# smrt-model/smrt

Measured on AMD Instinct MI355X. Metric: snowpack x frequency DORT solves/sec (20 layers, 32 streams), higher is better.
Workload: dtype f64

## Files before the change

__graft_entry__.py:

```python
import os
import subprocess
import sys
from concurrent.futures import ThreadPoolExecutor

ROOT = os.path.dirname(os.path.abspath(__file__))
CSRC = os.path.join(ROOT, "smrt_amd", "csrc")
LIB = os.path.join(CSRC, "libsmrt_dort.so")
OBJ_DIR = os.path.join(CSRC, "build")
EMU_DIR = os.path.join(ROOT, "tests", "hostemu")
EMU_LIB = os.path.join(EMU_DIR, "libsmrt_emu.so")


def _newer(target, sources):
    if not os.path.exists(target):
        return True
    t = os.path.getmtime(target)
    return any(os.path.getmtime(s) > t for s in sources)


def _run(cmd):
    print("+", " ".join(cmd), flush=True)
    subprocess.check_call(cmd, cwd=ROOT)


def _unit_flags(src):
    with open(src) as fh:
        for _ in range(10):
            line = fh.readline()
            if line.startswith("// hipcc-flags:"):
                return line.split(":", 1)[1].split()
    return []


def _compile_objects(hipcc, sources, headers, force, extra_flags=()):
    from concurrent.futures import ThreadPoolExecutor

    os.makedirs(OBJ_DIR, exist_ok=True)
    jobs = []
    for src in sources:
        obj = os.path.join(OBJ_DIR, os.path.basename(src)[:-4] + ".o")
        if force or _newer(obj, [src] + headers):
            jobs.append([hipcc, "--offload-arch=gfx950", "-O3", "-std=c++17", "-fPIC", "-fvisibility=hidden", "-Rpass-analysis=kernel-resource-usage",
                         *_unit_flags(src), *extra_flags, "-c", src, "-o", obj])

    def compile_one(cmd):
        print("+", " ".join(cmd), flush=True)
        proc = subprocess.run(cmd, cwd=ROOT, stderr=subprocess.PIPE, text=True)
        remarks, other = [], []
        for line in proc.stderr.splitlines():
            (remarks if "kernel-resource-usage" in line else other).append(line)
        kept = [ln for ln in other if not ln.lstrip().startswith(("|", "^")) and "__global__" not in ln]
        if proc.returncode != 0:
            sys.stderr.write(proc.stderr)
            raise subprocess.CalledProcessError(proc.returncode, cmd)
        if kept:
            sys.stderr.write("\n".join(kept) + "\n")
        with open(cmd[-1][:-2] + ".resources.txt", "w") as fh:
            fh.write("\n".join(ln.split("remark:", 1)[1].replace("[-Rpass-analysis=kernel-resource-usage]", "").rstrip()
                               for ln in remarks if "remark:" in ln) + "\n")

    if jobs:
        with ThreadPoolExecutor(max_workers=min(len(jobs), os.cpu_count() or 1)) as pool:
            list(pool.map(compile_one, jobs))
    return [os.path.join(OBJ_DIR, os.path.basename(src)[:-4] + ".o") for src in sources], bool(jobs)


def build(force=False):
    units = sorted(os.path.join(CSRC, f) for f in os.listdir(CSRC) if f.endswith(".hip"))
    headers = sorted(os.path.join(CSRC, f) for f in os.listdir(CSRC) if f.endswith(".hpp"))
    headers.append(os.path.join(ROOT, "include", "smrt_dort.h"))
    hip_src = [os.path.join(CSRC, "dort_hip.hip")] + headers
    hipcc = os.environ.get("HIPCC") or ("/opt/rocm/bin/hipcc" if os.path.exists("/opt/rocm/bin/hipcc") else "hipcc")
    objects, rebuilt = _compile_objects(hipcc, units, headers, force)
    if rebuilt or not os.path.exists(LIB):
        _run([hipcc, "--offload-arch=gfx950", "-shared", "-fPIC", "-o", LIB, *objects, "-ldl"])
    emu_src = hip_src[1:] + [os.path.join(EMU_DIR, "emu_lib.cpp"), os.path.join(EMU_DIR, "emu_runtime.hpp")]
    emu_jobs = [(lib, flags) for lib, flags in ((EMU_LIB, ["-O2"]), (EMU_LIB[:-3] + "_fastpanel.so", ["-O2", "-DSMRT_GJ_FAST_PANEL"]),
                                                (EMU_LIB[:-3] + "_asan.so", ["-O1", "-g", "-fsanitize=address"]))
                if force or _newer(lib, emu_src)]
    if emu_jobs:
        with ThreadPoolExecutor(max_workers=len(emu_jobs)) as pool:
            list(pool.map(lambda j: _run(["g++", "-std=c++17", "-shared", "-fPIC", *j[1], "-I", EMU_DIR, "-o", j[0],
                                          os.path.join(EMU_DIR, "emu_lib.cpp")]), emu_jobs))
    rough_lib = os.path.join(EMU_DIR, "librough_boundary_host.so")
    rough_src = os.path.join(EMU_DIR, "rough_boundary_host.cpp")
    if force or _newer(rough_lib, hip_src[1:] + [rough_src, os.path.join(EMU_DIR, "emu_runtime.hpp")]):
        _run(["g++", "-O2", "-std=c++17", "-shared", "-fPIC", "-DSMRT_HOST_EMU", "-I", EMU_DIR, "-o", rough_lib, rough_src])
    prep_lib = os.path.join(EMU_DIR, "libprep_layer_host.so")
    prep_src = os.path.join(EMU_DIR, "prep_layer_host.cpp")
    if force or _newer(prep_lib, emu_src + [prep_src]):
        _run(["g++", "-O2", "-std=c++17", "-shared", "-fPIC", "-I", EMU_DIR, "-o", prep_lib, prep_src])
    if ROOT not in sys.path:
        sys.path.insert(0, ROOT)
    import smrt_amd
    from smrt_amd import _native

    lib = _native.load_library()
    missing = [s for s in _native.EXPORTED_SYMBOLS if not hasattr(lib, s)]
    if missing:
        raise RuntimeError("libsmrt_dort.so lacks symbols: %s" % missing)
    print("build ok:", lib.smrt_dort_version().decode())


def smoke():
    if ROOT not in sys.path:
        sys.path.insert(0, ROOT)
    import numpy as np

    from oracle import dort_oracle as O
    from smrt_amd._native import DortContext, PackedBatch

    sp = dict(thickness=np.array([0.1, 100.0]), density=np.array([200.0, 400.0]),
              temperature=np.array([250.0, 250.0]), microstructure="exponential",
              corr_length=np.array([5e-5, 5e-5]))
    theta = np.deg2rad([55.0])
    batch = PackedBatch([2], sp["thickness"], sp["density"] / O.DENSITY_OF_ICE, sp["temperature"], sp["corr_length"],
                        None, [36.5e9], theta)
    ctx = DortContext(0)
    out = ctx.run(batch)
    assert out.status[0] == 0, out.status
    tb = out.values[0]
    ref = O.solve(sp, 36.5e9, [55.0])
    print("smoke: Tb(V,H) gpu =", tb[:, 0], " oracle =", ref[:, 0], " kernel ms =", ctx.last_kernel_ms())
    assert np.abs(tb - ref).max() < 1e-6
    assert np.abs(tb[:, 0] - np.array([248.09044325849692, 237.3487270223389])).max() < 1e-4
    radar = PackedBatch([2], sp["thickness"], sp["density"] / O.DENSITY_OF_ICE, sp["temperature"], sp["corr_length"],
                        None, [19e9], theta, mode="A", m_max=2)
    out = ctx.run(radar)
    assert out.status[0] == 0, out.status
    ref = O.solve(sp, 19e9, [55.0], mode="A", theta_inc_deg=[55.0])
    sig = 10 * np.log10(4 * np.pi * np.cos(theta[0]) * np.array([out.values[0][0, 0, 0], out.values[0][1, 1, 0], out.values[0][1, 0, 0]]))
    print("smoke: sigma0 (VV, HH, HV) gpu =", sig, "dB")
    assert (np.abs(out.values[0] - ref)[:2, :2] / np.abs(ref[:2, :2]).max(axis=(0, 1))).max() < 1e-8
    assert np.abs(sig - np.array([-24.044882546524693, -24.416295329469907, -51.544272924876886])).max() < 1e-4
    ctx.close()
    print("smoke ok")


if __name__ == "__main__":
    build(force="--force" in sys.argv)
    if "smoke" in sys.argv:
        smoke()
```

include/smrt_dort.h:

```cpp
#ifndef SMRT_DORT_H
#define SMRT_DORT_H

#include <stdint.h>

#ifdef __cplusplus
extern "C" {
#endif
#if defined(__GNUC__)
#pragma GCC visibility push(default)
#endif

typedef struct smrt_dort_ctx smrt_dort_ctx;

#define SMRT_EM_IBA 0
#define SMRT_EM_DMRT_QCA_SHORTRANGE 1
#define SMRT_EM_DMRT_QCACP_SHORTRANGE 2
#define SMRT_EM_NONSCATTERING 3
#define SMRT_EM_HOST 4
#define SMRT_EM_IBA_INVERTED 5
#define SMRT_EM_IBA_HOST 6
#define SMRT_EM_RAYLEIGH_HOST 7
#define SMRT_MS_EXPONENTIAL 0
#define SMRT_MS_STICKY_HARD_SPHERES 1
#define SMRT_MS_INDEPENDENT_SPHERE 2
// ... 29 lines not shown
    int32_t n_layers_max;
    int32_t n_frequencies;
    int32_t n_theta;
    int32_t emmodel;
    int32_t microstructure;
    int32_t mode;
    int32_t n_max_stream;
    int32_t m_max;
    int32_t phase_normalization;
    int32_t rayleigh_jeans;
    int32_t substrate_kind;
    const int32_t* n_layers;
    const double* thickness;
    const double* frac_volume;
    const double* temperature;
    const double* micro_p1;
    const double* micro_p2;
    const double* frequency;
    const double* theta;
    double phi;
    const double* substrate_p1;
    const double* substrate_p2;
    const double* substrate_temperature;
    const double* atm_tb_down;
    const double* atm_tb_up;
    const double* atm_transmittance;
    double prune_optical_depth;
    const int32_t* layer_kind;
    const double* host_layer;
    const int32_t* host_streams;
    const double* host_phase;
    int32_t process_coherent_layers;
    const double* host_substrate;
    const double* host_substrate_coh;
    const int32_t* host_interface_slot;
    const double* host_interface;
    const double* host_interface_coh;
    int32_t host_interface_slots;
    const double* liquid_water;
    const double* host_iba_coeff;
    const int32_t* rough_kind;
    const double* rough_params;
} smrt_batch;

#define SMRT_ROUGH_NONE 0
#define SMRT_ROUGH_GEOMETRICAL_OPTICS 1
#define SMRT_ROUGH_GEOMETRICAL_OPTICS_BACKSCATTER 2
#define SMRT_ROUGH_IEM_FUNG92 3
#define SMRT_ROUGH_M_MAX 4

int32_t smrt_dort_rough_matrices(smrt_dort_ctx* ctx, const smrt_batch* batch, int32_t* slot, double* itf, double* itf_coh,
                                 double* sub, double* sub_coh);
int32_t smrt_dort_rough_info(smrt_dort_ctx* ctx, double* info, int32_t n);

int32_t smrt_dort_out_stride(const smrt_batch* b);

int32_t smrt_dort_device_count(void);

int32_t smrt_dort_create(smrt_dort_ctx** ctx, int32_t device);
void smrt_dort_destroy(smrt_dort_ctx* ctx);
const char* smrt_dort_last_error(const smrt_dort_ctx* ctx);

int32_t smrt_dort_run(smrt_dort_ctx* ctx, const smrt_batch* batch, int64_t pair_begin, int64_t pair_count,
                      double* out, int32_t* status, double* layer_out, double* stream_out);

int32_t smrt_dort_run_pairs(smrt_dort_ctx* ctx, const smrt_batch* batch, const int64_t* pairs, int64_t n_pairs,
                            double* out, int32_t* status, double* layer_out, double* stream_out);

int32_t smrt_dort_upload(smrt_dort_ctx* ctx, const smrt_batch* batch, int64_t pair_begin, int64_t pair_count);
int32_t smrt_dort_upload_pairs(smrt_dort_ctx* ctx, const smrt_batch* batch, const int64_t* pairs, int64_t n_pairs);
int32_t smrt_dort_launch(smrt_dort_ctx* ctx, void* out_dev, void* status_dev);
int32_t smrt_dort_sync(smrt_dort_ctx* ctx);
int32_t smrt_dort_download(smrt_dort_ctx* ctx, double* out, int32_t* status, double* layer_out,
                           double* stream_out);

double smrt_dort_last_kernel_ms(smrt_dort_ctx* ctx);

int32_t smrt_dort_kernel_breakdown(smrt_dort_ctx* ctx, int32_t enable, double* ms3);

int32_t smrt_dort_set_diagonalisation(smrt_dort_ctx* ctx, int32_t mode);

int32_t smrt_dort_set_prep(smrt_dort_ctx* ctx, int32_t mode);

enum { SMRT_INFO_PIPELINE = 0, SMRT_INFO_CHUNK_PAIRS, SMRT_INFO_CHUNKS, SMRT_INFO_PRUNE_ROUNDS, SMRT_INFO_STAGED_ITEMS,
       SMRT_INFO_BLOCK_THREADS, SMRT_INFO_N_MAX, SMRT_INFO_DIAGONALISATION, SMRT_INFO_RAYLEIGH_CLOSED_FORM, SMRT_INFO_PREP,
       SMRT_INFO_COUNT };
enum { SMRT_PREP_PER_PAIR = 0, SMRT_PREP_PER_LAYER = 1 };
enum { SMRT_DIAG_JACOBI = 0,
       SMRT_DIAG_SYMMETRIC = 1 };
enum { SMRT_PIPELINE_FUSED = 0,
       SMRT_PIPELINE_LDS_TWO_SLOT = 1,
       SMRT_PIPELINE_LDS_FOUR_SLOT = 2,
       SMRT_PIPELINE_LDS_REG = 3,
       SMRT_PIPELINE_FUSED_GMEM = 4,
       SMRT_PIPELINE_GMEM = 5,
       SMRT_PIPELINE_BIG = 6,
       SMRT_PIPELINE_GMEM_STRIP = 7,
       SMRT_PIPELINE_LDS_STRIP = 8 };
int32_t smrt_dort_launch_info(smrt_dort_ctx* ctx, int64_t* info, int32_t n);
double smrt_dort_total_kernel_ms(smrt_dort_ctx* ctx, int64_t* n_launches, int32_t reset);

int32_t smrt_dort_set_block_threads(smrt_dort_ctx* ctx, int32_t threads);

int32_t smrt_dort_set_pipeline(smrt_dort_ctx* ctx, int32_t split);

int32_t smrt_dort_finish_reg_lds_bytes(int32_t n_max_stream, int32_t n_layers_max);

int32_t smrt_dort_finish_strip_lds_bytes(int32_t n_max_stream, int32_t n_layers_max, int32_t wavefronts);

int32_t smrt_dort_jacobi_lds_bytes(int32_t n_max_stream, int32_t n_pol, int32_t size_class_columns);

double smrt_dort_sum_n3(smrt_dort_ctx* ctx);

int32_t smrt_dort_ft_even_phase(smrt_dort_ctx* ctx, int32_t emmodel, int32_t microstructure, double frequency,
                                double frac_volume, double temperature, double micro_p1, double micro_p2,
                                const double* mu_s, int32_t n_s, const double* mu_i, int32_t n_i, int32_t m_max,
                                int32_t npol, double* out);

int32_t smrt_dort_pair_cost(smrt_dort_ctx* ctx, double* cost);

int32_t smrt_dort_stage_cycles(smrt_dort_ctx* ctx, double* out16);

int32_t smrt_gauss_legendre_positive(int32_t n, double* mu, double* weight);

#define SMRT_COMM_ID_BYTES 128
int32_t smrt_dort_comm_library(char* path, int32_t capacity, int32_t* version);
int32_t smrt_dort_comm_unique_id(char* id);
int32_t smrt_dort_comm_init(smrt_dort_ctx* ctx, int32_t world, int32_t rank, const char* id);
int32_t smrt_dort_comm_init_all(smrt_dort_ctx** ctxs, int32_t n);
int32_t smrt_dort_comm_destroy(smrt_dort_ctx* ctx);
int32_t smrt_dort_gather(smrt_dort_ctx* ctx, int32_t root, const int64_t* counts, double* out, int32_t* status);
int32_t smrt_dort_comm_allreduce_max(smrt_dort_ctx* ctx, double* values, int32_t n);

typedef struct smrt_gather_op { int32_t peer; int32_t reserved; int64_t offset_rows; int64_t rows; } smrt_gather_op;
int32_t smrt_dort_gather_plan(int32_t world, int32_t root, int32_t rank, const int64_t* counts, smrt_gather_op* ops,
                              int32_t capacity, int64_t* own_offset_rows, int64_t* total_rows);

int32_t smrt_dort_abi(int32_t* out, int32_t capacity);

const char* smrt_dort_version(void);

typedef struct smrt_first_order_extras {
    int32_t n_interface_slots;
    int32_t reserved;
    const int32_t* host_interface_slot;
    const double* host_interface_values;
    const double* host_phase_samples;
} smrt_first_order_extras;

int32_t smrt_first_order_out_stride(const smrt_batch* b);
int32_t smrt_first_order_run_pairs(smrt_dort_ctx* ctx, const smrt_batch* batch, const smrt_first_order_extras* extras,
                                   const int64_t* pairs, int64_t n_pairs, double* out, int32_t* status, double* layer_out,
                                   double* backscatter_layer, double* diag);
int32_t smrt_first_order_upload_pairs(smrt_dort_ctx* ctx, const smrt_batch* batch, const smrt_first_order_extras* extras,
                                      const int64_t* pairs, int64_t n_pairs);
int32_t smrt_first_order_launch(smrt_dort_ctx* ctx);
int32_t smrt_first_order_sync(smrt_dort_ctx* ctx);
int32_t smrt_first_order_download(smrt_dort_ctx* ctx, double* out, int32_t* status, double* layer_out,
                                  double* backscatter_layer, double* diag);
int32_t smrt_first_order_kernel_ms(smrt_dort_ctx* ctx, double* ms2);
int32_t smrt_first_order_abi(int32_t* out, int32_t capacity);

typedef struct smrt_second_order_extras {
    int32_t compute_scattering_interlayer;
    int32_t reserved;
    int64_t workspace_budget_bytes;
    const smrt_first_order_extras* first_order;
    const double* substrate_diffuse_modes;
} smrt_second_order_extras;
// ... 151 lines not shown
```

smrt_amd/_native.py:

```python
from __future__ import annotations

import ctypes as C
import os
import threading

import numpy as np

from .core.error import SMRTError

_HERE = os.path.dirname(os.path.abspath(__file__))
LIB_PATH = os.environ.get("SMRT_DORT_LIB") or os.path.join(_HERE, "csrc", "libsmrt_dort.so")

EM_CODES = {"iba": 0, "dmrt_qca_shortrange": 1, "dmrt_qcacp_shortrange": 2, "nonscattering": 3, "host": 4,
            "iba_inverted": 5, "iba_host": 6, "rayleigh_host": 7}
MS_CODES = {"exponential": 0, "sticky_hard_spheres": 1, "independent_sphere": 2, "teubner_strey": 3,
            "unified_scaled_exponential": 0, "unified_sticky_hard_spheres": 1, "unified_teubner_strey": 3,
            "exponential_complex_k": 4, "sticky_hard_spheres_complex_k": 5, "independent_sphere_complex_k": 6,
            "teubner_strey_complex_k": 7}
SUBSTRATE_CODES = {"flat": 1, "reflector": 2, "host": 3, "soil_wegmuller": 4, "soil_qnh": 5, "rough_choudhury79": 6}
SOIL_KINDS = ("soil_wegmuller", "soil_qnh", "rough_choudhury79")
NORM_CODES = {False: 0, None: 0, True: 1, "auto": 1, "forced": 2}
STATUS_MESSAGES = {
    1: "The eigen-decomposition did not converge in DORT.",
    2: "The re-normalization of the phase function exceeds the predefined threshold of 30%. This is likely because "
# ... 531 lines not shown
                _dptr(self.vertical), _dptr(self.echo))


_lib = None


def load_library():
    global _lib
    if _lib is not None:
        return _lib
    if not os.path.exists(LIB_PATH):
        raise SMRTError(f"{LIB_PATH} is missing: build it with `python __graft_entry__.py` (hipcc, gfx950). "
                        "smrt_amd has no CPU fallback.")
    lib = C.CDLL(LIB_PATH)
    P = C.POINTER
    lib.smrt_dort_version.restype = C.c_char_p
    lib.smrt_dort_out_stride.argtypes = [P(SmrtBatch)]
    lib.smrt_dort_out_stride.restype = C.c_int32
    lib.smrt_dort_create.argtypes = [P(C.c_void_p), C.c_int32]
    lib.smrt_dort_create.restype = C.c_int32
    lib.smrt_dort_destroy.argtypes = [C.c_void_p]
    lib.smrt_dort_destroy.restype = None
    lib.smrt_dort_last_error.argtypes = [C.c_void_p]
    lib.smrt_dort_last_error.restype = C.c_char_p
    lib.smrt_dort_run.argtypes = [C.c_void_p, P(SmrtBatch), C.c_int64, C.c_int64, P(C.c_double), P(C.c_int32),
                                  P(C.c_double), P(C.c_double)]
    lib.smrt_dort_run.restype = C.c_int32
    lib.smrt_dort_upload.argtypes = [C.c_void_p, P(SmrtBatch), C.c_int64, C.c_int64]
    lib.smrt_dort_upload.restype = C.c_int32
    lib.smrt_dort_run_pairs.argtypes = [C.c_void_p, P(SmrtBatch), P(C.c_int64), C.c_int64, P(C.c_double), P(C.c_int32),
                                        P(C.c_double), P(C.c_double)]
    lib.smrt_dort_run_pairs.restype = C.c_int32
    lib.smrt_dort_upload_pairs.argtypes = [C.c_void_p, P(SmrtBatch), P(C.c_int64), C.c_int64]
    lib.smrt_dort_upload_pairs.restype = C.c_int32
    lib.smrt_dort_ft_even_phase.argtypes = [C.c_void_p, C.c_int32, C.c_int32, C.c_double, C.c_double, C.c_double, C.c_double,
                                            C.c_double, P(C.c_double), C.c_int32, P(C.c_double), C.c_int32, C.c_int32, C.c_int32,
                                            P(C.c_double)]
    lib.smrt_dort_ft_even_phase.restype = C.c_int32
    lib.smrt_dort_rough_matrices.argtypes = [C.c_void_p, P(SmrtBatch), P(C.c_int32), P(C.c_double), P(C.c_double), P(C.c_double),
                                             P(C.c_double)]
    lib.smrt_dort_rough_matrices.restype = C.c_int32
    lib.smrt_dort_rough_info.argtypes = [C.c_void_p, P(C.c_double), C.c_int32]
    lib.smrt_dort_rough_info.restype = C.c_int32
    lib.smrt_dort_pair_cost.argtypes = [C.c_void_p, P(C.c_double)]
    lib.smrt_dort_pair_cost.restype = C.c_int32
    lib.smrt_dort_launch_info.argtypes = [C.c_void_p, P(C.c_int64), C.c_int32]
    lib.smrt_dort_launch_info.restype = C.c_int32
    lib.smrt_dort_comm_library.argtypes = [C.c_char_p, C.c_int32, P(C.c_int32)]
    lib.smrt_dort_comm_library.restype = C.c_int32
    lib.smrt_dort_comm_unique_id.argtypes = [C.c_char_p]
    lib.smrt_dort_comm_unique_id.restype = C.c_int32
    lib.smrt_dort_comm_init.argtypes = [C.c_void_p, C.c_int32, C.c_int32, C.c_char_p]
    lib.smrt_dort_comm_init.restype = C.c_int32
    lib.smrt_dort_comm_init_all.argtypes = [P(C.c_void_p), C.c_int32]
    lib.smrt_dort_comm_init_all.restype = C.c_int32
    lib.smrt_dort_comm_destroy.argtypes = [C.c_void_p]
    lib.smrt_dort_comm_destroy.restype = C.c_int32
    lib.smrt_dort_gather.argtypes = [C.c_void_p, C.c_int32, P(C.c_int64), P(C.c_double), P(C.c_int32)]
    lib.smrt_dort_gather.restype = C.c_int32
    lib.smrt_dort_comm_allreduce_max.argtypes = [C.c_void_p, P(C.c_double), C.c_int32]
    lib.smrt_dort_comm_allreduce_max.restype = C.c_int32
    lib.smrt_dort_abi.argtypes = [P(C.c_int32), C.c_int32]
    lib.smrt_dort_abi.restype = C.c_int32
    lib.smrt_dort_launch.argtypes = [C.c_void_p, C.c_void_p, C.c_void_p]
    lib.smrt_dort_launch.restype = C.c_int32
    lib.smrt_dort_sync.argtypes = [C.c_void_p]
    lib.smrt_dort_sync.restype = C.c_int32
    lib.smrt_dort_download.argtypes = [C.c_void_p, P(C.c_double), P(C.c_int32), P(C.c_double), P(C.c_double)]
    lib.smrt_dort_download.restype = C.c_int32
    lib.smrt_dort_last_kernel_ms.argtypes = [C.c_void_p]
    lib.smrt_dort_last_kernel_ms.restype = C.c_double
    lib.smrt_dort_kernel_breakdown.argtypes = [C.c_void_p, C.c_int32, P(C.c_double)]
    lib.smrt_dort_kernel_breakdown.restype = C.c_int32
    lib.smrt_dort_total_kernel_ms.argtypes = [C.c_void_p, P(C.c_int64), C.c_int32]
    lib.smrt_dort_total_kernel_ms.restype = C.c_double
    lib.smrt_dort_set_block_threads.argtypes = [C.c_void_p, C.c_int32]
    lib.smrt_dort_set_block_threads.restype = C.c_int32
    lib.smrt_dort_set_pipeline.argtypes = [C.c_void_p, C.c_int32]
    lib.smrt_dort_set_pipeline.restype = C.c_int32
    lib.smrt_dort_set_diagonalisation.argtypes = [C.c_void_p, C.c_int32]
    lib.smrt_dort_set_diagonalisation.restype = C.c_int32
    lib.smrt_dort_set_prep.argtypes = [C.c_void_p, C.c_int32]
    lib.smrt_dort_set_prep.restype = C.c_int32
    lib.smrt_dort_gather_plan.argtypes = [C.c_int32, C.c_int32, C.c_int32, P(C.c_int64), C.c_void_p, C.c_int32,
                                          P(C.c_int64), P(C.c_int64)]
    lib.smrt_dort_gather_plan.restype = C.c_int32
    lib.smrt_dort_finish_reg_lds_bytes.argtypes = [C.c_int32, C.c_int32]
    lib.smrt_dort_finish_reg_lds_bytes.restype = C.c_int32
    lib.smrt_dort_finish_strip_lds_bytes.argtypes = [C.c_int32, C.c_int32, C.c_int32]
    lib.smrt_dort_finish_strip_lds_bytes.restype = C.c_int32
    lib.smrt_dort_jacobi_lds_bytes.argtypes = [C.c_int32, C.c_int32, C.c_int32]
    lib.smrt_dort_jacobi_lds_bytes.restype = C.c_int32
    lib.smrt_dort_sum_n3.argtypes = [C.c_void_p]
    lib.smrt_dort_sum_n3.restype = C.c_double
    lib.smrt_dort_stage_cycles.argtypes = [C.c_void_p, P(C.c_double)]
    lib.smrt_dort_stage_cycles.restype = C.c_int32
    lib.smrt_dort_device_count.argtypes = []
    lib.smrt_dort_device_count.restype = C.c_int32
    lib.smrt_gauss_legendre_positive.argtypes = [C.c_int32, P(C.c_double), P(C.c_double)]
    lib.smrt_gauss_legendre_positive.restype = C.c_int32
    X = P(FirstOrderExtras)
    lib.smrt_first_order_out_stride.argtypes = [P(SmrtBatch)]
    lib.smrt_first_order_out_stride.restype = C.c_int32
    lib.smrt_first_order_run_pairs.argtypes = [C.c_void_p, P(SmrtBatch), X, P(C.c_int64), C.c_int64, P(C.c_double), P(C.c_int32),
                                               P(C.c_double), P(C.c_double), P(C.c_double)]
    lib.smrt_first_order_run_pairs.restype = C.c_int32
    lib.smrt_first_order_upload_pairs.argtypes = [C.c_void_p, P(SmrtBatch), X, P(C.c_int64), C.c_int64]
    lib.smrt_first_order_upload_pairs.restype = C.c_int32
    lib.smrt_first_order_launch.argtypes = [C.c_void_p]
    lib.smrt_first_order_launch.restype = C.c_int32
    lib.smrt_first_order_sync.argtypes = [C.c_void_p]
    lib.smrt_first_order_sync.restype = C.c_int32
    lib.smrt_first_order_download.argtypes = [C.c_void_p, P(C.c_double), P(C.c_int32), P(C.c_double), P(C.c_double), P(C.c_double)]
    lib.smrt_first_order_download.restype = C.c_int32
    lib.smrt_first_order_kernel_ms.argtypes = [C.c_void_p, P(C.c_double)]
    lib.smrt_first_order_kernel_ms.restype = C.c_int32
    lib.smrt_first_order_abi.argtypes = [P(C.c_int32), C.c_int32]
    lib.smrt_first_order_abi.restype = C.c_int32
    X2 = P(SecondOrderExtras)
    lib.smrt_second_order_out_stride.argtypes = [P(SmrtBatch)]
    lib.smrt_second_order_run_pairs.argtypes = [C.c_void_p, P(SmrtBatch), X2, P(C.c_int64), C.c_int64, P(C.c_double), P(C.c_int32),
                                                P(C.c_double), P(C.c_double), P(C.c_double)]
    lib.smrt_second_order_upload_pairs.argtypes = [C.c_void_p, P(SmrtBatch), X2, P(C.c_int64), C.c_int64]
    lib.smrt_second_order_launch.argtypes = [C.c_void_p]
    lib.smrt_second_order_sync.argtypes = [C.c_void_p]
    lib.smrt_second_order_download.argtypes = [C.c_void_p, P(C.c_double), P(C.c_int32), P(C.c_double), P(C.c_double), P(C.c_double)]
    lib.smrt_second_order_kernel_ms.argtypes = [C.c_void_p, P(C.c_double)]
    lib.smrt_second_order_abi.argtypes = [P(C.c_int32), C.c_int32]
    for name in ("out_stride", "run_pairs", "upload_pairs", "launch", "sync", "download", "kernel_ms", "abi"):
        getattr(lib, "smrt_second_order_" + name).restype = C.c_int32
    so_out = [P(C.c_double), P(C.c_int32), P(C.c_double), P(C.c_double), P(C.c_int32), P(C.c_double), P(C.c_int32)]
    lib.smrt_successive_order_out_stride.argtypes = [P(SmrtBatch), C.c_int32]
    lib.smrt_successive_order_out_stride.restype = C.c_int32
    lib.smrt_successive_order_run_pairs.argtypes = [C.c_void_p, P(SmrtBatch), C.c_int32, C.c_double, C.c_int64, P(C.c_int64), C.c_int64] + so_out
    lib.smrt_successive_order_run_pairs.restype = C.c_int32
    lib.smrt_successive_order_upload_pairs.argtypes = [C.c_void_p, P(SmrtBatch), C.c_int32, C.c_double, C.c_int64, P(C.c_int64), C.c_int64]
    lib.smrt_successive_order_upload_pairs.restype = C.c_int32
    lib.smrt_successive_order_launch.argtypes = [C.c_void_p]
    lib.smrt_successive_order_launch.restype = C.c_int32
    lib.smrt_successive_order_sync.argtypes = [C.c_void_p]
    lib.smrt_successive_order_sync.restype = C.c_int32
    lib.smrt_successive_order_download.argtypes = [C.c_void_p] + so_out
    lib.smrt_successive_order_download.restype = C.c_int32
    lib.smrt_successive_order_kernel_ms.argtypes = [C.c_void_p, P(C.c_double)]
    lib.smrt_successive_order_kernel_ms.restype = C.c_int32
    lib.smrt_successive_order_launch_info.argtypes = [C.c_void_p, P(C.c_int64), C.c_int32]
    lib.smrt_successive_order_launch_info.restype = C.c_int32
    soa_in = [C.c_void_p, P(SmrtBatch), C.c_int32, C.c_double, C.c_int32, P(C.c_double), C.c_int32, C.c_int32, C.c_int64, P(C.c_int64),
              C.c_int64]
    lib.smrt_so_active_out_stride.argtypes = [C.c_int32, C.c_int32]
    lib.smrt_so_active_out_stride.restype = C.c_int32
    lib.smrt_so_active_run_pairs.argtypes = soa_in + so_out
    lib.smrt_so_active_run_pairs.restype = C.c_int32
    lib.smrt_so_active_upload_pairs.argtypes = soa_in
    lib.smrt_so_active_upload_pairs.restype = C.c_int32
    lib.smrt_so_active_launch.argtypes = [C.c_void_p]
    lib.smrt_so_active_launch.restype = C.c_int32
    lib.smrt_so_active_sync.argtypes = [C.c_void_p]
    lib.smrt_so_active_sync.restype = C.c_int32
    lib.smrt_so_active_download.argtypes = [C.c_void_p] + so_out
    lib.smrt_so_active_download.restype = C.c_int32
    lib.smrt_so_active_kernel_ms.argtypes = [C.c_void_p, P(C.c_double)]
    lib.smrt_so_active_kernel_ms.restype = C.c_int32
    lib.smrt_so_active_launch_info.argtypes = [C.c_void_p, P(C.c_int64), C.c_int32]
    lib.smrt_so_active_launch_info.restype = C.c_int32
    mf_out = [P(C.c_double), P(C.c_int32), P(C.c_int32), P(C.c_double), P(C.c_double)]
# ... 42 lines not shown
    return lib


def abi_layout(lib):
    n = lib.smrt_dort_abi(None, 0)
    a = (C.c_int32 * n)()
    lib.smrt_dort_abi(a, n)
    return list(a)


def check_struct_layout(lib):
    mine = [C.sizeof(SmrtBatch)] + [getattr(SmrtBatch, name).offset for name, _ in SmrtBatch._fields_]
    theirs = abi_layout(lib)
    if mine != theirs:
        raise SMRTError(f"smrt_batch layout mismatch between smrt_amd/_native.py {mine} and {LIB_PATH} {theirs}: "
                        "rebuild the library or update the binding (include/smrt_dort.h)")
    mine, theirs = first_order_extras_layout(), first_order_abi_layout(lib)
    if mine != theirs:
        raise SMRTError(f"smrt_first_order_extras layout mismatch between smrt_amd/_native.py {mine} and {LIB_PATH} {theirs}: "
                        "rebuild the library or update the binding (include/smrt_dort.h)")
    mine, theirs = second_order_extras_layout(), second_order_abi_layout(lib)
    if mine != theirs:
        raise SMRTError(f"smrt_second_order_extras layout mismatch between smrt_amd/_native.py {mine} and {LIB_PATH} {theirs}: "
                        "rebuild the library or update the binding (include/smrt_dort.h)")
    mine, theirs = lrm_params_layout(), lrm_abi_layout(lib)
    if mine != theirs:
        raise SMRTError(f"smrt_lrm_params layout mismatch between smrt_amd/_native.py {mine} and {LIB_PATH} {theirs}: "
                        "rebuild the library or update the binding (include/smrt_dort.h)")
    mine, theirs = sar_params_layout(), sar_abi_layout(lib)
    if mine != theirs:
        raise SMRTError(f"smrt_sar_params layout mismatch between smrt_amd/_native.py {mine} and {LIB_PATH} {theirs}: "
                        "rebuild the library or update the binding (include/smrt_dort.h)")


def sar_params_layout():
    return [C.sizeof(SarParams)] + [getattr(SarParams, name).offset for name, _ in SarParams._fields_]


def sar_abi_layout(lib):
    n = lib.smrt_sar_abi(None, 0)
    a = (C.c_int32 * n)()
    lib.smrt_sar_abi(a, n)
    return list(a)


def lrm_params_layout():
    return [C.sizeof(LrmParams)] + [getattr(LrmParams, name).offset for name, _ in LrmParams._fields_]


def lrm_abi_layout(lib):
    n = lib.smrt_lrm_abi(None, 0)
    a = (C.c_int32 * n)()
    lib.smrt_lrm_abi(a, n)
    return list(a)


def second_order_extras_layout():
    return [C.sizeof(SecondOrderExtras)] + [getattr(SecondOrderExtras, name).offset for name, _ in SecondOrderExtras._fields_]


def second_order_abi_layout(lib):
    n = lib.smrt_second_order_abi(None, 0)
    a = (C.c_int32 * n)()
    lib.smrt_second_order_abi(a, n)
    return list(a)


def first_order_extras_layout():
    return [C.sizeof(FirstOrderExtras)] + [getattr(FirstOrderExtras, name).offset for name, _ in FirstOrderExtras._fields_]


def first_order_abi_layout(lib):
    n = lib.smrt_first_order_abi(None, 0)
    a = (C.c_int32 * n)()
    lib.smrt_first_order_abi(a, n)
    return list(a)


EXPORTED_SYMBOLS = [
    "smrt_dort_out_stride", "smrt_dort_create", "smrt_dort_destroy", "smrt_dort_last_error", "smrt_dort_run",
    "smrt_dort_upload", "smrt_dort_upload_pairs", "smrt_dort_run_pairs", "smrt_dort_abi", "smrt_dort_pair_cost", "smrt_dort_ft_even_phase",
    "smrt_dort_launch_info", "smrt_dort_comm_library", "smrt_dort_comm_unique_id", "smrt_dort_comm_init", "smrt_dort_comm_init_all", "smrt_dort_comm_destroy", "smrt_dort_gather",
    "smrt_dort_comm_allreduce_max", "smrt_dort_launch", "smrt_dort_sync", "smrt_dort_download", "smrt_dort_last_kernel_ms", "smrt_dort_kernel_breakdown",
    "smrt_dort_total_kernel_ms", "smrt_dort_set_block_threads", "smrt_dort_set_pipeline", "smrt_dort_set_diagonalisation", "smrt_dort_set_prep", "smrt_dort_sum_n3", "smrt_dort_stage_cycles", "smrt_dort_device_count", "smrt_gauss_legendre_positive",
    "smrt_dort_version", "smrt_dort_finish_reg_lds_bytes", "smrt_dort_finish_strip_lds_bytes", "smrt_dort_jacobi_lds_bytes", "smrt_dort_gather_plan",
    "smrt_first_order_out_stride", "smrt_first_order_run_pairs", "smrt_first_order_upload_pairs", "smrt_first_order_launch",
    "smrt_first_order_sync", "smrt_first_order_download", "smrt_first_order_kernel_ms", "smrt_first_order_abi",
    "smrt_second_order_out_stride", "smrt_second_order_run_pairs", "smrt_second_order_upload_pairs", "smrt_second_order_launch",
    "smrt_second_order_sync", "smrt_second_order_download", "smrt_second_order_kernel_ms", "smrt_second_order_abi",
    "smrt_successive_order_out_stride", "smrt_successive_order_run_pairs", "smrt_successive_order_upload_pairs",
    "smrt_successive_order_launch", "smrt_successive_order_sync", "smrt_successive_order_download",
    "smrt_successive_order_kernel_ms", "smrt_successive_order_launch_info",
    "smrt_so_active_out_stride", "smrt_so_active_run_pairs", "smrt_so_active_upload_pairs", "smrt_so_active_launch",
    "smrt_so_active_sync", "smrt_so_active_download", "smrt_so_active_kernel_ms", "smrt_so_active_launch_info",
    "smrt_multifresnel_out_stride", "smrt_multifresnel_run_pairs", "smrt_multifresnel_upload_pairs", "smrt_multifresnel_launch",
    "smrt_multifresnel_sync", "smrt_multifresnel_download", "smrt_multifresnel_kernel_ms",
    "smrt_lrm_out_stride", "smrt_lrm_run_pairs", "smrt_lrm_upload_pairs", "smrt_lrm_launch", "smrt_lrm_sync", "smrt_lrm_download",
    "smrt_lrm_kernel_ms", "smrt_lrm_abi", "smrt_lrm_layers",
    "smrt_sar_out_stride", "smrt_sar_run_pairs", "smrt_sar_upload_pairs", "smrt_sar_launch", "smrt_sar_sync", "smrt_sar_download",
    "smrt_sar_kernel_ms", "smrt_sar_abi",
    "smrt_dort_rough_matrices", "smrt_dort_rough_info",
]


class RoughMatrices:

    def __init__(self, batch):
        s = batch.struct
        S, Lmax = int(s.n_snowpacks), int(s.n_layers_max)
        FS, ne = batch.n_pairs, 3 * int(s.n_max_stream)
        nm = int(s.m_max) + 1 if batch.mode == "A" else 1
        kinds = batch.rough_kind
        self.slots = max(int(np.count_nonzero(kinds[k, :batch.n_layers[k]])) for k in range(S))
        self.has_substrate = bool(kinds[0, batch.n_layers[0]])
        self.slot = -np.ones((FS, Lmax), np.int32)
        self.itf = np.zeros((FS, self.slots, nm, 4, ne, ne))
        self.itf_coh = np.zeros((FS, self.slots, 4, ne))
        self.sub = np.zeros((FS, nm, ne, ne))
        self.sub_coh = np.zeros((FS, nm, ne))

    def pointers(self):
        return (self.slot.ctypes.data_as(C.POINTER(C.c_int32)), _dptr(self.itf), _dptr(self.itf_coh), _dptr(self.sub),
                _dptr(self.sub_coh))


class BatchOutput:
    def __init__(self, batch, pair_count):
        Lmax, nmax = int(batch.struct.n_layers_max), int(batch.struct.n_max_stream)
        self.values = np.empty((pair_count,) + batch.out_shape(), dtype=np.float64)
        self.status = np.empty(pair_count, dtype=np.int32)
        self.layers = np.empty((pair_count, Lmax, 5), dtype=np.float64)
        self.streams = np.empty((pair_count, 1 + nmax), dtype=np.float64)


class DortContext:

    def __init__(self, device=0):
        self._lib = load_library()
        self._h = C.c_void_p()
        rc = self._lib.smrt_dort_create(C.byref(self._h), int(device))
        if rc != 0:
            self._h = C.c_void_p()
            raise SMRTError(f"smrt_dort_create(device={device}) failed with code {rc}: no usable MI355X GPU. "
                            "smrt_amd has no CPU fallback.")
        self.device = int(device)
        self.lock = threading.RLock()

    def close(self):
        if getattr(self, "_h", None) is not None and self._h.value:
            self._lib.smrt_dort_destroy(self._h)
            self._h = C.c_void_p()

    def __del__(self):
        try:
            self.close()
        except Exception:
            pass

    def _check(self, rc, what):
        if rc != 0:
            raise SMRTError(f"{what} failed: {self._lib.smrt_dort_last_error(self._h).decode()}")

    def set_block_threads(self, n):
        self._check(self._lib.smrt_dort_set_block_threads(self._h, int(n)), "smrt_dort_set_block_threads")

    def set_pipeline(self, split=1):
        self._check(self._lib.smrt_dort_set_pipeline(self._h, int(split)), "smrt_dort_set_pipeline")

    DIAGONALISATIONS = ("jacobi", "symmetric")

    def set_diagonalisation(self, mode="default"):
        code = -1 if mode in (None, "default") else self.DIAGONALISATIONS.index(mode)
        self._check(self._lib.smrt_dort_set_diagonalisation(self._h, code), "smrt_dort_set_diagonalisation")

    PREPS = ("per_pair", "per_layer")

    def set_prep(self, mode="default"):
        code = -1 if mode in (None, "default") else self.PREPS.index(mode)
        self._check(self._lib.smrt_dort_set_prep(self._h, code), "smrt_dort_set_prep")

    def run(self, batch: PackedBatch, pair_begin=0, pair_count=-1, pairs=None) -> BatchOutput:
        if pairs is not None:
            pairs = np.ascontiguousarray(pairs, dtype=np.int64)
            o = BatchOutput(batch, len(pairs))
            with self.lock:
                self._check(self._lib.smrt_dort_run_pairs(
                    self._h, C.byref(batch.struct), pairs.ctypes.data_as(C.POINTER(C.c_int64)), len(pairs),
                    _dptr(o.values), o.status.ctypes.data_as(C.POINTER(C.c_int32)), _dptr(o.layers), _dptr(o.streams)),
                    "smrt_dort_run_pairs")
            return o
        if pair_count < 0:
            pair_count = batch.n_pairs - pair_begin
        o = BatchOutput(batch, pair_count)
        with self.lock:
            self._check(self._lib.smrt_dort_run(self._h, C.byref(batch.struct), pair_begin, pair_count, _dptr(o.values),
                                                o.status.ctypes.data_as(C.POINTER(C.c_int32)), _dptr(o.layers),
                                                _dptr(o.streams)), "smrt_dort_run")
        return o

    def upload(self, batch: PackedBatch, pair_begin=0, pair_count=-1, pairs=None):
        if pairs is not None:
            pairs = np.ascontiguousarray(pairs, dtype=np.int64)
            self._check(self._lib.smrt_dort_upload_pairs(self._h, C.byref(batch.struct),
                                                         pairs.ctypes.data_as(C.POINTER(C.c_int64)), len(pairs)),
                        "smrt_dort_upload_pairs")
            self._resident = (batch, len(pairs))
            return
        if pair_count < 0:
            pair_count = batch.n_pairs - pair_begin
        self._check(self._lib.smrt_dort_upload(self._h, C.byref(batch.struct), pair_begin, pair_count), "smrt_dort_upload")
        self._resident = (batch, pair_count)

    def launch(self, out_dev=None, status_dev=None):
        self._check(self._lib.smrt_dort_launch(self._h, C.c_void_p(out_dev or 0), C.c_void_p(status_dev or 0)),
                    "smrt_dort_launch")

    def sync(self):
        self._check(self._lib.smrt_dort_sync(self._h), "smrt_dort_sync")

    def download(self) -> BatchOutput:
        batch, pair_count = self._resident
        o = BatchOutput(batch, pair_count)
        self._check(self._lib.smrt_dort_download(self._h, _dptr(o.values), o.status.ctypes.data_as(C.POINTER(C.c_int32)),
                                                 _dptr(o.layers), _dptr(o.streams)), "smrt_dort_download")
        return o

    def _solver_call(self, symbol, *args):
        with self.lock:
            rc = getattr(self._lib, symbol)(self._h, *args)
            if rc < 0:
                raise SMRTError(f"{symbol} failed: {self._lib.smrt_dort_last_error(self._h).decode()}")
        return rc

    def _solver_run(self, prefix, output, cargs, oargs):
        o = output(*oargs)
        self._solver_call(f"smrt_{prefix}_run_pairs", *cargs, *o.pointers())
        return o

    def _solver_upload(self, prefix, cargs, oargs):
        with self.lock:
            self._solver_call(f"smrt_{prefix}_upload_pairs", *cargs)
            setattr(self, f"_{prefix}_resident", oargs)

    def _solver_download(self, prefix, output):
        with self.lock:
            o = output(*getattr(self, f"_{prefix}_resident"))
            self._solver_call(f"smrt_{prefix}_download", *o.pointers())
        return o

    def _solver_kernel_ms(self, prefix, n):
        a = np.zeros(n)
        self._solver_call(f"smrt_{prefix}_kernel_ms", _dptr(a))
        return tuple(float(x) for x in a)

    def _solver_launch_info(self, prefix):
        a = np.zeros(4, dtype=np.int64)
        self._solver_call(f"smrt_{prefix}_launch_info", a.ctypes.data_as(C.POINTER(C.c_int64)), 4)
        return dict(chunks=int(a[0]), reserved_bytes=int(a[1]), over_budget=int(a[2]), budget=int(a[3]))

    @staticmethod
    def _pair_list(batch, pairs):
        if pairs is None:
            return None, -1, batch.n_pairs
# ... 159 lines not shown
        self._solver_upload("lrm", *self._lrm_pack(batch, params, pairs))

    def lrm_layers(self, batch: PackedBatch, params):
        a = np.empty((batch.n_pairs, int(batch.struct.n_layers_max), 5))
        with self.lock:
            self.lrm_upload(batch, params)
            self._solver_call("smrt_lrm_layers", _dptr(a))
        return a

    def lrm_launch(self):
        self._solver_call("smrt_lrm_launch")

    def lrm_sync(self):
        self._solver_call("smrt_lrm_sync")

    def lrm_download(self) -> LrmOutput:
        return self._solver_download("lrm", LrmOutput)

    def lrm_kernel_ms(self):
        return self._solver_kernel_ms("lrm", 3)

    def sar_run(self, batch: PackedBatch, params, pairs=None) -> SarOutput:
        return self._solver_run("sar", SarOutput, *self._lrm_pack(batch, params, pairs))

    def sar_upload(self, batch: PackedBatch, params, pairs=None):
        self._solver_upload("sar", *self._lrm_pack(batch, params, pairs))

    def sar_launch(self):
        self._solver_call("smrt_sar_launch")

    def sar_sync(self):
        self._solver_call("smrt_sar_sync")

    def sar_download(self) -> SarOutput:
        return self._solver_download("sar", SarOutput)

    def sar_kernel_ms(self):
        return self._solver_kernel_ms("sar", 4)

    def ft_even_phase(self, emmodel, microstructure, frequency, frac_volume, temperature, p1, p2, mu_s, mu_i, m_max, npol):
        mu_s = np.ascontiguousarray(np.atleast_1d(mu_s), dtype=np.float64)
        mu_i = np.ascontiguousarray(np.atleast_1d(mu_i), dtype=np.float64)
        out = np.empty((npol, npol, m_max + 1, len(mu_s), len(mu_i)))
        with self.lock:
            self._check(self._lib.smrt_dort_ft_even_phase(
                self._h, EM_CODES[emmodel], MS_CODES[microstructure], float(frequency), float(frac_volume), float(temperature),
                float(p1), float(p2), _dptr(mu_s), len(mu_s), _dptr(mu_i), len(mu_i), int(m_max), int(npol), _dptr(out)),
                "smrt_dort_ft_even_phase")
        return out

    rough_on_device = True

    @property
    def rough_workspace_budget(self):
        v = (C.c_double * 6)()
        self._lib.smrt_dort_rough_info(self._h, v, 6)
        return min(4 << 30, int(0.5 * v[5]))

    def rough_matrices(self, batch: PackedBatch) -> RoughMatrices:
        o = RoughMatrices(batch)
        with self.lock:
            rc = self._lib.smrt_dort_rough_matrices(self._h, C.byref(batch.struct), *o.pointers())
            self._check(0 if rc >= 0 else -1, "smrt_dort_rough_matrices")
        return o

    def rough_info(self):
        v = (C.c_double * 5)()
        self._lib.smrt_dort_rough_info(self._h, v, 5)
        return dict(m_max_limit=int(v[0]), slots=int(v[1]), builder_ms=float(v[2]), built_bytes=int(v[3]), host_matrix_bytes=int(v[4]))

    def pair_cost(self):
        _, pair_count = self._resident
        cost = np.empty(pair_count)
        self._check(self._lib.smrt_dort_pair_cost(self._h, _dptr(cost)), "smrt_dort_pair_cost")
        return cost

    PIPELINES = ("fused", "lds_two_slot", "lds_four_slot", "lds_reg", "fused_gmem", "gmem", "big", "gmem_strip", "lds_strip")

    def launch_info(self):
        v = (C.c_int64 * 16)()
        n = self._lib.smrt_dort_launch_info(self._h, v, 16)
        self._check(0 if n > 0 else -1, "smrt_dort_launch_info")
        keys = ("pipeline", "chunk_pairs", "chunks", "prune_rounds", "staged_items", "block_threads", "n_max", "diagonalisation",
                "rayleigh_closed_form", "prep")
        d = {k: int(v[i]) for i, k in enumerate(keys[:n])}
        d["pipeline"] = self.PIPELINES[d["pipeline"]]
        d["diagonalisation"] = self.DIAGONALISATIONS[d["diagonalisation"]]
        d["rayleigh_closed_form"] = bool(d.get("rayleigh_closed_form", 0))
        d["prep"] = self.PREPS[d.get("prep", 0)]
        if d.get("staged_items", -1) < 0:
            d["staged_items"] = None
        return d

    @staticmethod
    def comm_library():
        lib = load_library()
        buf, version = C.create_string_buffer(1024), C.c_int32(0)
        if lib.smrt_dort_comm_library(buf, len(buf), C.byref(version)) != 0:
            raise SMRTError("RCCL is not available: " + buf.value.decode(errors="replace"))
        v = int(version.value)
        return buf.value.decode(), "%d.%d.%d" % (v // 10000, v // 100 % 100, v % 100) if v >= 10000 else str(v)

    @staticmethod
    def comm_unique_id():
        lib = load_library()
        buf = C.create_string_buffer(128)
        if lib.smrt_dort_comm_unique_id(buf) != 0:
            raise SMRTError("smrt_dort_comm_unique_id failed (is librccl available?)")
        return buf.raw

    def comm_init(self, world, rank, unique_id):
        self._check(self._lib.smrt_dort_comm_init(self._h, int(world), int(rank), bytes(unique_id)), "smrt_dort_comm_init")
        self.world, self.rank = int(world), int(rank)

    @staticmethod
    def comm_init_all(contexts):
        lib = load_library()
        arr = (C.c_void_p * len(contexts))(*[c._h for c in contexts])
        if lib.smrt_dort_comm_init_all(arr, len(contexts)) != 0:
            raise SMRTError("smrt_dort_comm_init_all failed: " + lib.smrt_dort_last_error(contexts[0]._h).decode())
        for r, c in enumerate(contexts):
            c.world, c.rank = len(contexts), r

    def gather(self, counts, root=0, want_host=True):
        batch, _ = self._resident
        counts = np.ascontiguousarray(counts, dtype=np.int64)
        is_root = self.rank == root and want_host
        total = int(counts.sum())
        values = np.empty((total,) + batch.out_shape()) if is_root else None
        status = np.empty(total, np.int32) if is_root else None
        self._check(self._lib.smrt_dort_gather(self._h, int(root), counts.ctypes.data_as(C.POINTER(C.c_int64)),
                                               _dptr(values) if is_root else None,
                                               status.ctypes.data_as(C.POINTER(C.c_int32)) if is_root else None),
                    "smrt_dort_gather")
        return values, status

    def allreduce_max(self, values):
        a = np.ascontiguousarray(np.atleast_1d(values), dtype=np.float64).copy()
        self._check(self._lib.smrt_dort_comm_allreduce_max(self._h, _dptr(a), len(a)), "smrt_dort_comm_allreduce_max")
        return a

    def barrier(self):
        self._check(self._lib.smrt_dort_comm_allreduce_max(self._h, None, 0), "smrt_dort_comm_allreduce_max")

    def last_kernel_ms(self):
        return float(self._lib.smrt_dort_last_kernel_ms(self._h))

    def total_kernel_ms(self, reset=False):
        n = C.c_int64()
        ms = float(self._lib.smrt_dort_total_kernel_ms(self._h, C.byref(n), 1 if reset else 0))
        return ms, int(n.value)

    STAGE_NAMES = ["setup", "assemble", "cholesky", "LtL", "jacobi", "triangular", "R1", "LU1", "R45", "LU2", "R78",
                   "out"]

    def kernel_breakdown(self, enable=None):
        if enable is not None:
            self._check(min(self._lib.smrt_dort_kernel_breakdown(self._h, 1 if enable else 0, None), 0), "smrt_dort_kernel_breakdown")
            return None
        a = np.zeros(3)
        n = self._lib.smrt_dort_kernel_breakdown(self._h, -1, _dptr(a))
        self._check(min(n, 0), "smrt_dort_kernel_breakdown")
        return {"prep": float(a[0]), "jacobi": float(a[1]), "finish": float(a[2]), "intervals": int(n)}

    def stage_cycles(self):
        a = np.zeros(16)
        self._check(self._lib.smrt_dort_stage_cycles(self._h, _dptr(a)), "smrt_dort_stage_cycles")
        d = dict(zip(self.STAGE_NAMES, a[: len(self.STAGE_NAMES)]))
        d["_jacobi_sweeps"] = a[12]
        d["_gj_panel"], d["_gj_update"], d["_gj_perm"] = a[13], a[14], a[15]
        return d

# ... 31 lines not shown
```

smrt_amd/csrc/dort_ctx.hpp:

```cpp
#pragma once
#include <hip/hip_runtime.h>
#include <string>
#include <vector>

#include "dort_layout.hpp"

namespace smrt { struct PhaseRequest; struct FoBatch; }
struct smrt_batch;

struct DevBuf {
    void* p = nullptr;
    size_t cap = 0;
    hipError_t reserve(size_t bytes) {
        if (bytes <= cap) return hipSuccess;
        if (p) (void)hipFree(p);
        p = nullptr;
        cap = 0;
        hipError_t e = hipMalloc(&p, bytes);
        if (e == hipSuccess) cap = bytes;
        return e;
    }
    void release() { if (p) (void)hipFree(p); p = nullptr; cap = 0; }
};

struct smrt_dort_ctx {
    int device = 0;
    hipStream_t stream = nullptr;
    hipEvent_t ev0 = nullptr, ev1 = nullptr;
    std::string err;
    DevBuf d_nl, d_thick, d_fv, d_temp, d_p1, d_p2, d_freq, d_theta, d_gl, d_out, d_status, d_layer, d_stream, d_n3, d_stage, d_work, d_stL, d_stB, d_std, d_sts, d_stn, d_sti, d_sub1, d_sub2, d_subT, d_atm, d_pairmap, d_kind, d_phase, d_done, d_hostlayer, d_hostcoeff, d_hoststreams, d_hostphase, d_dispatch, d_regws, d_itfslot, d_itf, d_itfcoh, d_lw, d_ste, d_strot, d_strec;
    smrt::DevBatch dev{};
    bool uploaded = false;
    int out_stride = 0;
    int nt = 256;
    size_t lds_bytes = 0;
    size_t prep_lds_bytes = 0;
    size_t finish2_lds_bytes = 0;
    size_t finish_reg_lds_bytes = 0;
    size_t prep_wide_lds_bytes = 0;
    int prep_mode = -1;
    bool prep_layers = false;
    bool prep_wide = false;
    size_t finish_strip_lds_bytes = 0, finish_strip4_lds_bytes = 0;
    bool finish_strip4 = false;
    bool finish_strip = false;
    bool finish_reg = false;
    int finish_mode = -1;
    bool finish2 = true;
    float last_ms = 0.f;
    double total_ms = 0.0;
    int64_t n_launch = 0;
    bool timing_pending = false;
    bool breakdown_on = false;
    std::vector<hipEvent_t> bd_events;
    std::vector<int> bd_kind;
    size_t bd_used = 0;
    int max_lds = 0;
    bool split = true;
    long long chunk_pairs = 0;
    int lanes = 1;
    hipStream_t lane_stream[4] = {nullptr, nullptr, nullptr, nullptr};
    hipEvent_t lane_ev[4] = {nullptr, nullptr, nullptr, nullptr};
    hipEvent_t fork_ev = nullptr;
    size_t jacobi_lds = 0;
    int diag_mode = -1;
    bool eig = false;
    size_t jacobi16_lds = 0;
    smrt::DevStage stage{};
    bool gmem_path = false;
    bool gmem_split = false;
    bool big = false;
    int jac_in_lds = 0;
    bool active = false;
    int gmem_grid = 0;
    long long ws_stride = 0;
    int nmax_rows = 0;
    void* comm = nullptr;
    int comm_world = 0, comm_rank = 0;
    DevBuf d_gather_out, d_gather_status, d_scalar;
    struct FirstOrderState* first_order = nullptr;
    struct SuccessiveOrderState* successive_order = nullptr;
    struct SuccessiveOrderActiveState* successive_order_active = nullptr;
    struct MultiFresnelState* multifresnel = nullptr;
    struct SecondOrderState* second_order = nullptr;
    struct LrmState* lrm = nullptr;
    struct SarState* sar = nullptr;
    struct RoughState* rough = nullptr;
    struct { int slots = 0, has_sub = 0; float ms = 0.f; size_t built_bytes = 0, host_matrix_bytes = 0; } rough_info;
};

#ifndef SMRT_JACOBI_NT
#define SMRT_JACOBI_NT 256
#endif

namespace smrt_launch {
hipError_t prep(smrt_dort_ctx* ctx, const smrt::DevBatch& c, int nt);
hipError_t prep_wide(smrt_dort_ctx* ctx, const smrt::DevBatch& c);
hipError_t finish(smrt_dort_ctx* ctx, const smrt::DevBatch& c, int nt, bool two_slot);
void occupancy_report(smrt_dort_ctx* ctx, int nt);
hipError_t prep_layers(smrt_dort_ctx* ctx, const smrt::DevBatch& c, long long items);
hipError_t finish_reg(smrt_dort_ctx* ctx, const smrt::DevBatch& c);
hipError_t finish_strip(smrt_dort_ctx* ctx, const smrt::DevBatch& c);
hipError_t finish_strip4(smrt_dort_ctx* ctx, const smrt::DevBatch& c);
hipError_t jacobi(smrt_dort_ctx* ctx, const smrt::DevBatch& c, long long items);
hipError_t eig(smrt_dort_ctx* ctx, const smrt::DevBatch& c, long long items);
hipError_t rayleigh(smrt_dort_ctx* ctx, const smrt::DevBatch& c, long long items);
hipError_t active_prep(smrt_dort_ctx* ctx, const smrt::DevBatch& c, int nt);
hipError_t active_finish(smrt_dort_ctx* ctx, const smrt::DevBatch& c, int nt);
hipError_t prep_gmem(smrt_dort_ctx* ctx, const smrt::DevBatch& c, unsigned grid, bool active);
hipError_t finish_gmem(smrt_dort_ctx* ctx, const smrt::DevBatch& c, unsigned grid, bool active);
hipError_t prep_gmem_big(smrt_dort_ctx* ctx, const smrt::DevBatch& c, unsigned grid, bool active, int ch);
hipError_t finish_gmem_big(smrt_dort_ctx* ctx, const smrt::DevBatch& c, unsigned grid, bool active, int ch);
hipError_t jacobi_big(smrt_dort_ctx* ctx, const smrt::DevBatch& c, long long items);
hipError_t fused(smrt_dort_ctx* ctx, const smrt::DevBatch& d, int nt, bool active);
hipError_t fused_gmem(smrt_dort_ctx* ctx, const smrt::DevBatch& d, int ch, bool active);
hipError_t ft_even_phase(smrt_dort_ctx* ctx, const smrt::PhaseRequest& q);
hipError_t prune_mark(smrt_dort_ctx* ctx, const smrt::DevBatch& c, int* done_dev);
hipError_t pair_cost(smrt_dort_ctx* ctx, const smrt::DevBatch& d, double* cost_dev);
void first_order_release(smrt_dort_ctx* ctx);
void successive_order_release(smrt_dort_ctx* ctx);
void successive_order_active_release(smrt_dort_ctx* ctx);
void multifresnel_release(smrt_dort_ctx* ctx);
void second_order_release(smrt_dort_ctx* ctx);
void lrm_release(smrt_dort_ctx* ctx);
void sar_release(smrt_dort_ctx* ctx);
int rough_prepare(smrt_dort_ctx* ctx, const smrt_batch* b, smrt::DevBatch& d);
void rough_release(smrt_dort_ctx* ctx);
smrt::FoBatch* first_order_resident(smrt_dort_ctx* ctx);
}
```

smrt_amd/csrc/dort_device.hpp:

```cpp
#pragma once
#include "spmd.hpp"
#include <math.h>
#include <string.h>

#include "dort_layout.hpp"
#include "dort_physics.hpp"
#include "dort_dense.hpp"
#include "dort_gauss_jordan.hpp"
#include "dort_passive.hpp"
#include "dort_jacobi_kernel.hpp"
#include "dort_jacobi_big.hpp"
```

smrt_amd/csrc/dort_hip.hip:

```cpp
#include <hip/hip_runtime.h>
#include <algorithm>
#include <cstddef>
#include <cstdio>
#include <cstdlib>
#include <cstring>
#include <string>
#include <vector>

#include "dort_ctx.hpp"
#include "dort_eig_kernel.hpp"
#include "dort_rayleigh_kernel.hpp"
#include "dort_jacobi_big.hpp"
#include "dort_host_common.hpp"
#include "dort_phase_kernel.hpp"
#include "dort_finish_reg.hpp"
#include "dort_finish_strip.hpp"
#include "solver_host.hpp"

using namespace smrt;

static int upload_array(smrt_dort_ctx* ctx, DevBuf& buf, const void* src, size_t bytes) {
    HIPCHK(buf.reserve(bytes));
    HIPCHK(hipMemcpyAsync(buf.p, src, bytes, hipMemcpyHostToDevice, ctx->stream));
    return 0;
}


static DevBatch chunk_of(const smrt_dort_ctx* ctx, const DevBatch& d, long long c0, long long cn) {
    DevBatch c = d;
    c.pair_begin = d.pair_begin + c0; c.pair_count = cn;
    c.out = d.out + c0 * ctx->out_stride; c.status = d.status + c0;
    c.layer_out = d.layer_out + c0 * (long long)d.Lmax * 5;
    c.stream_out = d.stream_out + c0 * (long long)(1 + d.n_max_stream);
    c.n3_out = d.n3_out + c0; c.stage_out = d.stage_out + c0 * 16;
    if (d.dispatch) c.dispatch = d.dispatch + c0;
    return c;
}

#ifndef SMRT_DORT_LANES_DEFAULT
#define SMRT_DORT_LANES_DEFAULT 1
#endif
#ifndef SMRT_PREP_DEFAULT
#define SMRT_PREP_DEFAULT SMRT_PREP_PER_LAYER
#endif
#ifndef SMRT_FINISH_STRIP_DEFAULT
#define SMRT_FINISH_STRIP_DEFAULT 1
#endif
#ifndef SMRT_FINISH_REG_DEFAULT
#define SMRT_FINISH_REG_DEFAULT 1
#endif
static hipError_t launch_pipeline(smrt_dort_ctx* ctx, const DevBatch& d) {
    const long long items_per_pair = (long long)(ctx->active ? d.m_max + 1 : 1) * d.Lmax;
    const long long modes = ctx->active ? d.m_max + 1 : 1;
    if (getenv("SMRT_DORT_DEBUG_OCCUPANCY") && !ctx->gmem_path && !ctx->active) smrt_launch::occupancy_report(ctx, ctx->nt);
    const int rounds = (d.prune_tau > 0.0 && !d.coherent && getenv("SMRT_DORT_NO_PRUNE_ROUNDS") == nullptr) ? std::min(4, d.Lmax) : 1;
    auto prep = [&](const DevBatch& c, unsigned grid) {
        if (ctx->prep_layers) return smrt_launch::prep_layers(ctx, c, c.pair_count * (c.layer_hi - c.layer_lo));
        if (ctx->big) return smrt_launch::prep_gmem_big(ctx, c, grid, ctx->active, ctx->nmax_rows <= 256 ? 4 : 6);
        if (ctx->prep_wide) return smrt_launch::prep_wide(ctx, c);
        if (ctx->gmem_split) return smrt_launch::prep_gmem(ctx, c, grid, ctx->active);
        return ctx->active ? smrt_launch::active_prep(ctx, c, ctx->nt) : smrt_launch::prep(ctx, c, ctx->nt);
    };
    auto finish = [&](const DevBatch& c, unsigned grid) {
        if (ctx->big) return smrt_launch::finish_gmem_big(ctx, c, grid, ctx->active, ctx->nmax_rows <= 256 ? 4 : 6);
        if (ctx->finish_strip) return smrt_launch::finish_strip(ctx, c);
        if (ctx->gmem_split) return smrt_launch::finish_gmem(ctx, c, grid, ctx->active);
        if (ctx->finish_strip4) return smrt_launch::finish_strip4(ctx, c);
        if (ctx->finish_reg) return smrt_launch::finish_reg(ctx, c);
        return ctx->active ? smrt_launch::active_finish(ctx, c, ctx->nt) : smrt_launch::finish(ctx, c, ctx->nt, ctx->finish2);
    };
    const hipStream_t main_stream = ctx->stream;
    const DevStage stage0 = ctx->stage;
    const int lanes = (ctx->lanes > 1 && d.pair_count > ctx->chunk_pairs) ? ctx->lanes : 1;
    struct Restore { smrt_dort_ctx* c; hipStream_t s; DevStage st; ~Restore() { c->stream = s; c->stage = st; } } restore{ctx, main_stream, stage0};
    if (lanes > 1) {
        hipError_t e;
        if ((e = hipEventRecord(ctx->fork_ev, main_stream)) != hipSuccess) return e;
        for (int k = 0; k < lanes; ++k)
            if ((e = hipStreamWaitEvent(ctx->lane_stream[k], ctx->fork_ev, 0)) != hipSuccess) return e;
    }
    auto timed = [&](int kind, auto&& launch) -> hipError_t {
        if (!ctx->breakdown_on) return launch();
        for (int k = 0; k < 2; ++k)
            if (ctx->bd_used + k >= ctx->bd_events.size()) {
                hipEvent_t ev;
                hipError_t e = hipEventCreate(&ev);
                if (e != hipSuccess) return e;
                ctx->bd_events.push_back(ev);
            }
        hipError_t e = hipEventRecord(ctx->bd_events[ctx->bd_used], ctx->stream);
        if (e != hipSuccess) return e;
        e = launch();
        if (e != hipSuccess) return e;
        e = hipEventRecord(ctx->bd_events[ctx->bd_used + 1], ctx->stream);
        ctx->bd_used += 2;
        ctx->bd_kind.push_back(kind);
        return e;
    };
    if (ctx->breakdown_on) { ctx->bd_used = 0; ctx->bd_kind.clear(); }
    long long chunk_index = 0;
    for (long long c0 = 0; c0 < d.pair_count; c0 += ctx->chunk_pairs, ++chunk_index) {
        const long long cn = std::min<long long>(ctx->chunk_pairs, d.pair_count - c0);
        DevBatch c = chunk_of(ctx, d, c0, cn);
        const unsigned grid = (unsigned)(ctx->gmem_path ? std::min<long long>(cn, ctx->gmem_grid) : cn);
        hipError_t e;
        const int lane = (int)(chunk_index % lanes);
        int* done_lane = (int*)ctx->d_done.p + (size_t)lane * ctx->chunk_pairs;
        if (lanes > 1) {
            const long long it0 = (long long)lane * ctx->chunk_pairs * items_per_pair;
            ctx->stream = ctx->lane_stream[lane];
            ctx->stage = stage0;
            ctx->stage.L = stage0.L + it0 * stage0.mat_stride; ctx->stage.B = stage0.B + it0 * stage0.mat_stride;
            ctx->stage.d = stage0.d + it0 * stage0.vec_stride; ctx->stage.sigma = stage0.sigma + it0 * stage0.vec_stride;
            ctx->stage.n = stage0.n + it0; ctx->stage.Linv = stage0.Linv + it0 * stage0.linv_stride;
            if (stage0.eig_rot) { ctx->stage.eig_e = stage0.eig_e + it0 * 2 * stage0.vec_stride; ctx->stage.eig_rot = stage0.eig_rot + it0 * stage0.rot_stride; }
            if (stage0.rec) ctx->stage.rec = stage0.rec + it0 * stage0.rec_stride;
            if (stage0.ws) ctx->stage.ws = stage0.ws + (long long)lane * ctx->chunk_pairs * rg::kSlotDoubles;
        }
        if (rounds > 1 || d.coherent) {
            if ((e = hipMemsetAsync(ctx->stage.n, 0, sizeof(int) * (size_t)(cn * items_per_pair), ctx->stream)) != hipSuccess) return e;
        }
        if (rounds > 1) {
            if ((e = hipMemsetAsync(done_lane, 0, sizeof(int) * (size_t)cn, ctx->stream)) != hipSuccess) return e;
            c.pair_done = (const int*)done_lane;
        }
        for (int r = 0; r < rounds; ++r) {
            c.layer_lo = (int)((long long)d.Lmax * r / rounds);
            c.layer_hi = (int)((long long)d.Lmax * (r + 1) / rounds);
            if ((e = timed(0, [&]() { return prep(c, grid); })) != hipSuccess) return e;
            const long long jitems = cn * modes * (c.layer_hi - c.layer_lo);
            if ((e = timed(1, [&]() { hipError_t e1 = ctx->big ? smrt_launch::jacobi_big(ctx, c, jitems) : ctx->eig ? smrt_launch::eig(ctx, c, jitems) : smrt_launch::jacobi(ctx, c, jitems);
                                           if (e1 == hipSuccess && c.rayleigh_direct) e1 = smrt_launch::rayleigh(ctx, c, jitems);
                                           return e1; })) != hipSuccess) return e;
            if (r + 1 < rounds && (e = smrt_launch::prune_mark(ctx, c, done_lane)) != hipSuccess) return e;
        }
        c.layer_lo = 0; c.layer_hi = d.Lmax; c.pair_done = nullptr;
        if ((e = timed(2, [&]() { return finish(c, grid); })) != hipSuccess) return e;
    }
    if (lanes > 1) {
        for (int k = 0; k < lanes; ++k) {
            hipError_t e;
            if ((e = hipEventRecord(ctx->lane_ev[k], ctx->lane_stream[k])) != hipSuccess) return e;
            if ((e = hipStreamWaitEvent(main_stream, ctx->lane_ev[k], 0)) != hipSuccess) return e;
        }
    }
    return hipSuccess;
}

extern "C" {

const char* smrt_dort_version(void) { return "smrt_dort 0.1 (gfx950)"; }

int32_t smrt_dort_out_stride(const smrt_batch* b) { return smrt_host::out_stride(b); }

int32_t smrt_gauss_legendre_positive(int32_t n, double* mu, double* weight) {
    if (n < 1 || !mu) return -1;
    smrt_host::gauss_legendre_positive(n, mu, weight);
    return 0;
}

int32_t smrt_dort_device_count(void) {
    int ndev = 0;
    if (hipGetDeviceCount(&ndev) != hipSuccess) return 0;
    return ndev;
}

int32_t smrt_dort_create(smrt_dort_ctx** out, int32_t device) {
    if (!out) return -1;
    *out = nullptr;
    int ndev = 0;
    if (hipGetDeviceCount(&ndev) != hipSuccess || ndev <= 0) return -2;
    if (device < 0 || device >= ndev) return -3;
    smrt_dort_ctx* ctx = new smrt_dort_ctx();
    ctx->device = device;
    if (hipSetDevice(device) != hipSuccess || hipStreamCreateWithFlags(&ctx->stream, hipStreamNonBlocking) != hipSuccess ||
        hipEventCreate(&ctx->ev0) != hipSuccess || hipEventCreate(&ctx->ev1) != hipSuccess) {
        delete ctx;
        return -4;
    }
    hipDeviceProp_t prop;
    if (hipGetDeviceProperties(&prop, device) == hipSuccess) ctx->max_lds = (int)prop.sharedMemPerBlock;
    if (ctx->max_lds < 160 * 1024) ctx->max_lds = 160 * 1024;
    *out = ctx;
    return 0;
}

void smrt_dort_destroy(smrt_dort_ctx* ctx) {
    if (!ctx) return;
    (void)smrt_dort_comm_destroy(ctx);
    (void)hipSetDevice(ctx->device);
    DevBuf* bufs[] = {&ctx->d_nl, &ctx->d_thick, &ctx->d_fv, &ctx->d_temp, &ctx->d_p1, &ctx->d_p2, &ctx->d_freq,
                      &ctx->d_theta, &ctx->d_gl, &ctx->d_out, &ctx->d_status, &ctx->d_layer, &ctx->d_stream, &ctx->d_n3, &ctx->d_stage, &ctx->d_work,
                      &ctx->d_stL, &ctx->d_stB, &ctx->d_std, &ctx->d_sts, &ctx->d_stn, &ctx->d_sti, &ctx->d_ste, &ctx->d_strot, &ctx->d_strec, &ctx->d_regws, &ctx->d_itfslot, &ctx->d_itf, &ctx->d_itfcoh,
                      &ctx->d_sub1, &ctx->d_sub2, &ctx->d_subT, &ctx->d_atm, &ctx->d_pairmap, &ctx->d_kind, &ctx->d_hostlayer, &ctx->d_hoststreams, &ctx->d_hostphase, &ctx->d_dispatch, &ctx->d_phase, &ctx->d_done, &ctx->d_lw, &ctx->d_gather_out, &ctx->d_gather_status,
                      &ctx->d_scalar};
    for (DevBuf* b : bufs) b->release();
    smrt_launch::first_order_release(ctx);
    smrt_launch::successive_order_release(ctx);
    smrt_launch::successive_order_active_release(ctx);
    smrt_launch::multifresnel_release(ctx);
    smrt_launch::lrm_release(ctx);
    smrt_launch::sar_release(ctx);
    smrt_launch::second_order_release(ctx);
    smrt_launch::rough_release(ctx);
    if (ctx->ev0) (void)hipEventDestroy(ctx->ev0);
    if (ctx->ev1) (void)hipEventDestroy(ctx->ev1);
    for (int k = 0; k < 4; ++k) {
        if (ctx->lane_ev[k]) (void)hipEventDestroy(ctx->lane_ev[k]);
        if (ctx->lane_stream[k]) (void)hipStreamDestroy(ctx->lane_stream[k]);
    }
    if (ctx->fork_ev) (void)hipEventDestroy(ctx->fork_ev);
    for (hipEvent_t ev : ctx->bd_events) (void)hipEventDestroy(ev);
    if (ctx->stream) (void)hipStreamDestroy(ctx->stream);
    delete ctx;
}

const char* smrt_dort_last_error(const smrt_dort_ctx* ctx) { return ctx ? ctx->err.c_str() : "null context"; }

int32_t smrt_dort_set_pipeline(smrt_dort_ctx* ctx, int32_t split) {
    if (!ctx) return -1;
    ctx->split = (split != 0);
    ctx->finish2 = (split != 2);
    ctx->finish_mode = (split == 3) ? 1 : (split == 4 ? 0 : (split == 5 ? 2 : -1));
    ctx->uploaded = false;
    return 0;
}

int32_t smrt_dort_set_diagonalisation(smrt_dort_ctx* ctx, int32_t mode) {
    if (!ctx) return -1;
    if (mode < -1 || mode > SMRT_DIAG_SYMMETRIC) { ctx->err = "unknown diagonalisation mode"; return -1; }
    ctx->diag_mode = mode;
    ctx->uploaded = false;
    return 0;
}

int32_t smrt_dort_set_prep(smrt_dort_ctx* ctx, int32_t mode) {
    if (!ctx) return -1;
    if (mode < -1 || mode > SMRT_PREP_PER_LAYER) { ctx->err = "unknown prep mode"; return -1; }
    ctx->prep_mode = mode;
    ctx->uploaded = false;
    return 0;
}

int32_t smrt_dort_finish_reg_lds_bytes(int32_t n_max_stream, int32_t n_layers_max) {
    return (int32_t)(sizeof(double) * (size_t)finish_reg_lds_doubles(n_max_stream, n_layers_max));
}

int32_t smrt_dort_finish_strip_lds_bytes(int32_t n_max_stream, int32_t n_layers_max, int32_t wavefronts) {
    if (wavefronts != 4 && wavefronts != 8) return -1;
    return (int32_t)(sizeof(double) * (size_t)finish_strip_lds_doubles(n_max_stream, n_layers_max, wavefronts));
}

int32_t smrt_dort_jacobi_lds_bytes(int32_t n_max_stream, int32_t n_pol, int32_t size_class_columns) {
    if (n_max_stream < 1 || (n_pol != 2 && n_pol != 3) || n_max_stream * n_pol > 128 || size_class_columns < 0) return -1;
    return (int32_t)(make_jacobi_plan(n_max_stream, n_pol, size_class_columns).total * sizeof(double));
}

int32_t smrt_dort_set_block_threads(smrt_dort_ctx* ctx, int32_t threads) {
    if (!ctx) return -1;
    if (threads == 0) threads = 256;
    if (threads != 64 && threads != 256) {
        ctx->err = "block threads must be 64 or 256";
        return -1;
    }
    ctx->nt = threads;
    return 0;
}

}

static int32_t upload_impl(smrt_dort_ctx* ctx, const smrt_batch* b, int64_t pair_begin, int64_t pair_count,
                           const int64_t* pairs) {
    if (!ctx) return -1;
    const char* why = smrt_host::validate(b);
    if (why) { ctx->err = why; return -1; }
    HIPCHK(hipSetDevice(ctx->device));
    ctx->active = (b->mode == SMRT_MODE_ACTIVE);
    if (ctx->active && (b->m_max < 0 || b->m_max > 64)) { ctx->err = "m_max must be in 0..64"; return -1; }
    const int64_t npairs = (int64_t)b->n_snowpacks * b->n_frequencies;
    if (pairs) {
        pair_begin = 0;
        if (pair_count <= 0) { ctx->err = "empty pair list"; return -1; }
        for (int64_t i = 0; i < pair_count; ++i)
            if (pairs[i] < 0 || pairs[i] >= npairs) { ctx->err = "pair index out of bounds"; return -1; }
    } else {
        if (pair_count < 0) pair_count = npairs - pair_begin;
        if (pair_begin < 0 || pair_count <= 0 || pair_begin + pair_count > npairs) { ctx->err = "pair range out of bounds"; return -1; }
    }
    const int P = ctx->active ? 3 : 2;
    const int nphi = ctx->active ? azimuth_samples(b->m_max) / 2 + 1 : 9;
    const int actd = ctx->active ? active_doubles(b->n_max_stream, b->n_layers_max, b->n_theta) : 0;
    const int actd_fin = ctx->active ? active_doubles(b->n_max_stream, b->n_layers_max, b->n_theta, false) : 0;
    LdsPlan plan = make_plan(b->n_max_stream, P, b->n_layers_max, b->n_theta, nphi, 1, actd);
    size_t lds = (size_t)plan.total * sizeof(double);
    ctx->gmem_path = (plan.NMAX > 64 || lds > (size_t)ctx->max_lds || getenv("SMRT_DORT_FORCE_GLOBAL_WORKSPACE") != nullptr);
    if (ctx->gmem_path) {
        if (plan.NMAX > 384) {
            ctx->err = "streams x polarisations above 384 (n_max_stream > 192 passive, > 128 active) is not supported by this build";
            return -1;
        }
        plan = make_plan(b->n_max_stream, P, b->n_layers_max, b->n_theta, nphi, 0, actd, 0, 1);
        ctx->jac_in_lds = 1;
        if ((size_t)plan.total * sizeof(double) > (size_t)ctx->max_lds) {
            plan = make_plan(b->n_max_stream, P, b->n_layers_max, b->n_theta, nphi, 0, actd);
            ctx->jac_in_lds = 0;
        }
        lds = (size_t)plan.total * sizeof(double);
        if (lds > (size_t)ctx->max_lds) { ctx->err = "too many layers for the LDS-resident per-layer tables"; return -1; }
        ctx->gmem_grid = (int)std::min<int64_t>(pair_count, 1024);
        ctx->ws_stride = (long long)plan.mat_doubles + plan.scratch_doubles;
        HIPCHK(ctx->d_work.reserve(sizeof(double) * (size_t)ctx->gmem_grid * (size_t)ctx->ws_stride));
    }
    ctx->nmax_rows = plan.NMAX;
    ctx->chunk_pairs = 0;
    ctx->eig = false;
    {
        int want = ctx->prep_mode < 0 ? SMRT_PREP_DEFAULT : ctx->prep_mode;
        if (const char* e = getenv("SMRT_DORT_PREP_LAYERS")) want = atoi(e) ? SMRT_PREP_PER_LAYER : SMRT_PREP_PER_PAIR;
        ctx->prep_layers = !ctx->gmem_path && ctx->split && !ctx->active && plan.NMAX <= 64 && want == SMRT_PREP_PER_LAYER;
    }
    const size_t rec_doubles = ctx->prep_layers ? (size_t)prep_record_doubles(b->n_max_stream) : 0;
    int big_min = 128;
    if (const char* e = getenv("SMRT_DORT_BIG_MIN_N")) big_min = std::max(64, atoi(e));
    ctx->big = ctx->gmem_path && ctx->split && plan.NMAX > big_min && getenv("SMRT_DORT_NO_BIG_PIPELINE") == nullptr &&
               (size_t)make_jacobi_big_plan(b->n_max_stream, P).total * sizeof(double) <= (size_t)ctx->max_lds;
    const bool split128 = ctx->gmem_path && ctx->split && !ctx->big && plan.NMAX <= 128 &&
        (size_t)make_jacobi_plan(b->n_max_stream, P).total * sizeof(double) <= (size_t)ctx->max_lds &&
        (size_t)make_plan(b->n_max_stream, P, b->n_layers_max, b->n_theta, nphi, 0, actd_fin, 0, 2).total * sizeof(double) <= (size_t)ctx->max_lds &&
        (size_t)make_plan(b->n_max_stream, P, b->n_layers_max, b->n_theta, nphi, 0, actd, 1).total * sizeof(double) <= (size_t)ctx->max_lds;
    if (split128) ctx->jac_in_lds = 1;
    ctx->gmem_split = ctx->big || split128;
    if (ctx->big) ctx->jac_in_lds = 0;
    if ((!ctx->gmem_path && ctx->split) || ctx->gmem_split) {
        const size_t nmodes = ctx->active ? (size_t)b->m_max + 1 : 1;
        const size_t mat = (size_t)plan.NMAX * plan.LD;
        const int linv_stride = (plan.NMAX > 64) ? 2048 : 1024;
        const size_t per_pair = nmodes * b->n_layers_max * ((2 * mat + 2 * plan.NMAX + linv_stride + rec_doubles) * sizeof(double) + sizeof(int));
        double budget = 12.0e9;
        if (ctx->big) {
            size_t free_b = 0, total_b = 0;
            if (hipMemGetInfo(&free_b, &total_b) == hipSuccess) budget = std::max(budget, 0.6 * (double)(free_b + ctx->d_stL.cap + ctx->d_stB.cap));
        }
        const bool one_per_cu = ctx->gmem_split && !ctx->big;
        if (one_per_cu) budget = 40.0e9;
        long long chunk = (long long)(budget / (double)per_pair);
        if (chunk < 1) chunk = 1;
        if (one_per_cu && chunk >= 512) chunk -= chunk % 256;
        const long long chunk_cap = chunk;
        if (chunk > pair_count) chunk = pair_count;
        {
            int want = ctx->diag_mode < 0 ? SMRT_DIAG_SYMMETRIC : ctx->diag_mode;
            if (const char* e = getenv("SMRT_DORT_EIG")) want = atoi(e) ? SMRT_DIAG_SYMMETRIC : SMRT_DIAG_JACOBI;
            ctx->eig = !ctx->gmem_path && !ctx->active && plan.NMAX <= 64 && want == SMRT_DIAG_SYMMETRIC;
        }
        ctx->lanes = 1;
        if (!ctx->gmem_path) {
            int want = ctx->eig ? 3 : SMRT_DORT_LANES_DEFAULT;
            if (const char* e = getenv("SMRT_DORT_LANES")) want = atoi(e);
            ctx->lanes = std::max(1, std::min(4, want));
            while (ctx->lanes > 1 && pair_count < 1024LL * ctx->lanes) --ctx->lanes;
        }
        {
            long long nchunks = (pair_count + chunk - 1) / chunk;
            if (ctx->lanes > 1) nchunks = ((nchunks + ctx->lanes - 1) / ctx->lanes) * ctx->lanes;
            chunk = (pair_count + nchunks - 1) / nchunks;
            if (one_per_cu && nchunks > 1) chunk = std::min(chunk_cap, ((chunk + 255) / 256) * 256);
        }
        ctx->chunk_pairs = chunk;
        for (int k = 0; k < ctx->lanes && ctx->lanes > 1; ++k) {
            if (!ctx->lane_stream[k]) HIPCHK(hipStreamCreateWithFlags(&ctx->lane_stream[k], hipStreamNonBlocking));
            if (!ctx->lane_ev[k]) HIPCHK(hipEventCreateWithFlags(&ctx->lane_ev[k], hipEventDisableTiming));
        }
        if (ctx->lanes > 1 && !ctx->fork_ev) HIPCHK(hipEventCreateWithFlags(&ctx->fork_ev, hipEventDisableTiming));
        const size_t items = (size_t)chunk * ctx->lanes * b->n_layers_max * nmodes;
        HIPCHK(ctx->d_stL.reserve(items * mat * sizeof(double)));
        HIPCHK(ctx->d_stB.reserve(items * mat * sizeof(double)));
        HIPCHK(ctx->d_std.reserve(items * plan.NMAX * sizeof(double)));
        HIPCHK(ctx->d_sts.reserve(items * plan.NMAX * sizeof(double)));
        HIPCHK(ctx->d_stn.reserve(items * sizeof(int)));
        HIPCHK(ctx->d_sti.reserve(ctx->big ? 8 : items * linv_stride * sizeof(double)));
        ctx->stage.L = (double*)ctx->d_stL.p; ctx->stage.B = (double*)ctx->d_stB.p;
        ctx->stage.d = (double*)ctx->d_std.p; ctx->stage.sigma = (double*)ctx->d_sts.p;
        ctx->stage.n = (int*)ctx->d_stn.p; ctx->stage.Linv = ctx->big ? nullptr : (double*)ctx->d_sti.p;
        ctx->stage.linv_stride = linv_stride;
        ctx->stage.mat_stride = (long long)mat; ctx->stage.vec_stride = plan.NMAX;
        ctx->stage.rec = nullptr; ctx->stage.rec_stride = (int)rec_doubles;
        if (ctx->prep_layers) {
            HIPCHK(ctx->d_strec.reserve(items * rec_doubles * sizeof(double)));
            ctx->stage.rec = (double*)ctx->d_strec.p;
        }
        {
            ctx->stage.eig_e = nullptr; ctx->stage.eig_rot = nullptr; ctx->stage.rot_stride = 0;
            if (ctx->eig) {
                const long long rs = eig_rot_doubles(plan.NMAX);
                HIPCHK(ctx->d_ste.reserve(items * 2 * plan.NMAX * sizeof(double)));
                HIPCHK(ctx->d_strot.reserve(items * (size_t)rs * sizeof(double)));
                ctx->stage.eig_e = (double*)ctx->d_ste.p; ctx->stage.eig_rot = (double*)ctx->d_strot.p; ctx->stage.rot_stride = rs;
            }
        }
        ctx->jacobi_lds = ctx->big ? (size_t)make_jacobi_big_plan(b->n_max_stream, P).total * sizeof(double)
                                   : (size_t)make_jacobi_plan(b->n_max_stream, P).total * sizeof(double);
        ctx->jacobi16_lds = 0;
        if (ctx->gmem_split && !ctx->big) {
            const size_t l16 = (size_t)make_jacobi_plan(b->n_max_stream, P, 0, 16).total * sizeof(double);
            if (l16 <= (size_t)ctx->max_lds) ctx->jacobi16_lds = l16;
        }
        ctx->prep_lds_bytes = (size_t)make_plan(b->n_max_stream, P, b->n_layers_max, b->n_theta, nphi, ctx->gmem_split ? 0 : 1, actd,
                                                (!ctx->gmem_split && !ctx->active) ? 3 : 1).total * sizeof(double);
        ctx->finish2_lds_bytes = ctx->gmem_split
            ? (size_t)make_plan(b->n_max_stream, P, b->n_layers_max, b->n_theta, nphi, 0, actd_fin, 0, ctx->big ? 3 : 2).total * sizeof(double)
            : (size_t)make_plan(b->n_max_stream, P, b->n_layers_max, b->n_theta, nphi, 1, actd_fin, 2).total * sizeof(double);
    }
    {
        const bool supported = !ctx->gmem_path && ctx->split && ctx->finish2 && !ctx->active && ctx->chunk_pairs > 0 &&
                               !b->process_coherent_layers && b->substrate_kind != SUB_HOST && !b->host_interface_slot && !b->rough_kind;
        int want = (ctx->finish_mode == 2) ? -1 : ctx->finish_mode;
        if (const char* e = getenv("SMRT_DORT_FINISH_REG")) want = atoi(e) ? 1 : 0;
        ctx->finish_reg_lds_bytes = sizeof(double) * (size_t)finish_reg_lds_doubles(b->n_max_stream, b->n_layers_max);
        const size_t cap = (want == 1) ? (size_t)64 * 1024 : (size_t)160 * 1024 / 3;
        ctx->finish_reg = supported && ctx->finish_reg_lds_bytes <= cap &&
                          (want == 1 || (want == -1 && SMRT_FINISH_REG_DEFAULT));
        ctx->stage.ws = nullptr;
        ctx->finish_strip4 = false;
        {
            int want4 = (ctx->finish_mode == 2) ? 1 : (ctx->finish_mode == -1 ? -1 : 0);
            if (getenv("SMRT_DORT_FINISH_REG") && want == 1 && want4 == -1) want4 = 0;
            if (const char* e = getenv("SMRT_DORT_FINISH_STRIP4")) want4 = atoi(e) ? 1 : 0;
            const size_t lds4 = sizeof(double) * (size_t)finish_strip_lds_doubles(b->n_max_stream, b->n_layers_max, 4);
            const size_t cap4 = (want4 == 1) ? (size_t)64 * 1024 : (size_t)160 * 1024 / 3;
            if (supported && lds4 <= cap4 && (want4 == 1 || (want4 == -1 && SMRT_FINISH_STRIP_DEFAULT))) {
                ctx->finish_strip4 = true; ctx->finish_strip4_lds_bytes = lds4; ctx->finish_reg = false;
                HIPCHK(ctx->d_regws.reserve(sizeof(double) * (size_t)ctx->chunk_pairs * ctx->lanes * StripFinish<4>::kWsDoubles));
                ctx->stage.ws = (double*)ctx->d_regws.p;
            }
        }
        if (ctx->finish_reg) {
            HIPCHK(ctx->d_regws.reserve(sizeof(double) * (size_t)ctx->chunk_pairs * ctx->lanes * rg::kSlotDoubles));
// ... 45 lines not shown
    if (b->host_layer && b->host_streams && b->host_phase) {
        const size_t PL = (size_t)npairs * b->n_layers_max;
        if (upload_array(ctx, ctx->d_hoststreams, b->host_streams, sizeof(int32_t) * PL)) return -1;
        if (upload_array(ctx, ctx->d_hostphase, b->host_phase, sizeof(double) * PL * host_modes * 2 * host_ne * host_ne)) return -1;
    }
    const size_t FS = (size_t)b->n_snowpacks * b->n_frequencies;
    ctx->rough_info = {};
    if (b->host_interface_slot) {
        const size_t ne = 3 * (size_t)b->n_max_stream, nm = ctx->active ? (size_t)b->m_max + 1 : 1, ns = (size_t)b->host_interface_slots;
        if (upload_array(ctx, ctx->d_itfslot, b->host_interface_slot, sizeof(int32_t) * FS * b->n_layers_max)) return -1;
        if (upload_array(ctx, ctx->d_itf, b->host_interface, sizeof(double) * FS * ns * nm * 4 * ne * ne)) return -1;
        if (upload_array(ctx, ctx->d_itfcoh, b->host_interface_coh, sizeof(double) * FS * ns * 4 * ne)) return -1;
        ctx->rough_info.host_matrix_bytes += sizeof(double) * FS * ns * nm * 4 * ne * ne;
    }
    if (b->substrate_kind == SMRT_SUBSTRATE_HOST) {
        const size_t ne = 3 * (size_t)b->n_max_stream, nm = ctx->active ? (size_t)b->m_max + 1 : 1;
        if (upload_array(ctx, ctx->d_sub1, b->host_substrate, sizeof(double) * FS * nm * ne * ne)) return -1;
        if (upload_array(ctx, ctx->d_sub2, b->host_substrate_coh, sizeof(double) * FS * nm * ne)) return -1;
        if (b->substrate_temperature && upload_array(ctx, ctx->d_subT, b->substrate_temperature, sizeof(double) * b->n_snowpacks)) return -1;
        ctx->rough_info.host_matrix_bytes += sizeof(double) * FS * nm * ne * ne;
    } else
    if (smrt_host::rough_substrate(b)) {
        if (upload_array(ctx, ctx->d_subT, b->substrate_temperature, sizeof(double) * b->n_snowpacks)) return -1;
    } else
    if (b->substrate_kind != SMRT_SUBSTRATE_NONE) {
        const size_t sub_doubles = smrt_host::substrate_array_doubles(b);
        if (upload_array(ctx, ctx->d_sub1, b->substrate_p1, sizeof(double) * sub_doubles)) return -1;
        if (upload_array(ctx, ctx->d_sub2, b->substrate_p2, sizeof(double) * sub_doubles)) return -1;
        if (upload_array(ctx, ctx->d_subT, b->substrate_temperature, sizeof(double) * b->n_snowpacks)) return -1;
    }
    std::vector<double> atm;
    if (b->atm_tb_down) {
        atm.insert(atm.end(), b->atm_tb_down, b->atm_tb_down + b->n_frequencies);
        atm.insert(atm.end(), b->atm_tb_up, b->atm_tb_up + b->n_frequencies);
        atm.insert(atm.end(), b->atm_transmittance, b->atm_transmittance + b->n_frequencies);
        if (upload_array(ctx, ctx->d_atm, atm.data(), sizeof(double) * atm.size())) return -1;
    }
    std::vector<double> gl(b->n_max_stream);
    smrt_host::gauss_legendre_positive(b->n_max_stream, gl.data(), nullptr);
    if (upload_array(ctx, ctx->d_gl, gl.data(), sizeof(double) * gl.size())) return -1;
    ctx->out_stride = smrt_host::out_stride(b);
    HIPCHK(ctx->d_out.reserve(sizeof(double) * pair_count * ctx->out_stride));
    HIPCHK(ctx->d_status.reserve(sizeof(int32_t) * pair_count));
    HIPCHK(ctx->d_layer.reserve(sizeof(double) * pair_count * b->n_layers_max * 5));
    HIPCHK(ctx->d_stream.reserve(sizeof(double) * pair_count * (1 + b->n_max_stream)));
    HIPCHK(ctx->d_n3.reserve(sizeof(double) * pair_count));
    HIPCHK(ctx->d_stage.reserve(sizeof(double) * pair_count * 16));
    HIPCHK(hipMemsetAsync(ctx->d_stage.p, 0, sizeof(double) * pair_count * 16, ctx->stream));
    DevBatch& d = ctx->dev;
    d.S = b->n_snowpacks; d.Lmax = b->n_layers_max; d.F = b->n_frequencies; d.n_theta = b->n_theta;
    d.emmodel = b->emmodel; d.micro = b->microstructure; d.mode = b->mode; d.n_max_stream = b->n_max_stream;
    d.m_max = b->m_max; d.normalization = b->phase_normalization; d.rayleigh_jeans = b->rayleigh_jeans;
    d.want_layer_out = 1; d.want_stream_out = 1;
    d.jac_in_lds = ctx->gmem_path ? ctx->jac_in_lds : 0;
    d.pair_begin = pair_begin; d.pair_count = pair_count;
    d.pair_map = pairs ? (const long long*)ctx->d_pairmap.p : nullptr;
    d.n_layers = (const int*)ctx->d_nl.p; d.thickness = (const double*)ctx->d_thick.p;
    d.frac_volume = (const double*)ctx->d_fv.p; d.temperature = (const double*)ctx->d_temp.p;
    d.p1 = (const double*)ctx->d_p1.p; d.p2 = (const double*)ctx->d_p2.p;
    d.frequency = (const double*)ctx->d_freq.p; d.theta = (const double*)ctx->d_theta.p;
    d.gl_mu = (const double*)ctx->d_gl.p; d.phi = b->phi;
    d.layer_kind = b->layer_kind ? (const int*)ctx->d_kind.p : nullptr;
    d.liquid_water = b->liquid_water ? (const double*)ctx->d_lw.p : nullptr;
    const bool has_host = b->host_layer && b->host_streams && b->host_phase;
    d.host_layer = b->host_layer ? (const double*)ctx->d_hostlayer.p : nullptr;
    d.host_coeff = (b->host_layer && b->host_iba_coeff) ? (const double*)ctx->d_hostcoeff.p : nullptr;
    d.host_streams = has_host ? (const int*)ctx->d_hoststreams.p : nullptr;
    d.host_phase = has_host ? (const double*)ctx->d_hostphase.p : nullptr;
    d.host_modes = (int)host_modes; d.host_ne = (int)host_ne;
    d.coherent = b->process_coherent_layers ? 1 : 0;
    d.sub_kind = b->substrate_kind;
    d.sub_p1 = (const double*)ctx->d_sub1.p; d.sub_p2 = (const double*)ctx->d_sub2.p; d.sub_T = (const double*)ctx->d_subT.p;
    d.host_itf_slot = b->host_interface_slot ? (const int*)ctx->d_itfslot.p : nullptr;
    d.host_itf = b->host_interface_slot ? (const double*)ctx->d_itf.p : nullptr;
    d.host_itf_coh = b->host_interface_slot ? (const double*)ctx->d_itfcoh.p : nullptr;
    d.host_itf_slots = b->host_interface_slot ? b->host_interface_slots : 0;
    d.host_substrate = (const double*)ctx->d_sub1.p; d.host_substrate_coh = (const double*)ctx->d_sub2.p;
    const bool has_atm = (b->atm_tb_down != nullptr) && b->mode == SMRT_MODE_PASSIVE;
    d.atm_down = has_atm ? (const double*)ctx->d_atm.p : nullptr;
    d.atm_up = has_atm ? (const double*)ctx->d_atm.p + b->n_frequencies : nullptr;
    d.atm_trans = has_atm ? (const double*)ctx->d_atm.p + 2 * b->n_frequencies : nullptr;
    d.prune_tau = (b->prune_optical_depth > 0.0) ? b->prune_optical_depth : 0.0;
    d.layer_lo = 0; d.layer_hi = b->n_layers_max; d.pair_done = nullptr;
    if (d.prune_tau > 0.0) HIPCHK(ctx->d_done.reserve(sizeof(int) * (size_t)std::max<long long>(ctx->chunk_pairs, 1) * ctx->lanes));
    const bool orth = ctx->finish_reg || ctx->finish_strip || ctx->finish_strip4;
    d.jacobi_skip2 = ctx->active ? 1e-30 : (orth ? SMRT_JACOBI_REG_SKIP_COS2 : SMRT_JACOBI_PASSIVE_SKIP_COS2);
    d.jacobi_exit2 = ctx->active ? 1e-22 : (orth ? SMRT_JACOBI_REG_EXIT_COS2 : SMRT_JACOBI_PASSIVE_EXIT_COS2);
    if (const char* e = getenv("SMRT_DORT_JACOBI_SKIP2")) d.jacobi_skip2 = atof(e);
    if (const char* e = getenv("SMRT_DORT_JACOBI_EXIT2")) d.jacobi_exit2 = atof(e);
    d.out = (double*)ctx->d_out.p; d.status = (int*)ctx->d_status.p; d.layer_out = (double*)ctx->d_layer.p;
    d.stream_out = (double*)ctx->d_stream.p; d.n3_out = (double*)ctx->d_n3.p; d.stage_out = (double*)ctx->d_stage.p;
    {
        const bool may_hold = b->layer_kind != nullptr || em_has_rayleigh_phase(b->emmodel);
        const char* e = getenv("SMRT_DORT_RAYLEIGH");
        d.rayleigh_direct = (!ctx->active && (ctx->finish_strip || ctx->finish_strip4) && ctx->stage.Linv && may_hold && !(e && atoi(e) == 0)) ? 1 : 0;
    }
    ctx->lds_bytes = lds;
    if (b->rough_kind && smrt_launch::rough_prepare(ctx, b, d)) return -1;
    HIPCHK(hipStreamSynchronize(ctx->stream));
    ctx->uploaded = true;
    d.dispatch = nullptr;
    if (pair_count > 1 && getenv("SMRT_DORT_NO_COST_ORDER") == nullptr) {
        HIPCHK(smrt_launch::pair_cost(ctx, d, d.n3_out));
        std::vector<double> cost((size_t)pair_count);
        HIPCHK(hipMemcpyAsync(cost.data(), d.n3_out, sizeof(double) * cost.size(), hipMemcpyDeviceToHost, ctx->stream));
        HIPCHK(hipStreamSynchronize(ctx->stream));
        std::vector<int32_t> order((size_t)pair_count);
        const long long chunk = ctx->chunk_pairs > 0 ? ctx->chunk_pairs : pair_count;
        for (long long c0 = 0; c0 < pair_count; c0 += chunk) {
            const long long cn = std::min<long long>(chunk, pair_count - c0);
            for (long long i = 0; i < cn; ++i) order[(size_t)(c0 + i)] = (int32_t)i;
            std::stable_sort(order.begin() + c0, order.begin() + c0 + cn,
                             [&](int32_t a, int32_t b2) { return cost[(size_t)(c0 + a)] > cost[(size_t)(c0 + b2)]; });
        }
        if (upload_array(ctx, ctx->d_dispatch, order.data(), sizeof(int32_t) * order.size())) return -1;
        d.dispatch = (const int*)ctx->d_dispatch.p;
    }
    return 0;
}

extern "C" {

int32_t smrt_dort_upload(smrt_dort_ctx* ctx, const smrt_batch* b, int64_t pair_begin, int64_t pair_count) {
    return upload_impl(ctx, b, pair_begin, pair_count, nullptr);
}

int32_t smrt_dort_upload_pairs(smrt_dort_ctx* ctx, const smrt_batch* b, const int64_t* pairs, int64_t n_pairs) {
    if (ctx && !pairs) { ctx->err = "null pair list"; return -1; }
    return upload_impl(ctx, b, 0, n_pairs, pairs);
}

int32_t smrt_dort_abi(int32_t* out, int32_t capacity) {
#define SMRT_OFF(f) (int32_t)offsetof(smrt_batch, f)
    const int32_t desc[] = {(int32_t)sizeof(smrt_batch),
        SMRT_OFF(n_snowpacks), SMRT_OFF(n_layers_max), SMRT_OFF(n_frequencies), SMRT_OFF(n_theta), SMRT_OFF(emmodel),
        SMRT_OFF(microstructure), SMRT_OFF(mode), SMRT_OFF(n_max_stream), SMRT_OFF(m_max), SMRT_OFF(phase_normalization),
        SMRT_OFF(rayleigh_jeans), SMRT_OFF(substrate_kind), SMRT_OFF(n_layers), SMRT_OFF(thickness), SMRT_OFF(frac_volume),
        SMRT_OFF(temperature), SMRT_OFF(micro_p1), SMRT_OFF(micro_p2), SMRT_OFF(frequency), SMRT_OFF(theta), SMRT_OFF(phi),
        SMRT_OFF(substrate_p1), SMRT_OFF(substrate_p2), SMRT_OFF(substrate_temperature), SMRT_OFF(atm_tb_down),
        SMRT_OFF(atm_tb_up), SMRT_OFF(atm_transmittance), SMRT_OFF(prune_optical_depth), SMRT_OFF(layer_kind),
        SMRT_OFF(host_layer), SMRT_OFF(host_streams), SMRT_OFF(host_phase), SMRT_OFF(process_coherent_layers),
        SMRT_OFF(host_substrate), SMRT_OFF(host_substrate_coh), SMRT_OFF(host_interface_slot), SMRT_OFF(host_interface),
        SMRT_OFF(host_interface_coh), SMRT_OFF(host_interface_slots), SMRT_OFF(liquid_water), SMRT_OFF(host_iba_coeff),
        SMRT_OFF(rough_kind), SMRT_OFF(rough_params)};
#undef SMRT_OFF
    const int32_t n = (int32_t)(sizeof(desc) / sizeof(desc[0]));
    for (int32_t i = 0; out && i < n && i < capacity; ++i) out[i] = desc[i];
    return n;
}

int32_t smrt_dort_rough_matrices(smrt_dort_ctx* ctx, const smrt_batch* b, int32_t* slot, double* itf, double* itf_coh, double* sub,
                                 double* sub_coh) {
    if (!ctx) return -1;
    if (!b || !b->rough_kind) { ctx->err = "smrt_dort_rough_matrices needs a batch with rough_kind"; return -1; }
    if (upload_impl(ctx, b, 0, -1, nullptr)) return -1;
    const size_t FS = (size_t)b->n_snowpacks * b->n_frequencies, ne = 3 * (size_t)b->n_max_stream, nm = ctx->active ? (size_t)b->m_max + 1 : 1;
    const size_t ns = (size_t)ctx->rough_info.slots;
    if (ns > 0) {
        if (slot) HIPCHK(hipMemcpy(slot, ctx->d_itfslot.p, sizeof(int32_t) * FS * b->n_layers_max, hipMemcpyDeviceToHost));
        if (itf) HIPCHK(hipMemcpy(itf, ctx->d_itf.p, sizeof(double) * FS * ns * nm * 4 * ne * ne, hipMemcpyDeviceToHost));
        if (itf_coh) HIPCHK(hipMemcpy(itf_coh, ctx->d_itfcoh.p, sizeof(double) * FS * ns * 4 * ne, hipMemcpyDeviceToHost));
    }
    if (ctx->rough_info.has_sub) {
        if (sub) HIPCHK(hipMemcpy(sub, ctx->d_sub1.p, sizeof(double) * FS * nm * ne * ne, hipMemcpyDeviceToHost));
        if (sub_coh) HIPCHK(hipMemcpy(sub_coh, ctx->d_sub2.p, sizeof(double) * FS * nm * ne, hipMemcpyDeviceToHost));
    }
    return (int32_t)ns;
}

int32_t smrt_dort_rough_info(smrt_dort_ctx* ctx, double* info, int32_t n) {
    if (!ctx || !info || n < 0) return -1;
    size_t free_b = 0, total_b = 0;
    if (n > 5 && hipMemGetInfo(&free_b, &total_b) != hipSuccess) free_b = 0;
    const double v[6] = {(double)SMRT_ROUGH_M_MAX, (double)ctx->rough_info.slots, (double)ctx->rough_info.ms,
                         (double)ctx->rough_info.built_bytes, (double)ctx->rough_info.host_matrix_bytes,
                         (double)(free_b + ctx->d_itf.cap + ctx->d_sub1.cap)};
    for (int k = 0; k < n && k < 6; ++k) info[k] = v[k];
    return 6;
}

int32_t smrt_dort_launch(smrt_dort_ctx* ctx, void* out_dev, void* status_dev) {
    if (!ctx) return -1;
    if (!ctx->uploaded) { ctx->err = "no batch uploaded"; return -1; }
    HIPCHK(hipSetDevice(ctx->device));
    DevBatch d = ctx->dev;
    if (out_dev) d.out = (double*)out_dev;
    if (status_dev) d.status = (int*)status_dev;
    if (ctx->timing_pending) {
        HIPCHK(hipEventSynchronize(ctx->ev1));
        float ms = 0.f;
        HIPCHK(hipEventElapsedTime(&ms, ctx->ev0, ctx->ev1));
        ctx->last_ms = ms; ctx->total_ms += ms; ctx->n_launch++;
        ctx->timing_pending = false;
    }
    HIPCHK(hipEventRecord(ctx->ev0, ctx->stream));
    hipError_t e;
    const bool lds_pipeline = !ctx->gmem_path && ctx->split && ctx->chunk_pairs > 0 && (!ctx->active || ctx->finish2);
    if (ctx->gmem_split || lds_pipeline) e = launch_pipeline(ctx, d);
    else if (ctx->gmem_path) e = smrt_launch::fused_gmem(ctx, d, ctx->nmax_rows <= 128 ? 2 : ctx->nmax_rows <= 256 ? 4 : 6, ctx->active);
    else e = smrt_launch::fused(ctx, d, ctx->nt, ctx->active);
    HIPCHK(e);
    HIPCHK(hipEventRecord(ctx->ev1, ctx->stream));
    ctx->timing_pending = true;
    return 0;
}

int32_t smrt_dort_sync(smrt_dort_ctx* ctx) {
    if (!ctx) return -1;
    HIPCHK(hipSetDevice(ctx->device));
    HIPCHK(hipStreamSynchronize(ctx->stream));
    if (ctx->timing_pending) {
        float ms = 0.f;
        HIPCHK(hipEventElapsedTime(&ms, ctx->ev0, ctx->ev1));
        ctx->last_ms = ms; ctx->total_ms += ms; ctx->n_launch++;
        ctx->timing_pending = false;
    }
    return 0;
}

double smrt_dort_last_kernel_ms(smrt_dort_ctx* ctx) { return ctx ? (double)ctx->last_ms : -1.0; }

int32_t smrt_dort_kernel_breakdown(smrt_dort_ctx* ctx, int32_t enable, double* ms3) {
    if (!ctx) return -1;
    HIPCHK(hipSetDevice(ctx->device));
    if (ms3) {
        HIPCHK(hipStreamSynchronize(ctx->stream));
        ms3[0] = ms3[1] = ms3[2] = 0.0;
        for (size_t k = 0; k < ctx->bd_kind.size() && 2 * k + 1 < ctx->bd_used; ++k) {
            float ms = 0.f;
            HIPCHK(hipEventElapsedTime(&ms, ctx->bd_events[2 * k], ctx->bd_events[2 * k + 1]));
            ms3[ctx->bd_kind[k]] += ms;
        }
    }
    const int32_t recorded = (int32_t)ctx->bd_kind.size();
    if (enable >= 0) {
        ctx->breakdown_on = (enable != 0);
        if (!ctx->breakdown_on) { ctx->bd_used = 0; ctx->bd_kind.clear(); }
    }
    return recorded;
}

int32_t smrt_dort_launch_info(smrt_dort_ctx* ctx, int64_t* info, int32_t n) {
    if (!ctx || !info || n < 0) return -1;
    if (!ctx->uploaded) { ctx->err = "no batch uploaded"; return -1; }
    const DevBatch& d = ctx->dev;
    const bool lds_pipeline = !ctx->gmem_path && ctx->split && ctx->chunk_pairs > 0 && (!ctx->active || ctx->finish2);
    int64_t v[SMRT_INFO_COUNT] = {0};
    v[SMRT_INFO_PIPELINE] = ctx->gmem_split ? (ctx->big ? SMRT_PIPELINE_BIG : ctx->finish_strip ? SMRT_PIPELINE_GMEM_STRIP : SMRT_PIPELINE_GMEM)
                          : lds_pipeline ? (ctx->finish_strip4 ? SMRT_PIPELINE_LDS_STRIP : ctx->finish_reg ? SMRT_PIPELINE_LDS_REG : ctx->finish2 ? SMRT_PIPELINE_LDS_TWO_SLOT : SMRT_PIPELINE_LDS_FOUR_SLOT)
                          : ctx->gmem_path ? SMRT_PIPELINE_FUSED_GMEM : SMRT_PIPELINE_FUSED;
    const bool three = ctx->gmem_split || lds_pipeline;
    v[SMRT_INFO_CHUNK_PAIRS] = three ? ctx->chunk_pairs : d.pair_count;
    v[SMRT_INFO_CHUNKS] = three ? (d.pair_count + ctx->chunk_pairs - 1) / ctx->chunk_pairs : 1;
    const int rounds = (three && d.prune_tau > 0.0 && !d.coherent && getenv("SMRT_DORT_NO_PRUNE_ROUNDS") == nullptr) ? std::min(4, d.Lmax) : 1;
    v[SMRT_INFO_PRUNE_ROUNDS] = rounds;
    v[SMRT_INFO_STAGED_ITEMS] = -1;
    if (three && (rounds > 1 || d.coherent) && ctx->n_launch + (ctx->timing_pending ? 1 : 0) > 0) {
        HIPCHK(hipSetDevice(ctx->device));
        HIPCHK(hipStreamSynchronize(ctx->stream));
        const long long items_per_pair = (long long)(ctx->active ? d.m_max + 1 : 1) * d.Lmax;
        const long long last = d.pair_count - (v[SMRT_INFO_CHUNKS] - 1) * ctx->chunk_pairs;
        std::vector<int> h((size_t)(last * items_per_pair));
        const int lanes = (ctx->lanes > 1 && d.pair_count > ctx->chunk_pairs) ? ctx->lanes : 1;
        const long long lane = (v[SMRT_INFO_CHUNKS] - 1) % lanes;
        HIPCHK(hipMemcpy(h.data(), ctx->stage.n + lane * ctx->chunk_pairs * items_per_pair, sizeof(int) * h.size(), hipMemcpyDeviceToHost));
        long long staged = 0;
        for (int x : h) staged += (x > 0);
        v[SMRT_INFO_STAGED_ITEMS] = staged;
    }
    v[SMRT_INFO_BLOCK_THREADS] = ctx->nt;
    v[SMRT_INFO_N_MAX] = ctx->nmax_rows;
    v[SMRT_INFO_DIAGONALISATION] = (three && ctx->eig) ? SMRT_DIAG_SYMMETRIC : SMRT_DIAG_JACOBI;
    v[SMRT_INFO_RAYLEIGH_CLOSED_FORM] = (three && d.rayleigh_direct) ? 1 : 0;
    v[SMRT_INFO_PREP] = (lds_pipeline && ctx->prep_layers) ? SMRT_PREP_PER_LAYER : SMRT_PREP_PER_PAIR;
    for (int k = 0; k < n && k < SMRT_INFO_COUNT; ++k) info[k] = v[k];
    return SMRT_INFO_COUNT;
}

double smrt_dort_total_kernel_ms(smrt_dort_ctx* ctx, int64_t* n_launches, int32_t reset) {
    if (!ctx) return -1.0;
    const double tot = ctx->total_ms;
    if (n_launches) *n_launches = ctx->n_launch;
    if (reset) { ctx->total_ms = 0.0; ctx->n_launch = 0; }
    return tot;
}

int32_t smrt_dort_download(smrt_dort_ctx* ctx, double* out, int32_t* status, double* layer_out, double* stream_out) {
    if (!ctx) return -1;
    if (!ctx->uploaded) { ctx->err = "no batch uploaded"; return -1; }
    HIPCHK(hipSetDevice(ctx->device));
    const DevBatch& d = ctx->dev;
    const size_t np = (size_t)d.pair_count;
    if (out) HIPCHK(hipMemcpyAsync(out, d.out, sizeof(double) * np * ctx->out_stride, hipMemcpyDeviceToHost, ctx->stream));
    if (status) HIPCHK(hipMemcpyAsync(status, d.status, sizeof(int32_t) * np, hipMemcpyDeviceToHost, ctx->stream));
    if (layer_out) HIPCHK(hipMemcpyAsync(layer_out, d.layer_out, sizeof(double) * np * d.Lmax * 5, hipMemcpyDeviceToHost, ctx->stream));
    if (stream_out) HIPCHK(hipMemcpyAsync(stream_out, d.stream_out, sizeof(double) * np * (1 + d.n_max_stream), hipMemcpyDeviceToHost, ctx->stream));
    return smrt_dort_sync(ctx);
}

double smrt_dort_sum_n3(smrt_dort_ctx* ctx) {
    if (!ctx || !ctx->uploaded) return -1.0;
    if (hipSetDevice(ctx->device) != hipSuccess) return -1.0;
    std::vector<double> h((size_t)ctx->dev.pair_count);
    if (hipMemcpy(h.data(), ctx->dev.n3_out, sizeof(double) * h.size(), hipMemcpyDeviceToHost) != hipSuccess) return -1.0;
    double s = 0.0;
    for (double v : h) s += v;
    return s;
}

int32_t smrt_dort_ft_even_phase(smrt_dort_ctx* ctx, int32_t emmodel, int32_t microstructure, double frequency, double frac_volume,
                                double temperature, double micro_p1, double micro_p2, const double* mu_s, int32_t n_s,
                                const double* mu_i, int32_t n_i, int32_t m_max, int32_t npol, double* out) {
    if (!ctx) return -1;
    if (!mu_s || !mu_i || !out || n_s < 1 || n_i < 1 || m_max < 0 || m_max > 64 || (npol != 2 && npol != 3)) {
        ctx->err = "invalid ft_even_phase request";
        return -1;
    }
    if (emmodel < SMRT_EM_IBA || (emmodel > SMRT_EM_NONSCATTERING && emmodel != SMRT_EM_IBA_INVERTED) ||
        (microstructure != SMRT_MS_EXPONENTIAL && microstructure != SMRT_MS_STICKY_HARD_SPHERES)) {
        ctx->err = "unknown emmodel / microstructure";
        return -1;
    }
    for (int i = 0; i < n_s; ++i) if (!(fabs(mu_s[i]) <= 1.0)) { ctx->err = "cosines must lie in [-1, 1]"; return -1; }
    for (int i = 0; i < n_i; ++i) if (!(fabs(mu_i[i]) <= 1.0)) { ctx->err = "cosines must lie in [-1, 1]"; return -1; }
    HIPCHK(hipSetDevice(ctx->device));
    const size_t n_out = (size_t)npol * npol * (m_max + 1) * n_s * n_i;
    const size_t bytes = sizeof(double) * (n_out + n_s + n_i) + 16;
    HIPCHK(ctx->d_phase.reserve(bytes));
    double* d_out = (double*)ctx->d_phase.p;
    double* d_mus = d_out + n_out;
    double* d_mui = d_mus + n_s;
    int* d_status = (int*)(d_mui + n_i);
    HIPCHK(hipMemcpyAsync(d_mus, mu_s, sizeof(double) * n_s, hipMemcpyHostToDevice, ctx->stream));
    HIPCHK(hipMemcpyAsync(d_mui, mu_i, sizeof(double) * n_i, hipMemcpyHostToDevice, ctx->stream));
    HIPCHK(hipMemsetAsync(d_status, 0, sizeof(int), ctx->stream));
    PhaseRequest q{emmodel, microstructure, frequency, frac_volume, temperature, micro_p1, micro_p2, d_mus, n_s, d_mui, n_i,
                   m_max, npol, azimuth_samples(m_max), d_out, d_status};
    HIPCHK(smrt_launch::ft_even_phase(ctx, q));
    int st = 0;
    HIPCHK(hipMemcpyAsync(out, d_out, sizeof(double) * n_out, hipMemcpyDeviceToHost, ctx->stream));
    HIPCHK(hipMemcpyAsync(&st, d_status, sizeof(int), hipMemcpyDeviceToHost, ctx->stream));
    HIPCHK(hipStreamSynchronize(ctx->stream));
    if (st != 0) { ctx->err = "invalid layer properties (temperature above the freezing point?)"; return -1; }
    return 0;
}

int32_t smrt_dort_pair_cost(smrt_dort_ctx* ctx, double* cost) {
    if (!ctx || !cost) return -1;
    if (!ctx->uploaded) { ctx->err = "no batch uploaded"; return -1; }
    HIPCHK(hipSetDevice(ctx->device));
    HIPCHK(smrt_launch::pair_cost(ctx, ctx->dev, ctx->dev.n3_out));
    HIPCHK(hipMemcpyAsync(cost, ctx->dev.n3_out, sizeof(double) * (size_t)ctx->dev.pair_count, hipMemcpyDeviceToHost, ctx->stream));
    HIPCHK(hipStreamSynchronize(ctx->stream));
    return 0;
}

int32_t smrt_dort_stage_cycles(smrt_dort_ctx* ctx, double* out16) {
// ... 26 lines not shown
```

smrt_amd/csrc/dort_layout.hpp:

```cpp
#pragma once
#include "spmd.hpp"
#include <math.h>
#include <string.h>

#if defined(SMRT_HOST_EMU)
#define SMRT_HD_EARLY inline
#else
#define SMRT_HD_EARLY __host__ __device__ inline
#endif

namespace smrt {

struct DevBatch {
    int S, Lmax, F, n_theta;
    int emmodel, micro, mode, n_max_stream, m_max, normalization, rayleigh_jeans;
    int want_layer_out, want_stream_out;
    int jac_in_lds;
    long long pair_begin, pair_count;
    const long long* pair_map;
    const int* n_layers;
    const double* thickness;
    const double* frac_volume;
    const double* temperature;
    const double* p1;
    const double* p2;
    const double* frequency;
    const double* theta;
    const int* layer_kind;
    const double* host_layer;
    const double* host_coeff;
    const int* host_streams;
    const double* host_phase;
    int host_modes, host_ne;
    int coherent;
    const double* host_substrate;
    const double* host_substrate_coh;
    const int* host_itf_slot;
    const double* host_itf;
    const double* host_itf_coh;
    int host_itf_slots;
    const double* liquid_water;
    const double* gl_mu;
    int sub_kind;
    const double *sub_p1, *sub_p2;
    const double* sub_T;
    const double *atm_down, *atm_up, *atm_trans;
    double phi;
    double jacobi_skip2, jacobi_exit2;
    double prune_tau;
    int layer_lo, layer_hi;
    const int* pair_done;
    const int* dispatch;
    double* out;
    int* status;
    double* layer_out;
    double* stream_out;
    double* n3_out;
    double* stage_out;
    int rayleigh_direct;
};

struct DevStage {
    double* L;
    double* B;
    double* d;
    double* sigma;
    int* n;
    long long mat_stride;
    int vec_stride;
    double* Linv;
    double* ws;
    int linv_stride;
    double* eig_e;
    double* eig_rot;
    long long rot_stride;
    double* rec;
    int rec_stride;
};

enum { kPrepRecN = 0 , kPrepRecKe, kPrepRecKs, kPrepRecPa, kPrepRecPb, kPrepRecPc, kPrepRecLo ,
       kPrepRecHead = 8  };

constexpr int kStageDirect = 4096;
SMRT_DEV int stage_rows(int n) { return n > 0 ? (n & (kStageDirect - 1)) : n; }
SMRT_DEV bool stage_direct(int n) { return n > kStageDirect; }

SMRT_DEV long long global_pair(const DevBatch& b, long long p) {
    return b.pair_map ? b.pair_map[b.pair_begin + p] : b.pair_begin + p;
}

SMRT_DEV long long dispatched_pair(const DevBatch& b, long long w) { return b.dispatch ? (long long)b.dispatch[w] : w; }

SMRT_DEV long long jacobi_item_of_block(const DevBatch& b, long long blk) {
    const int span = b.layer_hi - b.layer_lo;
    long long row = blk / span;
    if (b.dispatch) {
        const int nmodes = (b.mode == 1) ? b.m_max + 1 : 1;
        row = (long long)b.dispatch[row / nmodes] * nmodes + row % nmodes;
    }
    return row * b.Lmax + b.layer_lo + (blk % span);
}

constexpr double kCSpeed = 299792458.0;
constexpr double kPlanck = 6.62607015e-34;
constexpr double kBoltzmann = 1.380649e-23;
constexpr double kFreezing = 273.15;
constexpr double kPi = 3.14159265358979323846;

enum { EM_IBA = 0, EM_DMRT = 1, EM_QCACP = 2, EM_NONSCAT = 3, EM_HOST = 4, EM_IBA_INV = 5, EM_IBA_HOST = 6, EM_RAYLEIGH_HOST = 7 };
SMRT_HD_EARLY bool em_has_rayleigh_phase(int em) { return em == EM_DMRT || em == EM_QCACP || em == EM_NONSCAT || em == EM_RAYLEIGH_HOST; }
enum { MS_EXP = 0, MS_SHS = 1, MS_SPHERE = 2, MS_TS = 3, MS_EXPC = 4, MS_SHSC = 5, MS_SPHEREC = 6, MS_TSC = 7 };
enum { ST_OK = 0, ST_EIGEN = 1, ST_NORM = 2, ST_ALBEDO = 3, ST_SINGULAR = 4, ST_INPUT = 5, ST_COHERENT = 6 };
#if defined(SMRT_HOST_EMU)
constexpr bool kSoilInstanceByDefault = true;
#else
constexpr bool kSoilInstanceByDefault = false;
#endif
enum { SUB_NONE = 0, SUB_FLAT = 1, SUB_REFLECTOR = 2, SUB_HOST = 3, SUB_SOIL_WEGMULLER = 4, SUB_SOIL_QNH = 5, SUB_ROUGH_CHOUDHURY = 6 };

struct LdsPlan {
    int NMAX, LD, nmax, Lmax, nphi, ntheta;
    int slim;
    int matrices_in_lds;
    int mat_doubles;
    int scratch_doubles;
    int o_M[4];
    int o_rowvec;
    int o_strvec;
    int o_layvec;
    int o_phi;
    int o_tb;
    int o_int;
    int o_gj;
    int o_act;
    int stage_bufs;
    int o_jac;
    int total;
};

#if defined(SMRT_HOST_EMU)
#define SMRT_HD inline
#else
#define SMRT_HD __host__ __device__ inline
#endif

SMRT_HD int active_doubles(int n_max_stream, int Lmax, int ntheta, bool with_norm0 = true) {
    return 9 * 2 * ntheta + 2 * 2 * ntheta + (2 * ntheta + 2) / 2 + 1 + (with_norm0 ? 2 * n_max_stream * Lmax : 0);
}
SMRT_HD int prep_record_doubles(int n_max_stream) { return kPrepRecHead + 2 * n_max_stream; }
SMRT_HD int azimuth_samples(int m_max) {
    int e = 4, v = 1;
    while (v < m_max + 1) { v *= 2; ++e; }
    return 1 << e;
}

SMRT_HD LdsPlan make_plan(int n_max_stream, int P, int Lmax, int ntheta, int nphi, int matrices_in_lds = 1,
                          int act_doubles = 0, int slim = 0, int jac_in_lds = 0) {
    LdsPlan p;
    p.nmax = n_max_stream;
    p.NMAX = n_max_stream * P;
    p.LD = (p.NMAX + 1) | 1;
    p.Lmax = Lmax;
    p.nphi = nphi;
    p.ntheta = ntheta;
    p.matrices_in_lds = matrices_in_lds;
    const bool layer = (slim == 4), setup = (slim == 5);
    const bool packed = (slim == 3 || layer);
    if (packed || setup) slim = 1;
    const int nmat = setup ? 0 : slim ? 2 : 4;
    const int one = packed ? (p.LD * (p.LD + 1)) / 2 : p.NMAX * p.LD;
    p.mat_doubles = nmat * one;
    p.scratch_doubles = !matrices_in_lds ? 256 * ((p.NMAX + 15) / 16) : 0;
    int o = 0;
    for (int i = 0; i < 4; ++i) { p.o_M[i] = (i < nmat ? i : 0) * one; }
    if (slim == 2) p.o_M[3] = p.NMAX * p.LD;
    if (matrices_in_lds) o = p.mat_doubles;
    p.slim = slim;
    p.o_rowvec = o; o += (setup ? 0 : slim == 1 ? 4 : slim == 2 ? 14 : 17) * p.NMAX;
    p.o_strvec = o; o += layer ? 0 : 6 * p.nmax;
    p.o_layvec = o; o += layer ? 0 : 15 * Lmax;
    p.o_phi = o; o += (slim == 2 || setup ? 0 : layer ? 3 * nphi : 5 * nphi);
    p.o_tb = o; o += (layer || setup) ? 0 : p.NMAX;
    p.o_int = o; o += layer ? 4 : 8;
// ... 63 lines not shown
```

smrt_amd/csrc/dort_passive.hpp:

```cpp
#pragma once
#include "spmd.hpp"
#include <math.h>
#include <string.h>
#include "dort_gauss_jordan.hpp"
#include "dort_interface_dense.hpp"

namespace smrt {

template <int NT>
SMRT_DEV int pruned_layer_count(const DevStage& stg, long long item0, int L, const double* thick, double* tau,
                                double limit) {
    const int t = tid();
    const int lane = t % SMRT_LANES, wave = t / SMRT_LANES;
    constexpr int NW = NT / SMRT_LANES;
    for (int l = wave; l < L; l += NW) {
        const long long item = item0 + l;
        const int N = stage_rows(stg.n[item]);
        double m = 1e300;
        for (int r = lane; r < N; r += SMRT_LANES) {
            const double sg = stg.sigma[item * stg.vec_stride + r];
            m = sg < m ? sg : m;
        }
        for (int k = 1; k < SMRT_LANES; k <<= 1) { const double o = shfl_xor(m, k); m = o < m ? o : m; }
        if (lane == 0) tau[l] = (N > 0) ? m * thick[l] : -1.0;
    }
    block_sync();
    double acc = 0.0;
    int keep = L;
    for (int l = 0; l < L; ++l) {
        if (tau[l] < 0.0) break;
        acc += tau[l];
        if (acc > limit) { keep = l + 1; break; }
    }
    block_sync();
    return keep;
}

SMRT_DEV void prune_mark_pair(const DevBatch& b, const DevStage& stg, long long p, int* done) {
    const int lane = tid() % SMRT_LANES;
    const long long gp = global_pair(b, p);
    const int si = (int)(gp % b.S);
    const int L = b.n_layers[si];
    const int nmodes = (b.mode == 1) ? b.m_max + 1 : 1;
    const double* thick = b.thickness + (long long)si * b.Lmax;
    const int upto = b.layer_hi < L ? b.layer_hi : L;
    bool all_cut = true;
    for (int m = 0; m < nmodes; ++m) {
        double acc = 0.0;
        bool cut = false;
        for (int l = 0; l < upto && !cut; ++l) {
            const long long item = (p * nmodes + m) * b.Lmax + l;
            const int N = stage_rows(stg.n[item]);
            if (N < 0) { cut = true; break; }
            if (N == 0) break;
            double mn = 1e300;
            for (int r = lane; r < N; r += SMRT_LANES) { const double sg = stg.sigma[item * stg.vec_stride + r]; mn = sg < mn ? sg : mn; }
            for (int k = 1; k < SMRT_LANES; k <<= 1) { const double o = shfl_xor(mn, k); mn = o < mn ? o : mn; }
            acc += mn * thick[l];
            if (acc > b.prune_tau) cut = true;
        }
        all_cut = all_cut && cut;
    }
    if (lane == 0) done[p] = all_cut ? 1 : 0;
}

SMRT_DEV int first_failed_layer(const DevStage& stg, long long item0, int n_kept) {
    for (int l = 0; l < n_kept; ++l) {
        const int n = stg.n[item0 + l];
        if (n < 0) return -n;
    }
    return ST_OK;
}

template <int NT>
SMRT_DEV void fail_pair(const DevBatch& b, long long p, int code, int out_stride) {
    const int t = tid();
    for (int i = t; i < out_stride; i += NT) b.out[p * out_stride + i] = NAN;
    if (t == 0) b.status[p] = code;
}


template <int NT>
SMRT_DEV int pair_setup(const DevBatch& b, const Lds& s, double frequency, int L , const double* thickness,
                        const double* fracvol, const double* temperature, const double* mp1, const double* mp2,
                        const int* kinds = nullptr ,
                        long long gp = 0 ) {
    const int t = tid();
    const int nmax = b.n_max_stream;
// ... 572 lines not shown
        if (l > 0 || hs >= 0) {
            const int Nue = (hs >= 0) ? N : Nu;
            const int nc = (N < Nue) ? N : Nue;
            for_2d<NT>(Nue, Nue, [&](int i, int j) {
                double v = (i == j) ? s.Rbu[i] : 0.0;
                if (i < nc && j < nc) v += s.Ttop[i] * K[j * LD + i] * s.Tbu[j];
                s.M3[j * LD + i] = v;
            });
            for (int i = t; i < Nue; i += NT) s.svec[i] = (i < nc) ? s.Ttop[i] * s.up[i] : 0.0;
            block_sync();
            if (hs >= 0) {
                const int Nabove = (l > 0) ? Nu : n_air * P;
                if (!interface_dense_step<NT>(host_interface_matrices(b, gp, hs, 0, 1), 3 * nmax, K, s.M3, s.up, s.svec, s.gj,
                                              N, Nabove, LD, true)) { fail_pair<NT>(b, p, ST_SINGULAR, out_stride); return; }
            }
        }
        rough_surface = (l == 0 && hs >= 0);
    }

    if (MODE == 1) {
        if (t == 0) b.status[p] = ST_OK;
#ifdef SMRT_STAGE_TIMING
        SMRT_STAGE(SG_OUT);
        if (t == 0 && b.stage_out) for (int k = 0; k < 4; ++k) b.stage_out[p * 16 + k] = stage_acc[k];
#endif
        return;
    }
    SMRT_STAGE(SG_OUT);
    {
        const bool atm = (b.atm_down != nullptr);
        const double Idn = atm ? (b.rayleigh_jeans ? b.atm_down[fi] : planck_radiance(frequency, b.atm_down[fi])) : 0.0;
        const double Iup = atm ? (b.rayleigh_jeans ? b.atm_up[fi] : planck_radiance(frequency, b.atm_up[fi])) : 0.0;
        const double trans = atm ? b.atm_trans[fi] : 1.0;
        const double* K0 = s.M0;
        const cplx e0 = cmk(s.eps_re[0], s.eps_im[0]);
        for (int i = t; i < n_air * P; i += NT) {
            double I0 = s.Ttop[i] * s.up[i];
            if (rough_surface) {
                double acc = 0.0;
                for (int j = 0; j < n_air * P; ++j) acc += s.M3[j * LD + i];
                I0 = acc * Idn + s.svec[i];
            } else
            if (atm && Idn != 0.0) {
                double acc = 0.0;
                const cplx slab0 = cmk(s.slab_re[0], s.slab_im[0]);
                double Rv, Rh, Tv, Th;
                for (int j = 0; j < n_air; ++j) {
                    interface_RT(frequency, cmk(1.0, 0.0), e0, s.outmu[j], slab0, s.slab_th[0], &Rv, &Rh, &Tv, &Th);
                    acc += K0[(2 * j) * LD + i] * Tv + K0[(2 * j + 1) * LD + i] * Th;
                }
                interface_RT(frequency, cmk(1.0, 0.0), e0, s.outmu[i >> 1], slab0, s.slab_th[0], &Rv, &Rh, &Tv, &Th);
                I0 += ((i & 1) ? Rh : Rv) * Idn + s.Ttop[i] * acc * Idn;
            }
            if (atm) I0 = Iup + trans * I0;
            s.tb[i] = b.rayleigh_jeans ? I0 : planck_inverse(frequency, I0);
        }
    }
    block_sync();
    for (int idx = t; idx < P * b.n_theta; idx += NT) {
        const int pol = idx / b.n_theta, it = idx % b.n_theta;
        const double um = cos(b.theta[it]);
        double x0, x1, y0, y1;
        const double top = 0.5 * (s.tb[0] + s.tb[1]);
        if (um > s.outmu[0]) { x0 = 1.0; y0 = top; x1 = s.outmu[0]; y1 = s.tb[pol]; }
        else if (n_air == 1) { x0 = 1.0; y0 = top; x1 = s.outmu[0]; y1 = s.tb[pol]; }
        else {
            int k = 0;
            while (k < n_air - 2 && um < s.outmu[k + 1]) ++k;
            x0 = s.outmu[k]; y0 = s.tb[2 * k + pol]; x1 = s.outmu[k + 1]; y1 = s.tb[2 * (k + 1) + pol];
        }
        b.out[p * out_stride + idx] = y0 + (y1 - y0) * ((um - x0) / (x1 - x0));
    }
    if (t == 0) { b.status[p] = ST_OK; if (b.n3_out) b.n3_out[p] = n3; }
#ifdef SMRT_STAGE_TIMING
    SMRT_STAGE(SG_OUT);
    if (t == 0 && b.stage_out) {
        for (int k = (MODE >= 2 ? 4 : 0); k < 16; ++k) b.stage_out[p * 16 + k] = (k < SG_COUNT) ? stage_acc[k] : 0.0;
        b.stage_out[p * 16 + 12] = (double)n_sweeps;
        for (int k = 0; k < 3; ++k) b.stage_out[p * 16 + 13 + k] = sub_acc_store[k];
    }
#endif
}

}
```

smrt_amd/csrc/dort_prep_layer.hpp:

```cpp
#pragma once
#include "dort_passive.hpp"

namespace smrt {

SMRT_DEV double prep_stream_mu(const Lds& s, int l, int j) { const double rs = s.ri[l] * s.gsin[j]; return sqrt(1.0 - rs * rs); }
SMRT_DEV double prep_stream_weight(const Lds& s, int l, int j, int n) {
    double w;
    if (j == 0) w = 1.0 - 0.5 * (prep_stream_mu(s, l, 0) + prep_stream_mu(s, l, 1));
    else if (j == n - 1) w = fabs(0.5 * (prep_stream_mu(s, l, n - 2) + prep_stream_mu(s, l, n - 1)));
    else w = fabs(0.5 * (prep_stream_mu(s, l, j - 1) - prep_stream_mu(s, l, j + 1)));
    return w;
}

template <int NT>
SMRT_DEV void dort_prep_setup_pair(const DevBatch& b, long long p, double* lds_base, const DevStage& stg) {
    const int t = tid();
    const LdsPlan plan = make_plan(b.n_max_stream, 2, b.Lmax, b.n_theta, 9, 1, 0, 5);
    Lds s = carve(lds_base, lds_base, plan);
    const int nmax = b.n_max_stream;
    const long long gp = global_pair(b, p);
    const int fi = (int)(gp / b.S), si = (int)(gp % b.S);
    const double frequency = b.frequency[fi];
    int L = b.n_layers[si];
    if (t < 8) s.ints[t] = 0;
    block_sync();
    {
        const long long o = (long long)si * b.Lmax;
        const int st = pair_setup<NT>(b, s, frequency, L, b.thickness + o, b.frac_volume + o, b.temperature + o, b.p1 + o, b.p2 + o,
                                      b.layer_kind ? b.layer_kind + o : nullptr, gp);
        if (st != ST_OK) { fail_pair<NT>(b, p, st, 2 * b.n_theta); return; }
        L = s.ints[6];
    }
    if (b.pair_done && b.pair_done[p]) return;
    for (int l = 0; l < L; ++l) {
        if (l < b.layer_lo || l >= b.layer_hi) continue;
        const long long item = p * (long long)b.Lmax + l;
        double* rec = stg.rec + item * stg.rec_stride;
        const int n = (int)s.nl[l];
        for (int j = t; j < n; j += NT) {
            rec[kPrepRecHead + j] = prep_stream_mu(s, l, j);
            rec[kPrepRecHead + nmax + j] = prep_stream_weight(s, l, j, n);
        }
        if (t == 0) {
            rec[kPrepRecN] = (double)n; rec[kPrepRecKe] = s.ks[l] + s.ka[l]; rec[kPrepRecKs] = s.ks[l];
            rec[kPrepRecPa] = s.pa[l]; rec[kPrepRecPb] = s.pb[l]; rec[kPrepRecPc] = s.pc[l]; rec[kPrepRecLo] = s.lo[l];
            stg.n[item] = 2 * n;
        }
    }
    if (t == 0) b.status[p] = ST_OK;
}

SMRT_DEV int prep_item_rows(const DevBatch& b, const DevStage& stg, long long item) {
    const long long p = item / b.Lmax;
    const int l = (int)(item % b.Lmax);
    const int si = (int)(global_pair(b, p) % b.S);
    if (l >= b.n_layers[si] || b.status[p] != ST_OK) return 0;
    if (b.pair_done && b.pair_done[p]) return 0;
    const int n = stg.n[item];
    return (n > 0 && n <= stg.vec_stride) ? n : 0;
}

template <int NT, int HI>
SMRT_DEV void dort_prep_layer_item(const DevBatch& b, const DevStage& stg, long long item, double* lds_base) {
    const int t = tid();
    const int nphi = 9;
    const LdsPlan plan = make_plan(HI / 2, 2, 0, 0, nphi, 1, 0, 4);
    Lds s = carve(lds_base, lds_base, plan);
    const int LD = plan.LD;
    const int LDG = (int)(stg.mat_stride / stg.vec_stride);
    const long long p = item / b.Lmax;
    const long long gp = global_pair(b, p);
    const int si = (int)(gp % b.S);
    const double* rec = stg.rec + item * stg.rec_stride;
    const int n = (int)rec[kPrepRecN], N = 2 * n;
    const double ke = rec[kPrepRecKe], ks = rec[kPrepRecKs], pa = rec[kPrepRecPa], pb = rec[kPrepRecPb], pc = rec[kPrepRecPc];
    const int lo = (int)rec[kPrepRecLo];

    if (t < 8) s.ints[t] = 0;
    for (int k = t; k < nphi; k += NT) {
        const double ph = kPi * (double)k / (double)(nphi - 1);
        const double c = cos(ph), sn = sin(ph);
        s.cphi[k] = c; s.s2phi[k] = sn * sn;
        s.wphi[k] = ((k == 0 || k == nphi - 1) ? 1.0 : 2.0) / (double)(2 * (nphi - 1));
    }
    for (int j = t; j < n; j += NT) {
        const double m = rec[kPrepRecHead + j], w = rec[kPrepRecHead + b.n_max_stream + j];
        s.mrow[2 * j] = m; s.mrow[2 * j + 1] = m;
        s.wrow[2 * j] = w; s.wrow[2 * j + 1] = w;
    }
    block_sync();
    auto layer_failed = [&](int code) { if (t == 0) stg.n[item] = -code; };
    const bool ray_direct = b.rayleigh_direct && stg.Linv && em_has_rayleigh_phase((int)pc & 15);
    if (!ray_direct) {
        const int T = n * (n + 1) / 2;
        const int em_l = (int)pc & 15, ms_l = (int)pc >> 4;
        const long long o = (long long)si * b.Lmax + lo;
        const double fv = b.frac_volume[o], q1 = b.p1[o], q2 = b.p2[o];
        const double krho = __builtin_expect(ms_l >= MS_EXPC, 0) ? pc - (double)(int)pc : 0.0;
        for (int idx = t; idx < T; idx += NT) {
            int i = (int)((sqrt(8.0 * (double)idx + 1.0) - 1.0) * 0.5);
            while ((i + 1) * (i + 2) / 2 <= idx) ++i;
            while (i * (i + 1) / 2 > idx) --i;
            const int j = idx - i * (i + 1) / 2;
            phase_mode0_block<true>(b, gp, lo, em_l, ms_l, pa, pb, fv, q1, q2, krho, s.cphi, s.s2phi, s.wphi, nphi, i, j,
                                    s.mrow[2 * i], s.mrow[2 * j], s.M0, s.M1, LD);
        }
    }
    block_sync();
    for (int r = t; r < N; r += NT) {
        double rs = 0.0;
        if (ray_direct) {
            double W0 = 0.0, W2 = 0.0;
            for (int j = 0; j < n; ++j) { const double wj = s.wrow[2 * j], mj = s.mrow[2 * j]; W0 += wj; W2 += wj * mj * mj; }
            const double a2 = s.mrow[r] * s.mrow[r];
            rs = pa * ((r & 1) ? (W2 + W0) : (a2 * W2 + 2.0 * (1.0 - a2) * (W0 - W2) + a2 * W0));
        } else {
            for (int c = 0; c <= r; ++c) rs += s.M0[sidx<true>(r, c, LD)] * s.wrow[c];
            for (int c = r + 1; c < N; ++c) rs += s.M0[sidx<true>(c, r, LD)] * s.wrow[c];
        }
        double nr = 1.0;
        if (b.normalization != 0 && ks != 0.0) {
            nr = ks / (0.5 * rs);
            if (b.normalization == 1 && !(fabs(nr - 1.0) <= 0.3)) lds_max(&s.ints[0], ST_NORM);
        }
        const double uu = sqrt(nr * s.wrow[r] / s.mrow[r]);
        s.u[r] = uu;
        s.d[r] = uu / s.wrow[r];
    }
    block_sync();
// ... 36 lines not shown
```

smrt_amd/csrc/k_cost.hip:

```cpp
#include "dort_ctx.hpp"
#include "dort_device.hpp"

using namespace smrt;

template <int NT>
__global__ __launch_bounds__(NT) void dort_cost_kernel(DevBatch b, double* cost) {
    extern __shared__ __attribute__((aligned(16))) double smrt_lds[];
    const long long p = blockIdx.x;
    const int P = b.mode == 1 ? 3 : 2;
    const LdsPlan plan = make_plan(b.n_max_stream, P, b.Lmax, b.n_theta, 1, 0, 0, 1);
    Lds s = carve(smrt_lds, smrt_lds, plan);
    const int t = tid();
    if (t < 8) s.ints[t] = 0;
    block_sync();
    const long long gp = global_pair(b, p);
    const int fi = (int)(gp / b.S), si = (int)(gp % b.S);
    int L = b.n_layers[si];
    const long long o = (long long)si * b.Lmax;
    const int st = pair_setup<NT>(b, s, b.frequency[fi], L, b.thickness + o, b.frac_volume + o, b.temperature + o, b.p1 + o, b.p2 + o,
                                  b.layer_kind ? b.layer_kind + o : nullptr, gp);
    if (st == ST_OK) L = s.ints[6];
    if (t == 0) {
        double c = 0.0;
        if (st == ST_OK)
            for (int l = 0; l < L; ++l) {
                const double n2 = 2.0 * s.nl[l], n3 = 3.0 * s.nl[l];
                c += n2 * n2 * n2 + (b.mode == 1 ? b.m_max * n3 * n3 * n3 : 0.0);
            }
        cost[p] = c;
    }
}

__global__ __launch_bounds__(64) void dort_prune_mark_kernel(DevBatch b, DevStage stg, int* done) {
    prune_mark_pair(b, stg, (long long)blockIdx.x, done);
}

namespace smrt_launch {
hipError_t prune_mark(smrt_dort_ctx* ctx, const DevBatch& c, int* done_dev) {
    hipLaunchKernelGGL(dort_prune_mark_kernel, dim3((unsigned)c.pair_count), dim3(64), 0, ctx->stream, c, ctx->stage, done_dev);
    return hipGetLastError();
}
hipError_t pair_cost(smrt_dort_ctx* ctx, const DevBatch& d, double* cost_dev) {
    const int P = d.mode == 1 ? 3 : 2;
    const size_t lds = (size_t)make_plan(d.n_max_stream, P, d.Lmax, d.n_theta, 1, 0, 0, 1).total * sizeof(double);
    auto kern = dort_cost_kernel<64>;
    hipError_t e = hipFuncSetAttribute((const void*)kern, hipFuncAttributeMaxDynamicSharedMemorySize, (int)lds);
    if (e != hipSuccess) return e;
    hipLaunchKernelGGL(kern, dim3((unsigned)d.pair_count), dim3(64), lds, ctx->stream, d, cost_dev);
    return hipGetLastError();
}
}
```

smrt_amd/csrc/k_eig.hip:

```cpp
#include <cstdlib>
#include "dort_ctx.hpp"
#include "dort_device.hpp"
#include "dort_eig_kernel.hpp"

using namespace smrt;

#define SMRT_EIG_ROWS(NP_, CALL) \
    if constexpr (LO < (NP_) && (NP_) - 8 < HI) if (rows <= (NP_)) { CALL; return; }
#define SMRT_EIG_ROWS16(NP_, CALL) \
    if constexpr (LO < (NP_) && (NP_) - 16 < HI) if (rows <= (NP_)) { CALL; return; }

template <int LO, int HI>
__global__ __launch_bounds__(64) void dort_eig_gram_kernel(DevBatch b, DevStage st) {
    const long long item = uniform(jacobi_item_of_block(b, (long long)blockIdx.x));
    const int rows = uniform(eig_item_rows(b, st, item));
    if (rows <= LO || rows > HI) return;
    SMRT_EIG_ROWS16(16, (eig_gram_item<16>(st, item))) SMRT_EIG_ROWS16(32, (eig_gram_item<32>(st, item)))
    SMRT_EIG_ROWS16(48, (eig_gram_item<48>(st, item))) SMRT_EIG_ROWS16(64, (eig_gram_item<64>(st, item)))
}

template <int LO, int HI>
__global__ __launch_bounds__(64) void dort_eig_tridiag_kernel(DevBatch b, DevStage st) {
    const long long item = uniform(jacobi_item_of_block(b, (long long)blockIdx.x));
    const int rows = uniform(eig_item_rows(b, st, item));
    if (rows <= LO || rows > HI) return;
    SMRT_EIG_ROWS(8, (eig_tridiag_item<8>(st, item))) SMRT_EIG_ROWS(16, (eig_tridiag_item<16>(st, item)))
    SMRT_EIG_ROWS(24, (eig_tridiag_item<24>(st, item))) SMRT_EIG_ROWS(32, (eig_tridiag_item<32>(st, item)))
    SMRT_EIG_ROWS(40, (eig_tridiag_item<40>(st, item))) SMRT_EIG_ROWS(48, (eig_tridiag_item<48>(st, item)))
    SMRT_EIG_ROWS(56, (eig_tridiag_item<56>(st, item))) SMRT_EIG_ROWS(64, (eig_tridiag_item<64>(st, item)))
}

template <int LO, int HI>
__global__ __launch_bounds__(64) void dort_eig_vectors_kernel(DevBatch b, DevStage st) {
    __shared__ __attribute__((aligned(16))) double ring[2 * kEigRingSlots];
    const long long item = uniform(jacobi_item_of_block(b, (long long)blockIdx.x));
    const int rows = uniform(eig_item_rows(b, st, item));
    if (rows <= LO || rows > HI) return;
    SMRT_EIG_ROWS(8, (eig_vectors_item<8>(st, item, ring))) SMRT_EIG_ROWS(16, (eig_vectors_item<16>(st, item, ring)))
    SMRT_EIG_ROWS(24, (eig_vectors_item<24>(st, item, ring))) SMRT_EIG_ROWS(32, (eig_vectors_item<32>(st, item, ring)))
    SMRT_EIG_ROWS(40, (eig_vectors_item<40>(st, item, ring))) SMRT_EIG_ROWS(48, (eig_vectors_item<48>(st, item, ring)))
    SMRT_EIG_ROWS(56, (eig_vectors_item<56>(st, item, ring))) SMRT_EIG_ROWS(64, (eig_vectors_item<64>(st, item, ring)))
}

__global__ __launch_bounds__(kEigChaseLanes) void dort_eig_chase_kernel(DevBatch b, DevStage st, long long items) {
    extern __shared__ __attribute__((aligned(16))) double smrt_lds[];
    const long long blk = (long long)blockIdx.x * kEigChaseLanes + threadIdx.x;
    if (blk >= items) return;
    const long long item = jacobi_item_of_block(b, blk);
    if (eig_item_rows(b, st, item) <= 0) return;
    const int nmax = st.vec_stride;
    eig_chase_lane(st, item, smrt_lds + threadIdx.x, smrt_lds + kEigChaseLanes * nmax + threadIdx.x);
}

namespace smrt_launch {
template <int LO, int HI>
static hipError_t go_gram(smrt_dort_ctx* ctx, const DevBatch& c, long long items) {
    hipLaunchKernelGGL((dort_eig_gram_kernel<LO, HI>), dim3((unsigned)items), dim3(64), 0, ctx->stream, c, ctx->stage);
    return hipGetLastError();
}
template <int LO, int HI>
static hipError_t go_tridiag(smrt_dort_ctx* ctx, const DevBatch& c, long long items) {
    hipLaunchKernelGGL((dort_eig_tridiag_kernel<LO, HI>), dim3((unsigned)items), dim3(64), 0, ctx->stream, c, ctx->stage);
    return hipGetLastError();
}
template <int LO, int HI>
static hipError_t go_vectors(smrt_dort_ctx* ctx, const DevBatch& c, long long items) {
    hipLaunchKernelGGL((dort_eig_vectors_kernel<LO, HI>), dim3((unsigned)items), dim3(64), 0, ctx->stream, c, ctx->stage);
    return hipGetLastError();
}

hipError_t eig(smrt_dort_ctx* ctx, const DevBatch& c, long long items) {
    const int nmax = ctx->nmax_rows;
    hipError_t e;
    if ((e = go_gram<0, 32>(ctx, c, items)) != hipSuccess) return e;
    if (nmax > 32 && (e = go_gram<32, 48>(ctx, c, items)) != hipSuccess) return e;
    if (nmax > 48 && (e = go_gram<48, 64>(ctx, c, items)) != hipSuccess) return e;
    if ((e = go_tridiag<0, 32>(ctx, c, items)) != hipSuccess) return e;
    if (nmax > 32 && (e = go_tridiag<32, 48>(ctx, c, items)) != hipSuccess) return e;
    if (nmax > 48 && (e = go_tridiag<48, 64>(ctx, c, items)) != hipSuccess) return e;
    {
        const size_t lds = (size_t)2 * kEigChaseLanes * nmax * sizeof(double);
        e = hipFuncSetAttribute((const void*)dort_eig_chase_kernel, hipFuncAttributeMaxDynamicSharedMemorySize, (int)lds);
        if (e != hipSuccess) return e;
        hipLaunchKernelGGL(dort_eig_chase_kernel, dim3((unsigned)((items + kEigChaseLanes - 1) / kEigChaseLanes)), dim3(kEigChaseLanes), lds, ctx->stream, c, ctx->stage, items);
        if ((e = hipGetLastError()) != hipSuccess) return e;
    }
    if ((e = go_vectors<0, 32>(ctx, c, items)) != hipSuccess) return e;
    if (nmax > 32 && (e = go_vectors<32, 48>(ctx, c, items)) != hipSuccess) return e;
    if (nmax > 48 && (e = go_vectors<48, 64>(ctx, c, items)) != hipSuccess) return e;
    return hipSuccess;
}
}
```

smrt_amd/csrc/k_prep_layer.hip:

```cpp
#include <cstdlib>
#include "dort_ctx.hpp"
#include "dort_device.hpp"
#include "dort_prep_layer.hpp"

using namespace smrt;

__global__ __launch_bounds__(64) void dort_prep_setup_kernel(DevBatch b, DevStage st) {
    extern __shared__ __attribute__((aligned(16))) double smrt_lds[];
    dort_prep_setup_pair<64>(b, dispatched_pair(b, (long long)blockIdx.x), smrt_lds, st);
}

template <int NT, int LO, int HI, int WAVES>
__global__ __launch_bounds__(NT, WAVES) void dort_prep_layer_kernel(DevBatch b, DevStage st) {
    extern __shared__ __attribute__((aligned(16))) double smrt_lds[];
    const long long item = jacobi_item_of_block(b, (long long)blockIdx.x);
    const int rows = prep_item_rows(b, st, item);
    if (rows <= LO || rows > HI) return;
    dort_prep_layer_item<NT, HI>(b, st, item, smrt_lds);
}

namespace smrt_launch {

template <int NT, int LO, int HI, int WAVES>
static hipError_t go_layer(smrt_dort_ctx* ctx, const DevBatch& c, long long items) {
    const size_t lds = sizeof(double) * (size_t)make_plan(HI / 2, 2, 0, 0, 9, 1, 0, 4).total;
    hipError_t e = hipFuncSetAttribute((const void*)dort_prep_layer_kernel<NT, LO, HI, WAVES>, hipFuncAttributeMaxDynamicSharedMemorySize, (int)lds);
    if (e != hipSuccess) return e;
    hipLaunchKernelGGL((dort_prep_layer_kernel<NT, LO, HI, WAVES>), dim3((unsigned)items), dim3(NT), lds, ctx->stream, c, ctx->stage);
    return hipGetLastError();
}

hipError_t prep_layers(smrt_dort_ctx* ctx, const DevBatch& c, long long items) {
    const size_t lds = sizeof(double) * (size_t)make_plan(c.n_max_stream, 2, c.Lmax, c.n_theta, 9, 1, 0, 5).total;
    hipLaunchKernelGGL(dort_prep_setup_kernel, dim3((unsigned)c.pair_count), dim3(64), lds, ctx->stream, c, ctx->stage);
    hipError_t e = hipGetLastError();
    if (e != hipSuccess) return e;
    const int nmax = ctx->nmax_rows;
    static const bool nt128 = getenv("SMRT_DORT_PREP_LAYER_NT") && atoi(getenv("SMRT_DORT_PREP_LAYER_NT")) == 128;
    if (nt128) {
        if ((e = go_layer<128, 0, 32, 4>(ctx, c, items)) != hipSuccess) return e;
        if (nmax > 32 && (e = go_layer<128, 32, 48, 4>(ctx, c, items)) != hipSuccess) return e;
    } else {
        if ((e = go_layer<256, 0, 32, 4>(ctx, c, items)) != hipSuccess) return e;
        if (nmax > 32 && (e = go_layer<256, 32, 48, 4>(ctx, c, items)) != hipSuccess) return e;
    }
    if (nmax > 48 && (e = go_layer<256, 48, 64, 4>(ctx, c, items)) != hipSuccess) return e;
    return hipSuccess;
}

}
```

Before: 180,500.

## Build per-size-class item lists so row-class kernels launch only matching items

```diff
diff --git a/__graft_entry__.py b/__graft_entry__.py
--- a/__graft_entry__.py
+++ b/__graft_entry__.py
@@ -90,6 +90,10 @@
     prep_src = os.path.join(EMU_DIR, "prep_layer_host.cpp")
     if force or _newer(prep_lib, emu_src + [prep_src]):
         _run(["g++", "-O2", "-std=c++17", "-shared", "-fPIC", "-I", EMU_DIR, "-o", prep_lib, prep_src])
+    lists_lib = os.path.join(EMU_DIR, "libclass_lists_host.so")
+    lists_src = os.path.join(EMU_DIR, "class_lists_host.cpp")
+    if force or _newer(lists_lib, emu_src + [lists_src]):
+        _run(["g++", "-O2", "-std=c++17", "-shared", "-fPIC", "-DSMRT_HOST_EMU", "-I", EMU_DIR, "-o", lists_lib, lists_src])
     if ROOT not in sys.path:
         sys.path.insert(0, ROOT)
     import smrt_amd
diff --git a/include/smrt_dort.h b/include/smrt_dort.h
--- a/include/smrt_dort.h
+++ b/include/smrt_dort.h
@@ -135,9 +135,11 @@
 
 int32_t smrt_dort_set_prep(smrt_dort_ctx* ctx, int32_t mode);
 
+int32_t smrt_dort_set_class_lists(smrt_dort_ctx* ctx, int32_t mode);
+
 enum { SMRT_INFO_PIPELINE = 0, SMRT_INFO_CHUNK_PAIRS, SMRT_INFO_CHUNKS, SMRT_INFO_PRUNE_ROUNDS, SMRT_INFO_STAGED_ITEMS,
        SMRT_INFO_BLOCK_THREADS, SMRT_INFO_N_MAX, SMRT_INFO_DIAGONALISATION, SMRT_INFO_RAYLEIGH_CLOSED_FORM, SMRT_INFO_PREP,
-       SMRT_INFO_COUNT };
+       SMRT_INFO_CLASS_LISTS, SMRT_INFO_CLASS_LIST_ITEMS, SMRT_INFO_CLASS_LIST_MISSES, SMRT_INFO_COUNT };
 enum { SMRT_PREP_PER_PAIR = 0, SMRT_PREP_PER_LAYER = 1 };
 enum { SMRT_DIAG_JACOBI = 0,
        SMRT_DIAG_SYMMETRIC = 1 };
diff --git a/smrt_amd/_native.py b/smrt_amd/_native.py
--- a/smrt_amd/_native.py
+++ b/smrt_amd/_native.py
@@ -637,6 +637,8 @@
     lib.smrt_dort_set_diagonalisation.restype = C.c_int32
     lib.smrt_dort_set_prep.argtypes = [C.c_void_p, C.c_int32]
     lib.smrt_dort_set_prep.restype = C.c_int32
+    lib.smrt_dort_set_class_lists.argtypes = [C.c_void_p, C.c_int32]
+    lib.smrt_dort_set_class_lists.restype = C.c_int32
     lib.smrt_dort_gather_plan.argtypes = [C.c_int32, C.c_int32, C.c_int32, P(C.c_int64), C.c_void_p, C.c_int32,
                                           P(C.c_int64), P(C.c_int64)]
     lib.smrt_dort_gather_plan.restype = C.c_int32
@@ -845,7 +847,7 @@
     "smrt_dort_upload", "smrt_dort_upload_pairs", "smrt_dort_run_pairs", "smrt_dort_abi", "smrt_dort_pair_cost", "smrt_dort_ft_even_phase",
     "smrt_dort_launch_info", "smrt_dort_comm_library", "smrt_dort_comm_unique_id", "smrt_dort_comm_init", "smrt_dort_comm_init_all", "smrt_dort_comm_destroy", "smrt_dort_gather",
     "smrt_dort_comm_allreduce_max", "smrt_dort_launch", "smrt_dort_sync", "smrt_dort_download", "smrt_dort_last_kernel_ms", "smrt_dort_kernel_breakdown",
-    "smrt_dort_total_kernel_ms", "smrt_dort_set_block_threads", "smrt_dort_set_pipeline", "smrt_dort_set_diagonalisation", "smrt_dort_set_prep", "smrt_dort_sum_n3", "smrt_dort_stage_cycles", "smrt_dort_device_count", "smrt_gauss_legendre_positive",
+    "smrt_dort_total_kernel_ms", "smrt_dort_set_block_threads", "smrt_dort_set_pipeline", "smrt_dort_set_diagonalisation", "smrt_dort_set_prep", "smrt_dort_set_class_lists", "smrt_dort_sum_n3", "smrt_dort_stage_cycles", "smrt_dort_device_count", "smrt_gauss_legendre_positive",
     "smrt_dort_version", "smrt_dort_finish_reg_lds_bytes", "smrt_dort_finish_strip_lds_bytes", "smrt_dort_jacobi_lds_bytes", "smrt_dort_gather_plan",
     "smrt_first_order_out_stride", "smrt_first_order_run_pairs", "smrt_first_order_upload_pairs", "smrt_first_order_launch",
     "smrt_first_order_sync", "smrt_first_order_download", "smrt_first_order_kernel_ms", "smrt_first_order_abi",
@@ -942,6 +944,10 @@
         code = -1 if mode in (None, "default") else self.PREPS.index(mode)
         self._check(self._lib.smrt_dort_set_prep(self._h, code), "smrt_dort_set_prep")
 
+    def set_class_lists(self, mode="default"):
+        code = -1 if mode in (None, "default") else int(bool(mode))
+        self._check(self._lib.smrt_dort_set_class_lists(self._h, code), "smrt_dort_set_class_lists")
+
     def run(self, batch: PackedBatch, pair_begin=0, pair_count=-1, pairs=None) -> BatchOutput:
         if pairs is not None:
             pairs = np.ascontiguousarray(pairs, dtype=np.int64)
@@ -1267,12 +1273,15 @@
         n = self._lib.smrt_dort_launch_info(self._h, v, 16)
         self._check(0 if n > 0 else -1, "smrt_dort_launch_info")
         keys = ("pipeline", "chunk_pairs", "chunks", "prune_rounds", "staged_items", "block_threads", "n_max", "diagonalisation",
-                "rayleigh_closed_form", "prep")
+                "rayleigh_closed_form", "prep", "class_lists", "class_list_items", "class_list_misses")
         d = {k: int(v[i]) for i, k in enumerate(keys[:n])}
         d["pipeline"] = self.PIPELINES[d["pipeline"]]
         d["diagonalisation"] = self.DIAGONALISATIONS[d["diagonalisation"]]
         d["rayleigh_closed_form"] = bool(d.get("rayleigh_closed_form", 0))
         d["prep"] = self.PREPS[d.get("prep", 0)]
+        d["class_lists"] = bool(d.get("class_lists", 0))
+        if d.get("class_list_items", -1) < 0:
+            d["class_list_items"] = None
         if d.get("staged_items", -1) < 0:
             d["staged_items"] = None
         return d
diff --git a/smrt_amd/csrc/dort_class_lists.hpp b/smrt_amd/csrc/dort_class_lists.hpp
--- /dev/null
+++ b/smrt_amd/csrc/dort_class_lists.hpp
@@ -0,0 +1,71 @@
+#pragma once
+#include <vector>
+
+#include "dort_layout.hpp"
+
+namespace smrt {
+
+constexpr int kRowClasses = 3;
+SMRT_HD int row_class(int rows) { return rows <= 0 ? -1 : rows <= 32 ? 0 : rows <= 48 ? 1 : rows <= 64 ? 2 : -1; }
+template <int LO, int HI>
+constexpr int row_class_index() {
+    static_assert((LO == 0 && HI == 32) || (LO == 32 && HI == 48) || (LO == 48 && HI == 64), "not a size class of rows");
+    return LO == 0 ? 0 : LO == 32 ? 1 : 2;
+}
+
+SMRT_DEV int setup_item_rows(const Lds& s, int l) { return 2 * (int)s.nl[l]; }
+
+SMRT_DEV void class_count_pair(const DevBatch& b, const Lds& s, int st, long long p, int* rows, int* counts) {
+    const int L = (st == ST_OK) ? s.ints[6] : 0;
+    int c0 = 0, c1 = 0, c2 = 0;
+    for (int l = 0; l < b.Lmax; ++l) {
+        const int r = (l < L) ? setup_item_rows(s, l) : 0;
+        rows[p * b.Lmax + l] = r;
+        const int k = row_class(r);
+        c0 += (k == 0); c1 += (k == 1); c2 += (k == 2);
+    }
+    counts[p * kRowClasses] = c0; counts[p * kRowClasses + 1] = c1; counts[p * kRowClasses + 2] = c2;
+}
+
+struct ClassListPlan {
+    long long pair_count = 0, chunk_pairs = 0, chunks = 0, total = 0;
+    std::vector<long long> pair_offset, seg_offset, seg_count;
+    bool empty() const { return chunks == 0; }
+    void clear() { *this = ClassListPlan(); }
+};
+inline ClassListPlan make_class_list_plan(const int* counts, const int* dispatch, long long pair_count, long long chunk_pairs) {
+    ClassListPlan plan;
+    plan.pair_count = pair_count; plan.chunk_pairs = chunk_pairs;
+    plan.chunks = (pair_count + chunk_pairs - 1) / chunk_pairs;
+    plan.pair_offset.assign((size_t)pair_count * kRowClasses, 0);
+    plan.seg_offset.assign((size_t)plan.chunks * kRowClasses, 0);
+    plan.seg_count.assign((size_t)plan.chunks * kRowClasses, 0);
+    long long at = 0;
+    for (long long c = 0; c < plan.chunks; ++c) {
+        const long long c0 = c * chunk_pairs, cn = (chunk_pairs < pair_count - c0) ? chunk_pairs : pair_count - c0;
+        for (int k = 0; k < kRowClasses; ++k) {
+            plan.seg_offset[(size_t)c * kRowClasses + k] = at;
+            for (long long i = 0; i < cn; ++i) {
+                const long long slot = c0 + (dispatch ? (long long)dispatch[c0 + i] : i);
+                plan.pair_offset[(size_t)(c0 + i) * kRowClasses + k] = at;
+                at += counts[slot * kRowClasses + k];
+            }
+            plan.seg_count[(size_t)c * kRowClasses + k] = at - plan.seg_offset[(size_t)c * kRowClasses + k];
+        }
+    }
+    plan.total = at;
+    return plan;
+}
+
+SMRT_DEV void class_fill_pair(int Lmax, long long chunk_pairs, const int* dispatch, const int* rows, const long long* pair_offset, long long w, int* list) {
+    const long long c0 = (w / chunk_pairs) * chunk_pairs;
+    const long long slot = dispatch ? (long long)dispatch[w] : w - c0;
+    long long at[kRowClasses];
+    for (int k = 0; k < kRowClasses; ++k) at[k] = pair_offset[w * kRowClasses + k];
+    for (int l = 0; l < Lmax; ++l) {
+        const int k = row_class(rows[(c0 + slot) * Lmax + l]);
+        if (k >= 0) list[at[k]++] = (int)(slot * Lmax + l);
+    }
+}
+
+}
diff --git a/smrt_amd/csrc/dort_ctx.hpp b/smrt_amd/csrc/dort_ctx.hpp
--- a/smrt_amd/csrc/dort_ctx.hpp
+++ b/smrt_amd/csrc/dort_ctx.hpp
@@ -3,6 +3,7 @@
 #include <string>
 #include <vector>
 
+#include "dort_class_lists.hpp"
 #include "dort_layout.hpp"
 
 namespace smrt { struct PhaseRequest; struct FoBatch; }
@@ -28,7 +29,7 @@
     hipStream_t stream = nullptr;
     hipEvent_t ev0 = nullptr, ev1 = nullptr;
     std::string err;
-    DevBuf d_nl, d_thick, d_fv, d_temp, d_p1, d_p2, d_freq, d_theta, d_gl, d_out, d_status, d_layer, d_stream, d_n3, d_stage, d_work, d_stL, d_stB, d_std, d_sts, d_stn, d_sti, d_sub1, d_sub2, d_subT, d_atm, d_pairmap, d_kind, d_phase, d_done, d_hostlayer, d_hostcoeff, d_hoststreams, d_hostphase, d_dispatch, d_regws, d_itfslot, d_itf, d_itfcoh, d_lw, d_ste, d_strot, d_strec;
+    DevBuf d_nl, d_thick, d_fv, d_temp, d_p1, d_p2, d_freq, d_theta, d_gl, d_out, d_status, d_layer, d_stream, d_n3, d_stage, d_work, d_stL, d_stB, d_std, d_sts, d_stn, d_sti, d_sub1, d_sub2, d_subT, d_atm, d_pairmap, d_kind, d_phase, d_done, d_hostlayer, d_hostcoeff, d_hoststreams, d_hostphase, d_dispatch, d_regws, d_itfslot, d_itf, d_itfcoh, d_lw, d_ste, d_strot, d_strec, d_clrows, d_clcounts, d_cloffsets, d_cllist, d_clmiss;
     smrt::DevBatch dev{};
     bool uploaded = false;
     int out_stride = 0;
@@ -38,6 +39,11 @@
     size_t finish2_lds_bytes = 0;
     size_t finish_reg_lds_bytes = 0;
     size_t prep_wide_lds_bytes = 0;
+    int class_lists_mode = -1;
+    bool class_lists = false;
+    smrt::ClassListPlan class_plan;
+    std::vector<int32_t> dispatch_host;
+    std::vector<int32_t> class_counts_host;
     int prep_mode = -1;
     bool prep_layers = false;
     bool prep_wide = false;
@@ -93,17 +99,27 @@
 #define SMRT_JACOBI_NT 256
 #endif
 
+struct ClassSegments { const int* list[smrt::kRowClasses]; long long count[smrt::kRowClasses]; };
+
 namespace smrt_launch {
 hipError_t prep(smrt_dort_ctx* ctx, const smrt::DevBatch& c, int nt);
 hipError_t prep_wide(smrt_dort_ctx* ctx, const smrt::DevBatch& c);
 hipError_t finish(smrt_dort_ctx* ctx, const smrt::DevBatch& c, int nt, bool two_slot);
 void occupancy_report(smrt_dort_ctx* ctx, int nt);
-hipError_t prep_layers(smrt_dort_ctx* ctx, const smrt::DevBatch& c, long long items);
+hipError_t prep_layers(smrt_dort_ctx* ctx, const smrt::DevBatch& c, long long items, const ClassSegments* seg);
 hipError_t finish_reg(smrt_dort_ctx* ctx, const smrt::DevBatch& c);
 hipError_t finish_strip(smrt_dort_ctx* ctx, const smrt::DevBatch& c);
 hipError_t finish_strip4(smrt_dort_ctx* ctx, const smrt::DevBatch& c);
 hipError_t jacobi(smrt_dort_ctx* ctx, const smrt::DevBatch& c, long long items);
-hipError_t eig(smrt_dort_ctx* ctx, const smrt::DevBatch& c, long long items);
+hipError_t eig(smrt_dort_ctx* ctx, const smrt::DevBatch& c, long long items, const ClassSegments* seg);
+template <int LO, int HI>
+inline bool class_launch(smrt::DevBatch& cl, long long& items, const ClassSegments* seg) {
+    if (!seg) return true;
+    constexpr int k = smrt::row_class_index<LO, HI>();
+    if (seg->count[k] == 0) return false;
+    cl.class_list = seg->list[k]; items = seg->count[k];
+    return true;
+}
 hipError_t rayleigh(smrt_dort_ctx* ctx, const smrt::DevBatch& c, long long items);
 hipError_t active_prep(smrt_dort_ctx* ctx, const smrt::DevBatch& c, int nt);
 hipError_t active_finish(smrt_dort_ctx* ctx, const smrt::DevBatch& c, int nt);
@@ -116,7 +132,8 @@
 hipError_t fused_gmem(smrt_dort_ctx* ctx, const smrt::DevBatch& d, int ch, bool active);
 hipError_t ft_even_phase(smrt_dort_ctx* ctx, const smrt::PhaseRequest& q);
 hipError_t prune_mark(smrt_dort_ctx* ctx, const smrt::DevBatch& c, int* done_dev);
-hipError_t pair_cost(smrt_dort_ctx* ctx, const smrt::DevBatch& d, double* cost_dev);
+hipError_t pair_cost(smrt_dort_ctx* ctx, const smrt::DevBatch& d, double* cost_dev, int* class_rows_dev = nullptr, int* class_counts_dev = nullptr);
+hipError_t class_fill(smrt_dort_ctx* ctx, const smrt::DevBatch& d, long long chunk_pairs, const int* rows_dev, const long long* pair_offset_dev, int* list_dev);
 void first_order_release(smrt_dort_ctx* ctx);
 void successive_order_release(smrt_dort_ctx* ctx);
 void successive_order_active_release(smrt_dort_ctx* ctx);
diff --git a/smrt_amd/csrc/dort_device.hpp b/smrt_amd/csrc/dort_device.hpp
--- a/smrt_amd/csrc/dort_device.hpp
+++ b/smrt_amd/csrc/dort_device.hpp
@@ -4,6 +4,7 @@
 #include <string.h>
 
 #include "dort_layout.hpp"
+#include "dort_class_lists.hpp"
 #include "dort_physics.hpp"
 #include "dort_dense.hpp"
 #include "dort_gauss_jordan.hpp"
diff --git a/smrt_amd/csrc/dort_hip.hip b/smrt_amd/csrc/dort_hip.hip
--- a/smrt_amd/csrc/dort_hip.hip
+++ b/smrt_amd/csrc/dort_hip.hip
@@ -54,8 +54,8 @@
     const long long modes = ctx->active ? d.m_max + 1 : 1;
     if (getenv("SMRT_DORT_DEBUG_OCCUPANCY") && !ctx->gmem_path && !ctx->active) smrt_launch::occupancy_report(ctx, ctx->nt);
     const int rounds = (d.prune_tau > 0.0 && !d.coherent && getenv("SMRT_DORT_NO_PRUNE_ROUNDS") == nullptr) ? std::min(4, d.Lmax) : 1;
-    auto prep = [&](const DevBatch& c, unsigned grid) {
-        if (ctx->prep_layers) return smrt_launch::prep_layers(ctx, c, c.pair_count * (c.layer_hi - c.layer_lo));
+    auto prep = [&](const DevBatch& c, unsigned grid, const ClassSegments* seg) {
+        if (ctx->prep_layers) return smrt_launch::prep_layers(ctx, c, c.pair_count * (c.layer_hi - c.layer_lo), seg);
         if (ctx->big) return smrt_launch::prep_gmem_big(ctx, c, grid, ctx->active, ctx->nmax_rows <= 256 ? 4 : 6);
         if (ctx->prep_wide) return smrt_launch::prep_wide(ctx, c);
         if (ctx->gmem_split) return smrt_launch::prep_gmem(ctx, c, grid, ctx->active);
@@ -124,12 +124,19 @@
             if ((e = hipMemsetAsync(done_lane, 0, sizeof(int) * (size_t)cn, ctx->stream)) != hipSuccess) return e;
             c.pair_done = (const int*)done_lane;
         }
+        ClassSegments segs{};
+        const bool listed = ctx->class_lists && rounds == 1 && chunk_index < ctx->class_plan.chunks;
+        for (int k = 0; listed && k < kRowClasses; ++k) {
+            segs.list[k] = (const int*)ctx->d_cllist.p + ctx->class_plan.seg_offset[(size_t)chunk_index * kRowClasses + k];
+            segs.count[k] = ctx->class_plan.seg_count[(size_t)chunk_index * kRowClasses + k];
+        }
+        const ClassSegments* seg = listed ? &segs : nullptr;
         for (int r = 0; r < rounds; ++r) {
             c.layer_lo = (int)((long long)d.Lmax * r / rounds);
             c.layer_hi = (int)((long long)d.Lmax * (r + 1) / rounds);
-            if ((e = timed(0, [&]() { return prep(c, grid); })) != hipSuccess) return e;
+            if ((e = timed(0, [&]() { return prep(c, grid, seg); })) != hipSuccess) return e;
             const long long jitems = cn * modes * (c.layer_hi - c.layer_lo);
-            if ((e = timed(1, [&]() { hipError_t e1 = ctx->big ? smrt_launch::jacobi_big(ctx, c, jitems) : ctx->eig ? smrt_launch::eig(ctx, c, jitems) : smrt_launch::jacobi(ctx, c, jitems);
+            if ((e = timed(1, [&]() { hipError_t e1 = ctx->big ? smrt_launch::jacobi_big(ctx, c, jitems) : ctx->eig ? smrt_launch::eig(ctx, c, jitems, seg) : smrt_launch::jacobi(ctx, c, jitems);
                                            if (e1 == hipSuccess && c.rayleigh_direct) e1 = smrt_launch::rayleigh(ctx, c, jitems);
                                            return e1; })) != hipSuccess) return e;
             if (r + 1 < rounds && (e = smrt_launch::prune_mark(ctx, c, done_lane)) != hipSuccess) return e;
@@ -192,7 +199,7 @@
     DevBuf* bufs[] = {&ctx->d_nl, &ctx->d_thick, &ctx->d_fv, &ctx->d_temp, &ctx->d_p1, &ctx->d_p2, &ctx->d_freq,
                       &ctx->d_theta, &ctx->d_gl, &ctx->d_out, &ctx->d_status, &ctx->d_layer, &ctx->d_stream, &ctx->d_n3, &ctx->d_stage, &ctx->d_work,
                       &ctx->d_stL, &ctx->d_stB, &ctx->d_std, &ctx->d_sts, &ctx->d_stn, &ctx->d_sti, &ctx->d_ste, &ctx->d_strot, &ctx->d_strec, &ctx->d_regws, &ctx->d_itfslot, &ctx->d_itf, &ctx->d_itfcoh,
-                      &ctx->d_sub1, &ctx->d_sub2, &ctx->d_subT, &ctx->d_atm, &ctx->d_pairmap, &ctx->d_kind, &ctx->d_hostlayer, &ctx->d_hoststreams, &ctx->d_hostphase, &ctx->d_dispatch, &ctx->d_phase, &ctx->d_done, &ctx->d_lw, &ctx->d_gather_out, &ctx->d_gather_status,
+                      &ctx->d_sub1, &ctx->d_sub2, &ctx->d_subT, &ctx->d_atm, &ctx->d_pairmap, &ctx->d_kind, &ctx->d_hostlayer, &ctx->d_hoststreams, &ctx->d_hostphase, &ctx->d_dispatch, &ctx->d_phase, &ctx->d_done, &ctx->d_lw, &ctx->d_clrows, &ctx->d_clcounts, &ctx->d_cloffsets, &ctx->d_cllist, &ctx->d_clmiss, &ctx->d_gather_out, &ctx->d_gather_status,
                       &ctx->d_scalar};
     for (DevBuf* b : bufs) b->release();
     smrt_launch::first_order_release(ctx);
@@ -242,6 +249,14 @@
     return 0;
 }
 
+int32_t smrt_dort_set_class_lists(smrt_dort_ctx* ctx, int32_t mode) {
+    if (!ctx) return -1;
+    if (mode < -1 || mode > 1) { ctx->err = "unknown class list mode"; return -1; }
+    ctx->class_lists_mode = mode;
+    ctx->uploaded = false;
+    return 0;
+}
+
 int32_t smrt_dort_finish_reg_lds_bytes(int32_t n_max_stream, int32_t n_layers_max) {
     return (int32_t)(sizeof(double) * (size_t)finish_reg_lds_doubles(n_max_stream, n_layers_max));
 }
@@ -320,6 +335,10 @@
         ctx->prep_layers = !ctx->gmem_path && ctx->split && !ctx->active && plan.NMAX <= 64 && want == SMRT_PREP_PER_LAYER;
     }
     const size_t rec_doubles = ctx->prep_layers ? (size_t)prep_record_doubles(b->n_max_stream) : 0;
+    bool want_lists = ctx->class_lists_mode != 0;
+    if (const char* e = getenv("SMRT_DORT_CLASS_LISTS")) want_lists = atoi(e) != 0;
+    ctx->class_lists = false;
+    ctx->class_plan.clear();
     int big_min = 128;
     if (const char* e = getenv("SMRT_DORT_BIG_MIN_N")) big_min = std::max(64, atoi(e));
     ctx->big = ctx->gmem_path && ctx->split && plan.NMAX > big_min && getenv("SMRT_DORT_NO_BIG_PIPELINE") == nullptr &&
@@ -335,7 +354,8 @@
         const size_t nmodes = ctx->active ? (size_t)b->m_max + 1 : 1;
         const size_t mat = (size_t)plan.NMAX * plan.LD;
         const int linv_stride = (plan.NMAX > 64) ? 2048 : 1024;
-        const size_t per_pair = nmodes * b->n_layers_max * ((2 * mat + 2 * plan.NMAX + linv_stride + rec_doubles) * sizeof(double) + sizeof(int));
+        const size_t per_pair = nmodes * b->n_layers_max * ((2 * mat + 2 * plan.NMAX + linv_stride + rec_doubles) * sizeof(double) + sizeof(int) +
+                                                                  (want_lists && !ctx->active && plan.NMAX <= 64 ? 2 * sizeof(int) : 0));
         double budget = 12.0e9;
         if (ctx->big) {
             size_t free_b = 0, total_b = 0;
@@ -353,6 +373,7 @@
             if (const char* e = getenv("SMRT_DORT_EIG")) want = atoi(e) ? SMRT_DIAG_SYMMETRIC : SMRT_DIAG_JACOBI;
             ctx->eig = !ctx->gmem_path && !ctx->active && plan.NMAX <= 64 && want == SMRT_DIAG_SYMMETRIC;
         }
+        ctx->class_lists = want_lists && (ctx->prep_layers || ctx->eig) && chunk * (long long)b->n_layers_max < 0x7fffffffLL;
         ctx->lanes = 1;
         if (!ctx->gmem_path) {
             int want = ctx->eig ? 3 : SMRT_DORT_LANES_DEFAULT;
@@ -564,6 +585,7 @@
     d.atm_trans = has_atm ? (const double*)ctx->d_atm.p + 2 * b->n_frequencies : nullptr;
     d.prune_tau = (b->prune_optical_depth > 0.0) ? b->prune_optical_depth : 0.0;
     d.layer_lo = 0; d.layer_hi = b->n_layers_max; d.pair_done = nullptr;
+    d.class_list = nullptr; d.class_miss = nullptr;
     if (d.prune_tau > 0.0) HIPCHK(ctx->d_done.reserve(sizeof(int) * (size_t)std::max<long long>(ctx->chunk_pairs, 1) * ctx->lanes));
     const bool orth = ctx->finish_reg || ctx->finish_strip || ctx->finish_strip4;
     d.jacobi_skip2 = ctx->active ? 1e-30 : (orth ? SMRT_JACOBI_REG_SKIP_COS2 : SMRT_JACOBI_PASSIVE_SKIP_COS2);
@@ -582,21 +604,45 @@
     HIPCHK(hipStreamSynchronize(ctx->stream));
     ctx->uploaded = true;
     d.dispatch = nullptr;
-    if (pair_count > 1 && getenv("SMRT_DORT_NO_COST_ORDER") == nullptr) {
-        HIPCHK(smrt_launch::pair_cost(ctx, d, d.n3_out));
+    const bool cost_order = pair_count > 1 && getenv("SMRT_DORT_NO_COST_ORDER") == nullptr;
+    if (cost_order || ctx->class_lists) {
+        const long long Lmax = b->n_layers_max;
+        int *rows_dev = nullptr, *counts_dev = nullptr;
+        if (ctx->class_lists) {
+            HIPCHK(ctx->d_clrows.reserve(sizeof(int) * (size_t)(pair_count * Lmax)));
+            HIPCHK(ctx->d_clcounts.reserve(sizeof(int) * (size_t)pair_count * kRowClasses));
+            HIPCHK(ctx->d_clmiss.reserve(sizeof(unsigned long long)));
+            HIPCHK(hipMemsetAsync(ctx->d_clmiss.p, 0, sizeof(unsigned long long), ctx->stream));
+            rows_dev = (int*)ctx->d_clrows.p; counts_dev = (int*)ctx->d_clcounts.p;
+            d.class_miss = (unsigned long long*)ctx->d_clmiss.p;
+        }
+        HIPCHK(smrt_launch::pair_cost(ctx, d, d.n3_out, rows_dev, counts_dev));
         std::vector<double> cost((size_t)pair_count);
         HIPCHK(hipMemcpyAsync(cost.data(), d.n3_out, sizeof(double) * cost.size(), hipMemcpyDeviceToHost, ctx->stream));
+        if (ctx->class_lists) {
+            ctx->class_counts_host.resize((size_t)pair_count * kRowClasses);
+            HIPCHK(hipMemcpyAsync(ctx->class_counts_host.data(), counts_dev, sizeof(int32_t) * ctx->class_counts_host.size(), hipMemcpyDeviceToHost, ctx->stream));
+        }
         HIPCHK(hipStreamSynchronize(ctx->stream));
-        std::vector<int32_t> order((size_t)pair_count);
         const long long chunk = ctx->chunk_pairs > 0 ? ctx->chunk_pairs : pair_count;
-        for (long long c0 = 0; c0 < pair_count; c0 += chunk) {
-            const long long cn = std::min<long long>(chunk, pair_count - c0);
-            for (long long i = 0; i < cn; ++i) order[(size_t)(c0 + i)] = (int32_t)i;
-            std::stable_sort(order.begin() + c0, order.begin() + c0 + cn,
-                             [&](int32_t a, int32_t b2) { return cost[(size_t)(c0 + a)] > cost[(size_t)(c0 + b2)]; });
-        }
-        if (upload_array(ctx, ctx->d_dispatch, order.data(), sizeof(int32_t) * order.size())) return -1;
-        d.dispatch = (const int*)ctx->d_dispatch.p;
+        if (cost_order) {
+            std::vector<int32_t>& order = ctx->dispatch_host;
+            order.resize((size_t)pair_count);
+            for (long long c0 = 0; c0 < pair_count; c0 += chunk) {
+                const long long cn = std::min<long long>(chunk, pair_count - c0);
+                for (long long i = 0; i < cn; ++i) order[(size_t)(c0 + i)] = (int32_t)i;
+                std::stable_sort(order.begin() + c0, order.begin() + c0 + cn,
+                                 [&](int32_t a, int32_t b2) { return cost[(size_t)(c0 + a)] > cost[(size_t)(c0 + b2)]; });
+            }
+            if (upload_array(ctx, ctx->d_dispatch, order.data(), sizeof(int32_t) * order.size())) return -1;
+            d.dispatch = (const int*)ctx->d_dispatch.p;
+        }
+        if (ctx->class_lists) {
+            ctx->class_plan = make_class_list_plan(ctx->class_counts_host.data(), cost_order ? ctx->dispatch_host.data() : nullptr, pair_count, chunk);
+            if (upload_array(ctx, ctx->d_cloffsets, ctx->class_plan.pair_offset.data(), sizeof(long long) * ctx->class_plan.pair_offset.size())) return -1;
+            HIPCHK(ctx->d_cllist.reserve(sizeof(int) * (size_t)std::max<long long>(ctx->class_plan.total, 1)));
+            HIPCHK(smrt_launch::class_fill(ctx, d, chunk, rows_dev, (const long long*)ctx->d_cloffsets.p, (int*)ctx->d_cllist.p));
+        }
     }
     return 0;
 }
@@ -755,6 +801,16 @@
     v[SMRT_INFO_DIAGONALISATION] = (three && ctx->eig) ? SMRT_DIAG_SYMMETRIC : SMRT_DIAG_JACOBI;
     v[SMRT_INFO_RAYLEIGH_CLOSED_FORM] = (three && d.rayleigh_direct) ? 1 : 0;
     v[SMRT_INFO_PREP] = (lds_pipeline && ctx->prep_layers) ? SMRT_PREP_PER_LAYER : SMRT_PREP_PER_PAIR;
+    v[SMRT_INFO_CLASS_LISTS] = (lds_pipeline && ctx->class_lists && rounds == 1) ? 1 : 0;
+    v[SMRT_INFO_CLASS_LIST_ITEMS] = (lds_pipeline && ctx->class_lists) ? ctx->class_plan.total : -1;
+    v[SMRT_INFO_CLASS_LIST_MISSES] = 0;
+    if (lds_pipeline && ctx->class_lists) {
+        unsigned long long misses = 0;
+        HIPCHK(hipSetDevice(ctx->device));
+        HIPCHK(hipStreamSynchronize(ctx->stream));
+        HIPCHK(hipMemcpy(&misses, ctx->d_clmiss.p, sizeof(misses), hipMemcpyDeviceToHost));
+        v[SMRT_INFO_CLASS_LIST_MISSES] = (int64_t)misses;
+    }
     for (int k = 0; k < n && k < SMRT_INFO_COUNT; ++k) info[k] = v[k];
     return SMRT_INFO_COUNT;
 }
diff --git a/smrt_amd/csrc/dort_layout.hpp b/smrt_amd/csrc/dort_layout.hpp
--- a/smrt_amd/csrc/dort_layout.hpp
+++ b/smrt_amd/csrc/dort_layout.hpp
@@ -58,6 +58,8 @@
     double* n3_out;
     double* stage_out;
     int rayleigh_direct;
+    const int* class_list;
+    unsigned long long* class_miss;
 };
 
 struct DevStage {
@@ -99,6 +101,19 @@
         row = (long long)b.dispatch[row / nmodes] * nmodes + row % nmodes;
     }
     return row * b.Lmax + b.layer_lo + (blk % span);
+}
+
+SMRT_DEV long long class_item_of_block(const DevBatch& b, long long blk) {
+    return b.class_list ? (long long)b.class_list[blk] : jacobi_item_of_block(b, blk);
+}
+SMRT_DEV void class_list_left(const DevBatch& b, int rows) {
+    if (b.class_list && rows > 0 && tid() == 0) {
+#if defined(SMRT_HOST_EMU)
+        ++*b.class_miss;
+#else
+        atomicAdd(b.class_miss, 1ULL);
+#endif
+    }
 }
 
 constexpr double kCSpeed = 299792458.0;
diff --git a/smrt_amd/csrc/dort_passive.hpp b/smrt_amd/csrc/dort_passive.hpp
--- a/smrt_amd/csrc/dort_passive.hpp
+++ b/smrt_amd/csrc/dort_passive.hpp
@@ -4,6 +4,7 @@
 #include <string.h>
 #include "dort_gauss_jordan.hpp"
 #include "dort_interface_dense.hpp"
+#include "dort_class_lists.hpp"
 
 namespace smrt {
 
@@ -742,4 +743,31 @@
 #endif
 }
 
-}
+template <int NT>
+SMRT_DEV void dort_cost_pair(const DevBatch& b, long long p, double* lds_base, double* cost, int* class_rows, int* class_counts) {
+    const int P = b.mode == 1 ? 3 : 2;
+    const LdsPlan plan = make_plan(b.n_max_stream, P, b.Lmax, b.n_theta, 1, 0, 0, 1);
+    Lds s = carve(lds_base, lds_base, plan);
+    const int t = tid();
+    if (t < 8) s.ints[t] = 0;
+    block_sync();
+    const long long gp = global_pair(b, p);
+    const int fi = (int)(gp / b.S), si = (int)(gp % b.S);
+    int L = b.n_layers[si];
+    const long long o = (long long)si * b.Lmax;
+    const int st = pair_setup<NT>(b, s, b.frequency[fi], L, b.thickness + o, b.frac_volume + o, b.temperature + o, b.p1 + o, b.p2 + o,
+                                  b.layer_kind ? b.layer_kind + o : nullptr, gp);
+    if (st == ST_OK) L = s.ints[6];
+    if (t == 0) {
+        double c = 0.0;
+        if (st == ST_OK)
+            for (int l = 0; l < L; ++l) {
+                const double n2 = 2.0 * s.nl[l], n3 = 3.0 * s.nl[l];
+                c += n2 * n2 * n2 + (b.mode == 1 ? b.m_max * n3 * n3 * n3 : 0.0);
+            }
+        cost[p] = c;
+        if (class_rows) class_count_pair(b, s, st, p, class_rows, class_counts);
+    }
+}
+
+}
diff --git a/smrt_amd/csrc/dort_prep_layer.hpp b/smrt_amd/csrc/dort_prep_layer.hpp
--- a/smrt_amd/csrc/dort_prep_layer.hpp
+++ b/smrt_amd/csrc/dort_prep_layer.hpp
@@ -1,4 +1,5 @@
 #pragma once
+#include "dort_class_lists.hpp"
 #include "dort_passive.hpp"
 
 namespace smrt {
@@ -44,7 +45,7 @@
         if (t == 0) {
             rec[kPrepRecN] = (double)n; rec[kPrepRecKe] = s.ks[l] + s.ka[l]; rec[kPrepRecKs] = s.ks[l];
             rec[kPrepRecPa] = s.pa[l]; rec[kPrepRecPb] = s.pb[l]; rec[kPrepRecPc] = s.pc[l]; rec[kPrepRecLo] = s.lo[l];
-            stg.n[item] = 2 * n;
+            stg.n[item] = setup_item_rows(s, l);
         }
     }
     if (t == 0) b.status[p] = ST_OK;
diff --git a/smrt_amd/csrc/k_cost.hip b/smrt_amd/csrc/k_cost.hip
--- a/smrt_amd/csrc/k_cost.hip
+++ b/smrt_amd/csrc/k_cost.hip
@@ -4,31 +4,15 @@
 using namespace smrt;
 
 template <int NT>
-__global__ __launch_bounds__(NT) void dort_cost_kernel(DevBatch b, double* cost) {
+__global__ __launch_bounds__(NT) void dort_cost_kernel(DevBatch b, double* cost, int* class_rows, int* class_counts) {
     extern __shared__ __attribute__((aligned(16))) double smrt_lds[];
-    const long long p = blockIdx.x;
-    const int P = b.mode == 1 ? 3 : 2;
-    const LdsPlan plan = make_plan(b.n_max_stream, P, b.Lmax, b.n_theta, 1, 0, 0, 1);
-    Lds s = carve(smrt_lds, smrt_lds, plan);
-    const int t = tid();
-    if (t < 8) s.ints[t] = 0;
-    block_sync();
-    const long long gp = global_pair(b, p);
-    const int fi = (int)(gp / b.S), si = (int)(gp % b.S);
-    int L = b.n_layers[si];
-    const long long o = (long long)si * b.Lmax;
-    const int st = pair_setup<NT>(b, s, b.frequency[fi], L, b.thickness + o, b.frac_volume + o, b.temperature + o, b.p1 + o, b.p2 + o,
-                                  b.layer_kind ? b.layer_kind + o : nullptr, gp);
-    if (st == ST_OK) L = s.ints[6];
-    if (t == 0) {
-        double c = 0.0;
-        if (st == ST_OK)
-            for (int l = 0; l < L; ++l) {
-                const double n2 = 2.0 * s.nl[l], n3 = 3.0 * s.nl[l];
-                c += n2 * n2 * n2 + (b.mode == 1 ? b.m_max * n3 * n3 * n3 : 0.0);
-            }
-        cost[p] = c;
-    }
+    dort_cost_pair<NT>(b, (long long)blockIdx.x, smrt_lds, cost, class_rows, class_counts);
+}
+
+__global__ __launch_bounds__(256) void dort_class_fill_kernel(int Lmax, long long pair_count, long long chunk_pairs, const int* dispatch,
+                                                              const int* rows, const long long* pair_offset, int* list) {
+    const long long w = (long long)blockIdx.x * 256 + threadIdx.x;
+    if (w < pair_count) class_fill_pair(Lmax, chunk_pairs, dispatch, rows, pair_offset, w, list);
 }
 
 __global__ __launch_bounds__(64) void dort_prune_mark_kernel(DevBatch b, DevStage stg, int* done) {
@@ -40,13 +24,18 @@
     hipLaunchKernelGGL(dort_prune_mark_kernel, dim3((unsigned)c.pair_count), dim3(64), 0, ctx->stream, c, ctx->stage, done_dev);
     return hipGetLastError();
 }
-hipError_t pair_cost(smrt_dort_ctx* ctx, const DevBatch& d, double* cost_dev) {
+hipError_t pair_cost(smrt_dort_ctx* ctx, const DevBatch& d, double* cost_dev, int* class_rows_dev, int* class_counts_dev) {
     const int P = d.mode == 1 ? 3 : 2;
     const size_t lds = (size_t)make_plan(d.n_max_stream, P, d.Lmax, d.n_theta, 1, 0, 0, 1).total * sizeof(double);
     auto kern = dort_cost_kernel<64>;
     hipError_t e = hipFuncSetAttribute((const void*)kern, hipFuncAttributeMaxDynamicSharedMemorySize, (int)lds);
     if (e != hipSuccess) return e;
-    hipLaunchKernelGGL(kern, dim3((unsigned)d.pair_count), dim3(64), lds, ctx->stream, d, cost_dev);
+    hipLaunchKernelGGL(kern, dim3((unsigned)d.pair_count), dim3(64), lds, ctx->stream, d, cost_dev, class_rows_dev, class_counts_dev);
+    return hipGetLastError();
+}
+hipError_t class_fill(smrt_dort_ctx* ctx, const DevBatch& d, long long chunk_pairs, const int* rows_dev, const long long* pair_offset_dev, int* list_dev) {
+    hipLaunchKernelGGL(dort_class_fill_kernel, dim3((unsigned)((d.pair_count + 255) / 256)), dim3(256), 0, ctx->stream, d.Lmax, d.pair_count, chunk_pairs,
+                       d.dispatch, rows_dev, pair_offset_dev, list_dev);
     return hipGetLastError();
 }
 }
diff --git a/smrt_amd/csrc/k_eig.hip b/smrt_amd/csrc/k_eig.hip
--- a/smrt_amd/csrc/k_eig.hip
+++ b/smrt_amd/csrc/k_eig.hip
@@ -12,18 +12,18 @@
 
 template <int LO, int HI>
 __global__ __launch_bounds__(64) void dort_eig_gram_kernel(DevBatch b, DevStage st) {
-    const long long item = uniform(jacobi_item_of_block(b, (long long)blockIdx.x));
+    const long long item = uniform(class_item_of_block(b, (long long)blockIdx.x));
     const int rows = uniform(eig_item_rows(b, st, item));
-    if (rows <= LO || rows > HI) return;
+    if (rows <= LO || rows > HI) { class_list_left(b, rows); return; }
     SMRT_EIG_ROWS16(16, (eig_gram_item<16>(st, item))) SMRT_EIG_ROWS16(32, (eig_gram_item<32>(st, item)))
     SMRT_EIG_ROWS16(48, (eig_gram_item<48>(st, item))) SMRT_EIG_ROWS16(64, (eig_gram_item<64>(st, item)))
 }
 
 template <int LO, int HI>
 __global__ __launch_bounds__(64) void dort_eig_tridiag_kernel(DevBatch b, DevStage st) {
-    const long long item = uniform(jacobi_item_of_block(b, (long long)blockIdx.x));
+    const long long item = uniform(class_item_of_block(b, (long long)blockIdx.x));
     const int rows = uniform(eig_item_rows(b, st, item));
-    if (rows <= LO || rows > HI) return;
+    if (rows <= LO || rows > HI) { class_list_left(b, rows); return; }
     SMRT_EIG_ROWS(8, (eig_tridiag_item<8>(st, item))) SMRT_EIG_ROWS(16, (eig_tridiag_item<16>(st, item)))
     SMRT_EIG_ROWS(24, (eig_tridiag_item<24>(st, item))) SMRT_EIG_ROWS(32, (eig_tridiag_item<32>(st, item)))
     SMRT_EIG_ROWS(40, (eig_tridiag_item<40>(st, item))) SMRT_EIG_ROWS(48, (eig_tridiag_item<48>(st, item)))
@@ -33,9 +33,9 @@
 template <int LO, int HI>
 __global__ __launch_bounds__(64) void dort_eig_vectors_kernel(DevBatch b, DevStage st) {
     __shared__ __attribute__((aligned(16))) double ring[2 * kEigRingSlots];
-    const long long item = uniform(jacobi_item_of_block(b, (long long)blockIdx.x));
+    const long long item = uniform(class_item_of_block(b, (long long)blockIdx.x));
     const int rows = uniform(eig_item_rows(b, st, item));
-    if (rows <= LO || rows > HI) return;
+    if (rows <= LO || rows > HI) { class_list_left(b, rows); return; }
     SMRT_EIG_ROWS(8, (eig_vectors_item<8>(st, item, ring))) SMRT_EIG_ROWS(16, (eig_vectors_item<16>(st, item, ring)))
     SMRT_EIG_ROWS(24, (eig_vectors_item<24>(st, item, ring))) SMRT_EIG_ROWS(32, (eig_vectors_item<32>(st, item, ring)))
     SMRT_EIG_ROWS(40, (eig_vectors_item<40>(st, item, ring))) SMRT_EIG_ROWS(48, (eig_vectors_item<48>(st, item, ring)))
@@ -54,30 +54,36 @@
 
 namespace smrt_launch {
 template <int LO, int HI>
-static hipError_t go_gram(smrt_dort_ctx* ctx, const DevBatch& c, long long items) {
-    hipLaunchKernelGGL((dort_eig_gram_kernel<LO, HI>), dim3((unsigned)items), dim3(64), 0, ctx->stream, c, ctx->stage);
+static hipError_t go_gram(smrt_dort_ctx* ctx, const DevBatch& c, long long items, const ClassSegments* seg) {
+    DevBatch cl = c;
+    if (!class_launch<LO, HI>(cl, items, seg)) return hipSuccess;
+    hipLaunchKernelGGL((dort_eig_gram_kernel<LO, HI>), dim3((unsigned)items), dim3(64), 0, ctx->stream, cl, ctx->stage);
     return hipGetLastError();
 }
 template <int LO, int HI>
-static hipError_t go_tridiag(smrt_dort_ctx* ctx, const DevBatch& c, long long items) {
-    hipLaunchKernelGGL((dort_eig_tridiag_kernel<LO, HI>), dim3((unsigned)items), dim3(64), 0, ctx->stream, c, ctx->stage);
+static hipError_t go_tridiag(smrt_dort_ctx* ctx, const DevBatch& c, long long items, const ClassSegments* seg) {
+    DevBatch cl = c;
+    if (!class_launch<LO, HI>(cl, items, seg)) return hipSuccess;
+    hipLaunchKernelGGL((dort_eig_tridiag_kernel<LO, HI>), dim3((unsigned)items), dim3(64), 0, ctx->stream, cl, ctx->stage);
     return hipGetLastError();
 }
 template <int LO, int HI>
-static hipError_t go_vectors(smrt_dort_ctx* ctx, const DevBatch& c, long long items) {
-    hipLaunchKernelGGL((dort_eig_vectors_kernel<LO, HI>), dim3((unsigned)items), dim3(64), 0, ctx->stream, c, ctx->stage);
+static hipError_t go_vectors(smrt_dort_ctx* ctx, const DevBatch& c, long long items, const ClassSegments* seg) {
+    DevBatch cl = c;
+    if (!class_launch<LO, HI>(cl, items, seg)) return hipSuccess;
+    hipLaunchKernelGGL((dort_eig_vectors_kernel<LO, HI>), dim3((unsigned)items), dim3(64), 0, ctx->stream, cl, ctx->stage);
     return hipGetLastError();
 }
 
-hipError_t eig(smrt_dort_ctx* ctx, const DevBatch& c, long long items) {
+hipError_t eig(smrt_dort_ctx* ctx, const DevBatch& c, long long items, const ClassSegments* seg) {
     const int nmax = ctx->nmax_rows;
     hipError_t e;
-    if ((e = go_gram<0, 32>(ctx, c, items)) != hipSuccess) return e;
-    if (nmax > 32 && (e = go_gram<32, 48>(ctx, c, items)) != hipSuccess) return e;
-    if (nmax > 48 && (e = go_gram<48, 64>(ctx, c, items)) != hipSuccess) return e;
-    if ((e = go_tridiag<0, 32>(ctx, c, items)) != hipSuccess) return e;
-    if (nmax > 32 && (e = go_tridiag<32, 48>(ctx, c, items)) != hipSuccess) return e;
-    if (nmax > 48 && (e = go_tridiag<48, 64>(ctx, c, items)) != hipSuccess) return e;
+    if ((e = go_gram<0, 32>(ctx, c, items, seg)) != hipSuccess) return e;
+    if (nmax > 32 && (e = go_gram<32, 48>(ctx, c, items, seg)) != hipSuccess) return e;
+    if (nmax > 48 && (e = go_gram<48, 64>(ctx, c, items, seg)) != hipSuccess) return e;
+    if ((e = go_tridiag<0, 32>(ctx, c, items, seg)) != hipSuccess) return e;
+    if (nmax > 32 && (e = go_tridiag<32, 48>(ctx, c, items, seg)) != hipSuccess) return e;
+    if (nmax > 48 && (e = go_tridiag<48, 64>(ctx, c, items, seg)) != hipSuccess) return e;
     {
         const size_t lds = (size_t)2 * kEigChaseLanes * nmax * sizeof(double);
         e = hipFuncSetAttribute((const void*)dort_eig_chase_kernel, hipFuncAttributeMaxDynamicSharedMemorySize, (int)lds);
@@ -85,9 +91,9 @@
         hipLaunchKernelGGL(dort_eig_chase_kernel, dim3((unsigned)((items + kEigChaseLanes - 1) / kEigChaseLanes)), dim3(kEigChaseLanes), lds, ctx->stream, c, ctx->stage, items);
         if ((e = hipGetLastError()) != hipSuccess) return e;
     }
-    if ((e = go_vectors<0, 32>(ctx, c, items)) != hipSuccess) return e;
-    if (nmax > 32 && (e = go_vectors<32, 48>(ctx, c, items)) != hipSuccess) return e;
-    if (nmax > 48 && (e = go_vectors<48, 64>(ctx, c, items)) != hipSuccess) return e;
+    if ((e = go_vectors<0, 32>(ctx, c, items, seg)) != hipSuccess) return e;
+    if (nmax > 32 && (e = go_vectors<32, 48>(ctx, c, items, seg)) != hipSuccess) return e;
+    if (nmax > 48 && (e = go_vectors<48, 64>(ctx, c, items, seg)) != hipSuccess) return e;
     return hipSuccess;
 }
 }
diff --git a/smrt_amd/csrc/k_prep_layer.hip b/smrt_amd/csrc/k_prep_layer.hip
--- a/smrt_amd/csrc/k_prep_layer.hip
+++ b/smrt_amd/csrc/k_prep_layer.hip
@@ -13,24 +13,26 @@
 template <int NT, int LO, int HI, int WAVES>
 __global__ __launch_bounds__(NT, WAVES) void dort_prep_layer_kernel(DevBatch b, DevStage st) {
     extern __shared__ __attribute__((aligned(16))) double smrt_lds[];
-    const long long item = jacobi_item_of_block(b, (long long)blockIdx.x);
+    const long long item = class_item_of_block(b, (long long)blockIdx.x);
     const int rows = prep_item_rows(b, st, item);
-    if (rows <= LO || rows > HI) return;
+    if (rows <= LO || rows > HI) { class_list_left(b, rows); return; }
     dort_prep_layer_item<NT, HI>(b, st, item, smrt_lds);
 }
 
 namespace smrt_launch {
 
 template <int NT, int LO, int HI, int WAVES>
-static hipError_t go_layer(smrt_dort_ctx* ctx, const DevBatch& c, long long items) {
+static hipError_t go_layer(smrt_dort_ctx* ctx, const DevBatch& c, long long items, const ClassSegments* seg) {
+    DevBatch cl = c;
+    if (!class_launch<LO, HI>(cl, items, seg)) return hipSuccess;
     const size_t lds = sizeof(double) * (size_t)make_plan(HI / 2, 2, 0, 0, 9, 1, 0, 4).total;
     hipError_t e = hipFuncSetAttribute((const void*)dort_prep_layer_kernel<NT, LO, HI, WAVES>, hipFuncAttributeMaxDynamicSharedMemorySize, (int)lds);
     if (e != hipSuccess) return e;
-    hipLaunchKernelGGL((dort_prep_layer_kernel<NT, LO, HI, WAVES>), dim3((unsigned)items), dim3(NT), lds, ctx->stream, c, ctx->stage);
+    hipLaunchKernelGGL((dort_prep_layer_kernel<NT, LO, HI, WAVES>), dim3((unsigned)items), dim3(NT), lds, ctx->stream, cl, ctx->stage);
     return hipGetLastError();
 }
 
-hipError_t prep_layers(smrt_dort_ctx* ctx, const DevBatch& c, long long items) {
+hipError_t prep_layers(smrt_dort_ctx* ctx, const DevBatch& c, long long items, const ClassSegments* seg) {
     const size_t lds = sizeof(double) * (size_t)make_plan(c.n_max_stream, 2, c.Lmax, c.n_theta, 9, 1, 0, 5).total;
     hipLaunchKernelGGL(dort_prep_setup_kernel, dim3((unsigned)c.pair_count), dim3(64), lds, ctx->stream, c, ctx->stage);
     hipError_t e = hipGetLastError();
@@ -38,13 +40,13 @@
     const int nmax = ctx->nmax_rows;
     static const bool nt128 = getenv("SMRT_DORT_PREP_LAYER_NT") && atoi(getenv("SMRT_DORT_PREP_LAYER_NT")) == 128;
     if (nt128) {
-        if ((e = go_layer<128, 0, 32, 4>(ctx, c, items)) != hipSuccess) return e;
-        if (nmax > 32 && (e = go_layer<128, 32, 48, 4>(ctx, c, items)) != hipSuccess) return e;
+        if ((e = go_layer<128, 0, 32, 4>(ctx, c, items, seg)) != hipSuccess) return e;
+        if (nmax > 32 && (e = go_layer<128, 32, 48, 4>(ctx, c, items, seg)) != hipSuccess) return e;
     } else {
-        if ((e = go_layer<256, 0, 32, 4>(ctx, c, items)) != hipSuccess) return e;
-        if (nmax > 32 && (e = go_layer<256, 32, 48, 4>(ctx, c, items)) != hipSuccess) return e;
+        if ((e = go_layer<256, 0, 32, 4>(ctx, c, items, seg)) != hipSuccess) return e;
+        if (nmax > 32 && (e = go_layer<256, 32, 48, 4>(ctx, c, items, seg)) != hipSuccess) return e;
     }
-    if (nmax > 48 && (e = go_layer<256, 48, 64, 4>(ctx, c, items)) != hipSuccess) return e;
+    if (nmax > 48 && (e = go_layer<256, 48, 64, 4>(ctx, c, items, seg)) != hipSuccess) return e;
     return hipSuccess;
 }
 
```

New measurement: 185,300 (median of 6 runs). +2.7%, better.
